# mpitid/babble

Measured on AMD Instinct MI355X. Metric: consensus-ordered events/sec at N participants, higher is better.
Workload: dtype int32; 1 GPU; random-gossip DAG, 256 participants, 10000000 events per GPU, RunConsensus every K=256 events (39063 calls); participants=256, events_per_graph=10000000, k=256, graphs_per_gpu=1, parallelism=replicas1

## Files before the change

### babble_amd/csrc/hge_engine.hip

```cpp
#include <hip/hip_runtime.h>

#include <algorithm>
#include <chrono>
#include <cstdio>
#include <cstdlib>
#include <cstring>
#include <mutex>
#include <optional>
#include <string>
#include <thread>
#include <utility>
#include <vector>

#include "../../include/hge.h"
#include "hge_plan.h"
#include "hge_kernels.hip"
#include "hge_median_rows.hip"
#include "hge_wide32.hip"
#include "hge_coords.hip"
#include "hge_coords_win.hip"
#include "hge_rounds_coop.hip"
#include "hge_rounds_direct.hip"
#include "hge_walk_spec.hip"

// ... 104 lines not shown

  int R = 0;
  int R_set = 0;
  std::vector<std::vector<int32_t>> h_chain;
  int64_t cache_size = 0;
  int32_t chain_limit = INT32_MAX;
  int32_t chain_limit0 = INT32_MAX;
  bool wide32 = false, wide32_pending = false;
  int w32_done = 0;
  std::string failed;
  int test_w32_fail = getenv("HGE_TEST_W32_FAIL") ? atoi(getenv("HGE_TEST_W32_FAIL")) : 0;
  int lcr = -1;
  int lcre = 0;
  int64_t ctx = 0;
  std::vector<int32_t> consensus;
  int32_t* pin_ord = nullptr;
  int32_t* pin_ord_dev = nullptr;
  size_t pin_ord_cap = 0;
  int64_t cons_pin_n = 0;
  bool lazy_order = false;
  int64_t consensus_size() const { return (int64_t)consensus.size() + cons_pin_n; }
  void consensus_sync() {
    if (!cons_pin_n) return;
    consensus.insert(consensus.end(), pin_ord, pin_ord + cons_pin_n);
    cons_pin_n = 0;
  }
  void ensure_pin_ord(size_t n) {
    if (n <= pin_ord_cap && pin_ord) return;
    consensus_sync();
    if (pin_ord) HIPCHK(hipHostFree(pin_ord));
    pin_ord = nullptr;
    pin_ord_dev = nullptr;
    pin_ord_cap = 0;
    HIPCHK(hipHostMalloc((void**)&pin_ord, std::max<size_t>(n, 1) * 4, hipHostMallocDefault));
    pin_ord_cap = std::max<size_t>(n, 1);
    void* dp = nullptr;
    pin_ord_dev = hipHostGetDevicePointer(&dp, pin_ord, 0) == hipSuccess ? (int32_t*)dp : nullptr;
  }
  int64_t n_und = 0;

  std::vector<int64_t> replay_calls;
  std::vector<int64_t> replay_counts;

  int64_t Ecap = 0;
  int ccap = 0, Rcap = 0;
  DBuf<int32_t> d_creator, d_index, d_sp, d_op, d_ntx, d_round, d_rr, d_und;
  DBuf<int64_t> d_ts, d_cts;
  DBuf<uint64_t> d_S;
  DBuf<uint8_t> d_coin, d_wit;
  DBuf<int32_t> d_chain, d_LA, d_FD, d_FSS;
  DBuf<int32_t> s_w32, s_w32a;
  DBuf<uint32_t> d_LA16;
  DBuf<int2> d_opcp;
  DBuf<int64_t> d_tsch;
  DBuf<int32_t> d_C, d_W, d_rcnt, d_minw;
  DBuf<uint64_t> d_ssb, d_seeb;
  DBuf<uint8_t> d_fame;
  DBuf<int32_t> s_small, s_newwit;
  DBuf<int32_t> s_LCR, s_clast;
  DBuf<uint8_t> s_dec, s_decbit;
  DBuf<int32_t> s_segcnt, s_segcall, s_seground, s_theta;
  DBuf<uint8_t> s_segdec;
  DBuf<uint64_t> s_segfws;
  DBuf<int32_t> s_recv, s_rr, s_fund, s_upos, s_und2, s_bpos, s_vis;
  bool vis_all = false;
  DBuf<int64_t> s_cts;
  DBuf<unsigned char> s_keys, s_keys2;
  DBuf<int32_t> s_part, s_fst, s_relay, s_rfail;
  DBuf<uint8_t> s_dec2;
  bool minw_full = true;
  int n_sweeps = 0;
  DBuf<int32_t> d_FDT, s_chg, s_bar, s_dirty;
  DBuf<int32_t> s_src;
  DBuf<int4> s_lwplan;
  DBuf<uint32_t> s_lwsum, s_lwinit;
  DBuf<int32_t> s_lwpos, s_lwrisky;
  int ncu_cache = 0;
  int n_cu() {
    if (!ncu_cache) HIPCHK(hipDeviceGetAttribute(&ncu_cache, hipDeviceAttributeMultiprocessorCount, device));
    return ncu_cache;
  }
  DBuf<int32_t> d_FDTD;
  DBuf<uint8_t> d_FDTW;
  bool rows_bulk = false;
  bool fdtd_stale = false;
  int fdtd_maxlen = 0;
  DBuf<int32_t> s_fdlo;
  bool test_rows_fallback = getenv("HGE_TEST_MEDIAN_ROWS_FALLBACK") != nullptr;
  DBuf<int32_t> d_WLA;
  DBuf<uint16_t> d_WLR;
  DBuf<uint64_t> d_ssc, s_gran;
  DBuf<int32_t> s_bseg;
  DBuf<uint64_t> s_H;
  DBuf<int32_t> s_hn, s_hres;
  uint32_t walk_epoch = 0;
  int walk_chk[2] = {448, 2};
  bool coop_checked = false;
  int coop_nb = 0, coop_ncu = 0, coop_spec_nb = -1, coop_spec_bs = 0;
  const void* coop_spec_fn() const {
    return coop_spec_bs == 1024 ? (const void*)k_rounds_coop_spec<1024> : (const void*)k_rounds_coop_spec<512>;
  }
  DBuf<uint64_t> s_cH, s_cS, s_cT, s_cM;
  DBuf<uint32_t> s_mb;
  DBuf<int32_t> s_cn;
  uint32_t coop_epoch = 0;

  hipEvent_t ev[8] = {};
  bool prof_on = false;
  std::vector<hipEvent_t> prof_pool;
  std::vector<std::pair<std::string, int>> prof_rec;
  std::vector<std::string> prof_names;
  std::vector<double> prof_ms;
  std::vector<int64_t> prof_cnt;
  int R_div = 0;
  std::vector<int32_t> h_minw;
  DBuf<int32_t> s_cctl, s_out;
  std::vector<int32_t> h_cctl;
  int64_t* c_nc = nullptr;
  int32_t *c_Rc = nullptr, *c_Lc = nullptr, *c_flags = nullptr, *c_pr = nullptr, *c_pidx = nullptr;
  int32_t* c_sgo = nullptr;
  const int32_t* segoff_p = nullptr;
  DBuf<int32_t> s_kctl;
  std::vector<int32_t> h_kctl;
  std::vector<hge_plan::Seg> h_segs;
  bool und_fresh = false;
  float stage_ms[7] = {};

  Tables tables() const {
    Tables t;
    t.N = N;
    t.NW = NW;
    t.SM = SM;
    t.ccap = ccap;
    t.Rcap = Rcap;
    t.creator = d_creator.p;
    t.index = d_index.p;
    t.sp = d_sp.p;
    t.op = d_op.p;
    t.ts = d_ts.p;
    t.S = d_S.p;
    t.coin = d_coin.p;
    t.ntx = d_ntx.p;
    t.chain = d_chain.p;
    t.opcp = d_opcp.p;
    t.tsch = d_tsch.p;
    t.LA = d_LA.p;
    t.NW2 = (N + 1) / 2;
    t.LA16 = sweep16() ? d_LA16.p : nullptr;
    t.FD = fdt16() ? nullptr : d_FD.p;
    t.FD16 = fdt16() ? (uint16_t*)d_FD.p : nullptr;
    t.FDTD = d_FDTD.p;
    t.FDTW = d_FDTW.p;
    t.WLA = wla16() ? nullptr : d_WLA.p;
    t.WLA16 = wla16() ? (uint16_t*)d_WLA.p : nullptr;
    t.WLR = (N > 64 && !wide32) ? d_WLR.p : nullptr;
    t.round = d_round.p;
    t.wit = d_wit.p;
    t.C = d_C.p;
    t.W = d_W.p;
    t.ssb = d_ssb.p;
    t.seeb = d_seeb.p;
    t.fame = d_fame.p;
    t.rcnt = d_rcnt.p;
    return t;
  }

  void init(int n, int64_t cap, int dev) {
    N = n;
    NW = (N + 63) / 64;
    SM = 2 * N / 3 + 1;
    device = dev;
    HIPCHK(hipSetDevice(device));
    HIPCHK(hipStreamCreateWithFlags(&st, hipStreamNonBlocking));
    for (auto& e : ev) HIPCHK(hipEventCreate(&e));
    chain_len.assign(N, 0);
    chain_last.assign(N, -1);
    h_chain.assign(N, {});
    chain_limit = N > 32 ? 0xFFFE : INT32_MAX;
    if (const char* cl = getenv("HGE_CHAIN_LIMIT")) chain_limit = std::max(1, std::min(chain_limit, atoi(cl)));
    chain_limit0 = chain_limit;
    coords_len.assign(N, 0);
    const int64_t c0 = std::max<int64_t>(cap, 1024);
    ensure_events(c0);
    ensure_ccap(c0 / N + c0 / (8 * N) + 64);
    ensure_rcap(c0 / (2 * N) + 64);
    s_small.need(16);
  }

  void prof_begin(const char* name) {
    if (!prof_on) return;
    const int slot = (int)prof_rec.size() * 2;
    while ((int)prof_pool.size() < slot + 2) {
      hipEvent_t e;
      HIPCHK(hipEventCreate(&e));
      prof_pool.push_back(e);
    }
    HIPCHK(hipEventRecord(prof_pool[slot], st));
    prof_rec.push_back({name, slot});
  }
  void prof_end() {
    if (!prof_on) return;
    HIPCHK(hipEventRecord(prof_pool[prof_rec.back().second + 1], st));
  }
  void prof_collect() {
    if (prof_rec.empty()) return;
    HIPCHK(hipStreamSynchronize(st));
    for (auto& r : prof_rec) {
      float ms = 0;
      HIPCHK(hipEventElapsedTime(&ms, prof_pool[r.second], prof_pool[r.second + 1]));
      size_t k = 0;
      while (k < prof_names.size() && prof_names[k] != r.first) k++;
      if (k == prof_names.size()) {
        prof_names.push_back(r.first);
        prof_ms.push_back(0);
        prof_cnt.push_back(0);
      }
      prof_ms[k] += ms;
      prof_cnt[k] += 1;
    }
    prof_rec.clear();
  }

  DBuf<uint64_t> s_dbg;
  bool dbg_on = getenv("HGE_STAMPS") != nullptr;
  uint64_t* dbg_p() {
    if (!dbg_on) return nullptr;
    if (!s_dbg.p) {
      s_dbg.need(16);
      HIPCHK(hipMemset(s_dbg.p, 0, 16 * 8));
    }
    return s_dbg.p;
  }
  void dbg_dump() {
    if (!dbg_on || !s_dbg.p) return;
    uint64_t v[16];
    readback(v, s_dbg.p, 16);
    fprintf(stderr, "[hge stamps]");
    for (int i = 0; i < 16; i++) fprintf(stderr, " %llu", (unsigned long long)v[i]);
    fprintf(stderr, "\n");
  }

  void destroy() {
    if (st) (void)hipStreamSynchronize(st);
    if (getenv("HGE_HOST_PHASES") && hp.calls) {
      const double c = (double)hp.calls;
      fprintf(stderr,
              "{\"hge_host_phases\": {\"calls\": %lld, \"launches_per_call\": %.2f, \"copies_per_call\": %.2f, "
              "\"insert_us\": %.2f, \"consensus_us\": %.2f, \"sync_wait_us\": %.2f}}\n",
              (long long)hp.calls, hp.launches / c, hp.copies / c, hp.insert_ns / c / 1e3, hp.call_ns / c / 1e3,
              hp.wait_ns / c / 1e3);
    }
    for (auto& e : ev)
      if (e) (void)hipEventDestroy(e);
    for (auto& e : prof_pool) (void)hipEventDestroy(e);
    prof_pool.clear();
    DBuf<int32_t>* i32s[] = {&d_creator, &d_index,  &d_sp,    &d_op,     &d_ntx,     &d_round,
                             &d_rr,      &d_und,    &d_chain, &d_LA,     &d_FD,      &d_C,
                             &d_W,       &d_rcnt,   &d_minw,  &s_small,  &s_newwit,  &s_LCR,
                             &s_clast,   &s_segcnt, &s_segcall, &s_seground, &s_theta,
                             &s_recv,    &s_rr,     &s_bpos,  &s_fund,   &s_upos,    &s_vis,
                             &s_und2,    &s_part,   &s_fst,    &d_FSS,
                             &d_FDT,     &s_chg,    &s_bar,   &s_bseg,   &s_kctl,    &s_cctl,
                             &s_out,     &s_hn,     &s_hres,  &s_dirty,  &d_WLA,     &s_lwpos,
                             &s_lwrisky, &s_src,    &s_relay, &s_rfail,  &s_fdlo};
    for (auto* b : i32s) b->free_();
    s_dec2.free_();
    s_lwplan.free_();
    d_WLR.free_();
    s_xbuf.free_();
    s_sord.free_();
    s_soff.free_();
    s_lwsum.free_();
    s_lwinit.free_();
    d_ts.free_();
    d_FDTD.free_();
    d_FDTW.free_();
    d_cts.free_();
    s_cts.free_();
    d_S.free_();
    d_ssb.free_();
    d_seeb.free_();
    s_H.free_();
    s_wdbg.free_();
    s_segfws.free_();
    d_coin.free_();
    d_wit.free_();
    d_fame.free_();
    s_dec.free_();
    s_decbit.free_();
    s_segdec.free_();
    s_keys.free_();
    s_keys2.free_();
    d_opcp.free_();
    d_tsch.free_();
    d_LA16.free_();
    d_ssc.free_();
    s_gran.free_();
    s_cH.free_();
    s_cS.free_();
    s_cT.free_();
    s_cM.free_();
    s_cn.free_();
    s_mb.free_();
    s_hist.free_();
    s_hstate.free_();
    s_hssc.free_();
    if (pin) (void)hipHostFree(pin);
    pin = nullptr;
    pin_cap = pin_used = 0;
    if (pin_ord) (void)hipHostFree(pin_ord);
    pin_ord = nullptr;
    pin_ord_dev = nullptr;
    pin_ord_cap = 0;
    cons_pin_n = 0;
    if (st) (void)hipStreamDestroy(st);
    st = nullptr;
  }

  void ensure_events(int64_t m) {
    if (m <= Ecap) return;
    int64_t cap = std::max<int64_t>(m, Ecap + Ecap / 2);
    d_creator.grow_keep(cap, n_dev, st);
    d_index.grow_keep(cap, n_dev, st);
    d_sp.grow_keep(cap, n_dev, st);
    d_op.grow_keep(cap, n_dev, st);
    d_ntx.grow_keep(cap, n_dev, st);
    d_ts.grow_keep(cap, n_dev, st);
    d_S.grow_keep(4 * cap, 4 * n_dev, st);
    d_coin.grow_keep(cap, n_dev, st);
    d_round.grow_keep(cap, n_coords, st);
    d_wit.grow_keep(cap, n_coords, st);
    d_rr.grow_keep(cap, n_coords, st, 0xFF);
    d_cts.grow_keep(cap, n_coords, st, 0);
    d_und.grow_keep(cap, n_und, st);
    Ecap = cap;
  }

  template <typename T>
  void grow_chain_table(DBuf<T>& b, int64_t nc, bool keep, bool rowmajor = true) {
    T* q = nullptr;
    HIPCHK(hipMalloc(&q, sizeof(T) * (size_t)N * nc * N));
    const size_t rows = rowmajor ? N : (size_t)N * N, w = rowmajor ? N : 1;
    if (keep && ccap > 0 && b.p)
      HIPCHK(hipMemcpy2DAsync(q, sizeof(T) * nc * w, b.p, sizeof(T) * ccap * w,
                              sizeof(T) * ccap * w, rows, hipMemcpyDeviceToDevice, st));
    sync();
    b.free_();
    b.p = q;
    b.n = (size_t)N * nc * N;
  }

  void ensure_ccap(int64_t m) {
    if (m <= ccap) return;
    int64_t nc = (std::max<int64_t>(m, (int64_t)ccap + ccap / 2) + 63) & ~(int64_t)63;
    int32_t* chain = nullptr;
    HIPCHK(hipMalloc(&chain, sizeof(int32_t) * N * nc));
    HIPCHK(hipMemsetAsync(chain, 0xFF, sizeof(int32_t) * N * nc, st));
    if (ccap > 0)
      HIPCHK(hipMemcpy2DAsync(chain, sizeof(int32_t) * nc, d_chain.p, sizeof(int32_t) * ccap,
                              sizeof(int32_t) * ccap, N, hipMemcpyDeviceToDevice, st));
    sync();
    d_chain.free_();
    d_chain.p = chain;
    d_chain.n = (size_t)N * nc;
    int2* opcp = nullptr;
    HIPCHK(hipMalloc(&opcp, sizeof(int2) * N * nc));
    if (ccap > 0)
      HIPCHK(hipMemcpy2DAsync(opcp, sizeof(int2) * nc, d_opcp.p, sizeof(int2) * ccap,
                              sizeof(int2) * ccap, N, hipMemcpyDeviceToDevice, st));
    sync();
    d_opcp.free_();
    d_opcp.p = opcp;
    d_opcp.n = (size_t)N * nc;
    int64_t* tsch = nullptr;
    HIPCHK(hipMalloc(&tsch, sizeof(int64_t) * N * nc));
    if (ccap > 0)
      HIPCHK(hipMemcpy2DAsync(tsch, sizeof(int64_t) * nc, d_tsch.p, sizeof(int64_t) * ccap,
                              sizeof(int64_t) * ccap, N, hipMemcpyDeviceToDevice, st));
    sync();
    d_tsch.free_();
    d_tsch.p = tsch;
    d_tsch.n = (size_t)N * nc;
    if (!sweep16()) grow_chain_table(d_LA, nc, true);
    if (N > 32) {
      const size_t w = (size_t)(N + 1) / 2;
      uint32_t* q = nullptr;
      HIPCHK(hipMalloc(&q, sizeof(uint32_t) * (size_t)N * nc * w));
      if (ccap > 0 && d_LA16.p)
        HIPCHK(hipMemcpy2DAsync(q, sizeof(uint32_t) * nc * w, d_LA16.p, sizeof(uint32_t) * ccap * w,
                                sizeof(uint32_t) * ccap * w, N, hipMemcpyDeviceToDevice, st));
      sync();
      d_LA16.free_();
      d_LA16.p = q;
      d_LA16.n = (size_t)N * nc * w;
    }
    if (fdt16()) {
      int32_t* q = nullptr;
      HIPCHK(hipMalloc(&q, sizeof(uint16_t) * (size_t)N * nc * N));
      if (ccap > 0 && d_FD.p)
        HIPCHK(hipMemcpy2DAsync(q, 2 * (size_t)nc * N, d_FD.p, 2 * (size_t)ccap * N, 2 * (size_t)ccap * N, N,
                                hipMemcpyDeviceToDevice, st));
      sync();
      d_FD.free_();
      d_FD.p = q;
      d_FD.n = (size_t)N * nc * N / 2;
    } else {
      grow_chain_table(d_FD, nc, true);
    }
    if (N > 16) {
      grow_chain_table(d_FDTD, nc, true);
      const size_t NT = (size_t)(N + 63) / 64;
      uint8_t* q = nullptr;
      HIPCHK(hipMalloc(&q, (size_t)N * nc * NT));
      if (ccap > 0 && d_FDTW.p)
        HIPCHK(hipMemcpy2DAsync(q, nc * NT, d_FDTW.p, (size_t)ccap * NT, (size_t)ccap * NT, N,
                                hipMemcpyDeviceToDevice, st));
      sync();
      d_FDTW.free_();
      d_FDTW.p = q;
      d_FDTW.n = (size_t)N * nc * NT;
    }
    if (N <= 32) d_FSS.need((size_t)N * nc * std::max(N, 16));
    if (fdt16()) {
      int32_t* q = nullptr;
      HIPCHK(hipMalloc(&q, sizeof(int32_t) * (size_t)N * nc * N));
      if (ccap > 0 && d_FDT.p)
        HIPCHK(hipMemcpy2DAsync(q, 2 * (size_t)nc, d_FDT.p, 2 * (size_t)ccap, 2 * (size_t)ccap, (size_t)N * N,
                                hipMemcpyDeviceToDevice, st));
      sync();
      d_FDT.free_();
      d_FDT.p = q;
      d_FDT.n = (size_t)N * nc * N;
    } else {
      grow_chain_table(d_FDT, nc, true, false);
    }
    ccap = (int)nc;
  }

  void ensure_rcap(int64_t m) {
    if (m <= Rcap) return;
    int64_t nr = std::max<int64_t>(m, (int64_t)Rcap + Rcap / 2);
    const size_t oldn = (size_t)Rcap * N;
    d_C.grow_keep(nr * N, oldn, st, 0x7F);
    d_W.grow_keep(nr * N, oldn, st, 0xFF);
    d_ssb.grow_keep(nr * N * NW, oldn * NW, st, 0);
    d_seeb.grow_keep(nr * N * NW, oldn * NW, st, 0);
    if (N > 32) d_ssc.grow_keep(nr * N * NW, oldn * NW, st, 0);
    d_fame.grow_keep(nr * N, oldn, st, 0);
    d_rcnt.grow_keep(nr, Rcap, st, 0);
    d_minw.need(nr + 20);
    minw_full = true;
    fill_i32(d_C.p + oldn, (int64_t)(nr - Rcap) * N, INF32);
    sync();
    Rcap = (int)nr;
  }

  void reset_state() {
    sync();
    failed.clear();
    minw_full = true;
    cons_pin_n = 0;
    h_creator.clear();
    h_index.clear();
    h_sp.clear();
    h_op.clear();
    h_ntx.clear();
    h_ts.clear();
    h_S.clear();
    h_coin.clear();
    chain_len.assign(N, 0);
    chain_last.assign(N, -1);
    h_chain.assign(N, {});
    coords_len.assign(N, 0);
    n_events = n_dev = n_coords = n_divided = 0;
    up_n0 = up_n1 = -1;
    h_up.clear();
    R = 0;
    R_set = 0;
    h_minw.clear();
    lcr = -1;
    lcre = 0;
    ctx = 0;
    consensus.clear();
    n_und = 0;
    wide32 = wide32_pending = false;
    w32_done = 0;
    chain_limit = chain_limit0;
    reset_rounds();
    HIPCHK(hipMemsetAsync(d_chain.p, 0xFF, (size_t)N * ccap * 4, st));
    sync();
  }

  void reset_rounds() {
    const int64_t nrow = (int64_t)Rcap * N, nbits = nrow * NW;
    const int64_t most = std::max<int64_t>(std::max(nbits, Ecap), Rcap);
    KLAUNCH(k_reset_rounds, dim3(std::min(div_up(most, 256), 4096)), dim3(256), 0, st, tables(), nrow,
            nbits, Ecap, d_rr.p);
  }

  int admit(const hge_event& e, int32_t sp, int32_t op) {
    const int c = e.creator;
    if (c < 0 || c >= N) {
      err = "Could not find fake creator id";
      return HGE_ERR_CREATOR;
    }
    const int known = chain_len[c];
    if (sp == HGE_NONE && op == HGE_NONE && known == 0) {
      if (e.index != 0) {
        err = "Event index does not match the creator's chain position";
        return HGE_ERR_INDEX;
      }
      return HGE_OK;
    }
    if (sp < 0 || sp >= n_events) {
      err = "Self-parent not known";
      return HGE_ERR_SELF_PARENT_UNKNOWN;
    }
    if (h_creator[sp] != c) {
      err = "Self-parent has different creator";
      return HGE_ERR_SELF_PARENT_CREATOR;
    }
    if (op < 0 || op >= n_events) {
      err = "Other-parent not known";
      return HGE_ERR_OTHER_PARENT_UNKNOWN;
    }
    if (sp != chain_last[c]) {
      err = "Self-parent not last known event by creator";
      return HGE_ERR_SELF_PARENT_NOT_LAST;
    }
    if (e.index != known) {
      err = "Event index does not match the creator's chain position";
      return HGE_ERR_INDEX;
    }
    if (known >= chain_limit) {
      if (N > 32 && N <= 256 && !wide32) {
        size_t free_b = 0, total_b = 0;
        const size_t tab = sizeof(int32_t) * (size_t)N * N * (size_t)std::max(ccap, known + 2);
        if (hipMemGetInfo(&free_b, &total_b) == hipSuccess && free_b < (fdt16() ? 2 : 1) * tab + (64u << 20)) {
          err = "Chain capacity exceeded: the int32 position tables past 65,534 events per creator do not fit";
          return HGE_ERR_CAPACITY;
        }
        wide32_pending = true;
        chain_limit = INT32_MAX;
      } else {
        err = "Chain capacity exceeded: at most " + std::to_string(chain_limit) + " events per creator";
        return HGE_ERR_CAPACITY;
      }
    }
    return HGE_OK;
  }

  void append(const hge_event& e, int32_t sp, int32_t op) {
    const int64_t id = n_events++;
    h_creator.push_back(e.creator);
    h_index.push_back(e.index);
    h_sp.push_back(sp);
    h_op.push_back(op);
    h_ntx.push_back(e.n_tx);
    h_ts.push_back(e.timestamp_ns);
    for (int k = 0; k < 4; k++) {
      uint64_t v = 0;
      for (int b = 0; b < 8; b++) v = (v << 8) | e.s[8 * k + b];
      h_S.push_back(v);
    }
    h_coin.push_back(e.hash[16] != 0 ? 1 : 0);
    h_chain[e.creator].push_back((int32_t)id);
    chain_len[e.creator]++;
    chain_last[e.creator] = (int32_t)id;
  }

  std::vector<UpEv> h_up;
  int64_t up_n0 = -1, up_n1 = -1;
  void upload() {
    if (n_dev == n_events) return;
    ensure_events(n_events);
    int maxlen = 0;
    for (int c = 0; c < N; c++) maxlen = std::max(maxlen, chain_len[c]);
    ensure_ccap(maxlen + 1);
    const int64_t a = n_dev, m = n_events - n_dev;
    if (m <= 16384 && a == n_coords) {
      std::vector<UpEv> up((size_t)m);
      if (up_n0 >= 0) throw EngineError(HGE_ERR_INTERNAL, "packed upload pending twice");
      for (int64_t i = 0; i < m; i++) {
        UpEv& r = up[(size_t)i];
        const size_t x = (size_t)(a + i);
        r.creator = h_creator[x];
        r.index = h_index[x];
        r.sp = h_sp[x];
        r.op = h_op[x];
        r.ntx = h_ntx[x];
        r.coin = h_coin[x];
        r.ts = h_ts[x];
        for (int k = 0; k < 4; k++) r.S[k] = h_S[4 * x + k];
      }
      h_up.swap(up);
      up_n0 = a;
      up_n1 = n_events;
      n_dev = n_events;
      return;
    }
    HIPCHK(hipMemcpyAsync(d_creator.p + a, h_creator.data() + a, 4 * m, hipMemcpyHostToDevice, st));
    HIPCHK(hipMemcpyAsync(d_index.p + a, h_index.data() + a, 4 * m, hipMemcpyHostToDevice, st));
    HIPCHK(hipMemcpyAsync(d_sp.p + a, h_sp.data() + a, 4 * m, hipMemcpyHostToDevice, st));
    HIPCHK(hipMemcpyAsync(d_op.p + a, h_op.data() + a, 4 * m, hipMemcpyHostToDevice, st));
    HIPCHK(hipMemcpyAsync(d_ntx.p + a, h_ntx.data() + a, 4 * m, hipMemcpyHostToDevice, st));
    HIPCHK(hipMemcpyAsync(d_ts.p + a, h_ts.data() + a, 8 * m, hipMemcpyHostToDevice, st));
// ... 356 lines not shown
      s_fst.need(N + 1);
      KLAUNCH(k_frontier_start, dim3(1), dim3(256), 0, st, t, s.olen, s.len, s_fst.p, (int32_t*)nullptr,
              (int32_t*)nullptr, (uint64_t*)nullptr, 0);
      readback(fst.data(), s_fst.p, N + 1);
    }
    const int rlo = fst[0];
    if (rlo == INF32) return {};
    int tot = s.fresh ? s.tot0 : 0;
    if (!s.fresh) {
      std::vector<int32_t> lo_off(2 * N + 1);
      for (int c = 0; c < N; c++) {
        lo_off[c] = fst[1 + c];
        lo_off[N + c] = tot;
        tot += std::max(0, chain_len[c] - fst[1 + c]);
      }
      lo_off[2 * N] = tot;
      h2d(s.fss_lo, lo_off.data(), 4 * (2 * N + 1));
    }
    if (tot <= 0) return {};
    const bool long_chain = s.maxlen >= 0xFFFF;
    KLAUNCH_AS(k.fss_name, k.fss, dim3(div_up((int64_t)tot * k.NPC, 256)), dim3(256), 0, st, t, s.fss_lo, s.fss_off, tot,
               long_chain ? d_FSS.p : (int32_t*)nullptr, long_chain ? (uint16_t*)nullptr : (uint16_t*)d_FSS.p,
               (const int32_t*)nullptr);
    if (long_chain) {
      KLAUNCH_AS(k.rounds_fss_name, k.rounds_fss, dim3(1), dim3(64), 0, st, t, d_FSS.p, s.olen, s.len, s.rstate, rlo);
      return {};
    }
    const int nw = s.fresh ? spec_walkers(s.minlen) : 0;
    const int32_t* resume = nw > 1 ? spec_walk(t, s, k, nw) : nullptr;
    KLAUNCH_AS(k.walk_name, k.walk, dim3(1), dim3(1024), 0, st, t, (const uint16_t*)d_FSS.p, s.olen, s.len, s.rstate,
               resume ? 0 : rlo, resume ? 0 : Rprev, dbg_p(), resume, RoundAssign{});
    if (resume && getenv("HGE_WALK_DEBUG")) walk_debug(nw);
    return {};
  }
  const int32_t* spec_walk(const Tables& t, const CoordStep& s, const WalkKernels& k, int nw) {
    const char* hc = getenv("HGE_WALK_HCAP");
    const int Hcap = hc ? std::max(2, atoi(hc)) : std::max(256, std::min(Rcap, 3 * (Rcap / nw) + 256));
    if ((size_t)nw * Hcap * N > s_H.n) {
      s_H.need((size_t)nw * Hcap * N);
      HIPCHK(hipMemsetAsync(s_H.p, 0, s_H.n * sizeof(uint64_t), st));
    }
    s_hres.need(4 * (size_t)nw + 1);
    s_hn.need(2 * (size_t)nw);
    KLAUNCH_AS(k.spec_name, k.spec, dim3(nw), dim3(1024), 0, st, t, (const uint16_t*)d_FSS.p, s.len, nw, Hcap, s_H.p,
               s_hn.p, s_hn.p + nw, (int4*)s_hres.p, ++walk_epoch, walk_chk[0], walk_chk[1], walk_dbg(nw));
    int32_t* resume = s_hres.p + 4 * nw;
    KLAUNCH(k_walk_join, dim3(64), dim3(256), 0, st, t, (const uint64_t*)s_H.p, (const int32_t*)s_hn.p,
            (const int4*)s_hres.p, nw, Hcap, s.rstate, resume);
    return resume;
  }
  void assign_rounds(const CoordStep& s, const Walk& w) {
    const Tables t = tables();
    const int m = (int)(s.n1 - s.n0);
    s_newwit.need(m);
    if (s.fresh) {
      s_newwit.need((size_t)Rcap * N);
      KLAUNCH(k_round_ranges, dim3(div_up((int64_t)Rcap * N, 256)), dim3(256), 0, st, t, s.len,
              (const int32_t*)s.rstate, s_newwit.p, s.rstate + 2);
    } else if (!w.assigned) {
      und_appended = dividing && n_divided == s.n0;
      KLAUNCH(k_round_assign, dim3(div_up(m, 256)), dim3(256), 0, st, t, (int)s.n0, (int)s.n1,
              (const int32_t*)s.rstate, s_newwit.p, s.rstate + 2, und_appended ? d_und.p + n_und : (int32_t*)nullptr);
    }
  }
  int rounds_tail(const CoordStep& s, const Walk& w) {
    if (w.tail_done) return 0;
    const Tables t = tables();
    const int m = (int)(s.n1 - s.n0), G = wit_group();
    const int64_t n_mr = n_und + (s.n1 - n_divided);
    const int mr = !s.fresh && n_mr <= 65536 ? (int)std::max<int64_t>(1, std::min<int64_t>(16, div_up(n_mr, 2048))) : 0;
    const int64_t wmax = std::min<int64_t>(m, (int64_t)Rcap * N);
    const int nb_wb = std::max(1, std::min(div_up(wmax * NW * G, 256), 8192));
    KLAUNCH(k_round_tail, dim3(nb_wb + div_up(Rcap, 4) + mr), dim3(256), 0, st, t, s_newwit.p, s.rstate + 2,
            N > 32 ? (const uint64_t*)d_ssc.p : nullptr, G, nb_wb, (const int32_t*)s.rstate, d_minw.p, w.err_src, mr,
            (const int32_t*)d_und.p, (int)n_und, (int)n_divided, (int)s.n1);
    if (!s.fresh && !mr) {
      int32_t* mnr = d_minw.p + Rcap + hge_plan::kTailMinRound;
      if (n_und > 0)
        KLAUNCH(k_min_round, dim3(div_up(n_und, 256)), dim3(256), 0, st, d_round.p, d_und.p, (int)n_und, mnr);
      if (s.n1 > n_divided)
        KLAUNCH(k_min_round_range, dim3(div_up(s.n1 - n_divided, 256)), dim3(256), 0, st, d_round.p,
                (int)n_divided, (int)s.n1, mnr);
    }
    return mr;
  }
  RoundsOutcome read_rounds(const CoordStep& s, const Walk& w, int mr) {
    h_minw.resize(Rcap + hge_plan::kTailPartial + mr);
    d2h(h_minw.data(), d_minw.p, 4 * h_minw.size());
    sync();
    minw_full = false;
    const hge_plan::RoundsTail r = hge_plan::parse_rounds_tail(h_minw.data() + Rcap, mr);
    if (!s.fresh) mnr_pre = r.min_round;
    mnr_key[0] = s.fresh ? -1 : n_und;
    mnr_key[1] = n_divided;
    mnr_key[2] = s.n1;
    if (w.err_src ? r.handoff_err != 0 : w.host_err) return RoundsOutcome::HandoffTimeout;
    if (r.overflow) return RoundsOutcome::Grow;
    R = r.R;
    h_minw.resize(R);
    return RoundsOutcome::Done;
  }

  int spec_walkers(int minlen) {
    const char* ev = getenv("HGE_WALKERS");
    const int env = ev ? atoi(ev) : -1;
    const int nw = env >= 0 ? env : (minlen >= 4 * 192 ? std::min(32, minlen / 192) : 0);
    return std::max(0, std::min(nw, 64));
  }

  DBuf<uint64_t> s_wdbg;
  uint64_t* walk_dbg(int nw) {
    if (!getenv("HGE_WALK_DEBUG")) return nullptr;
    s_wdbg.need(4 * (size_t)nw);
    return s_wdbg.p;
  }
  void walk_debug(int nw) {
    std::vector<int32_t> res(4 * nw + 1), hn(nw);
    std::vector<uint64_t> wd(4 * nw);
    readback(res.data(), s_hres.p, res.size());
    readback(hn.data(), s_hn.p, hn.size());
    readback(wd.data(), s_wdbg.p, wd.size());
    fprintf(stderr, "walk: nw=%d resume=%d |", nw, res[4 * nw]);
    for (int w = 0; w < nw; w++)
      fprintf(stderr, " %d:%d[%d,%d,%d,%d](%llu/%llu/%llu)", w, hn[w], res[4 * w], res[4 * w + 1],
              res[4 * w + 2], res[4 * w + 3], (unsigned long long)wd[4 * w],
              (unsigned long long)wd[4 * w + 1], (unsigned long long)wd[4 * w + 2]);
    fprintf(stderr, "\n");
  }

  int coop_walkers(int minlen) {
    const int sbs = N > 64 ? 1024 : COOP_SPEC_BS;
    if (sbs != coop_spec_bs) {
      coop_spec_bs = sbs;
      HIPCHK(hipOccupancyMaxActiveBlocksPerMultiprocessor(&coop_spec_nb, coop_spec_fn(), sbs, 0));
    }
    const int cap = (int)std::min<int64_t>(16, (int64_t)coop_spec_nb * coop_ncu / N);
    const char* ev = getenv("HGE_COOP_WALKERS");
    int nw = ev ? atoi(ev) : (minlen >= 1024 && N <= 128 ? 8 : 0);
    nw = std::min(nw, cap);
    return nw >= 2 ? nw : 0;
  }

  std::vector<std::pair<std::pair<const void*, int>, int>> resident_nb;
  hipError_t launch_resident(const void* fn, dim3 grid, dim3 block, void** args) {
    const int bs = (int)(block.x * block.y * block.z);
    int nb = -1;
    for (auto& e : resident_nb)
      if (e.first.first == fn && e.first.second == bs) nb = e.second;
    if (nb < 0) {
      HIPCHK(hipOccupancyMaxActiveBlocksPerMultiprocessor(&nb, fn, bs, 0));
      resident_nb.push_back({{fn, bs}, nb});
    }
    const int64_t blocks = (int64_t)grid.x * grid.y * grid.z;
    if ((int64_t)nb * n_cu() < blocks)
      throw EngineError(HGE_ERR_DEVICE, "frontier grid of " + std::to_string(blocks) + " workgroups x " +
                                            std::to_string(bs) + " threads cannot be co-resident (" +
                                            std::to_string(nb) + " per CU x " + std::to_string(n_cu()) + " CUs)");
    return hipLaunchKernel(fn, grid, block, args, 0, st);
  }
  static std::mutex& frontier_mutex(int dev) {
    static std::mutex m[64];
    return m[dev & 63];
  }
  std::unique_lock<std::mutex> frontier_lock() { return std::unique_lock<std::mutex>(frontier_mutex(device)); }

  bool direct_rounds() const { return (N & 3) == 0; }

  bool frontier_fallback = false;
  int64_t n_frontier_fallbacks = 0;
  Walk rounds_coop(CoordStep& s) {
    const Tables t = tables();
    s_fst.need(N + 1);
    s_bar.need(2);
    s_gran.need(2 * (size_t)N);
    if (!s.take_frontier_start())
      KLAUNCH(k_frontier_start, dim3(1), dim3(256), 0, st, t, s.olen, s.len, s_fst.p, (int32_t*)nullptr,
              s_bar.p, (uint64_t*)s_gran.p, 2 * N);
    int32_t rlo = s.fresh ? INF32 : 0;
    const int32_t* rlo_dev = s.fresh ? nullptr : s_fst.p;
    if (s.fresh) readback(&rlo, s_fst.p, 1);
    if (rlo == INF32) return {};
    const int Rprev = R;
    if (!coop_resident()) {
      frontier_fallback = true;
      return rounds_step32(s);
    }
    if (s.maxlen >= 0xFFFF)
      throw EngineError(HGE_ERR_INTERNAL, "packed rounds walk reached a chain past 65,534 events");
    const bool from_zero = s.fresh && rlo == 0 && Rprev == 0;
    if (ext_on && from_zero && install_ext_rows(s, rlo)) return {};
    Walk w;
    const int nw = from_zero && rlo == 0 ? coop_walkers(s.minlen) : 0;
    if (nw >= 2) {
      const int resume = coop_spec_walk(t, s, nw, Rprev, w);
      if (resume < 0) return w;
      rlo = resume;
    }
    wide_walk(t, s, rlo, rlo_dev, Rprev);
    w.err_src = s_bar.p + 1;
    dbg_dump();
    return w;
  }
  bool coop_resident() {
    if (coop_checked) return true;
    int nb = 0, ncu = 0, coop = 0;
    HIPCHK(hipOccupancyMaxActiveBlocksPerMultiprocessor(&nb, (const void*)k_rounds_coop, COOP_BS, 0));
    HIPCHK(hipDeviceGetAttribute(&ncu, hipDeviceAttributeMultiprocessorCount, device));
    HIPCHK(hipDeviceGetAttribute(&coop, hipDeviceAttributeCooperativeLaunch, device));
    if (!coop || (int64_t)nb * ncu < N) return false;
    coop_nb = nb;
    coop_ncu = ncu;
    coop_checked = true;
    return true;
  }
  bool install_ext_rows(const CoordStep& s, int32_t& rlo) {
    const int K = ext_rows;
    if (K + 1 >= Rcap) {
      const int32_t ov[2] = {0, hge_plan::kRoundsFull};
      h2d(s.rstate, ov, 8);
      return true;
    }
    ext_on = false;
    h2d(d_C.p, ext_C.data(), sizeof(int32_t) * (size_t)K * N);
    if (K > 1) h2d(d_ssc.p + (size_t)N * NW, ext_ssc.data() + (size_t)N * NW, sizeof(uint64_t) * (size_t)(K - 1) * N * NW);
    if (ext_natural) {
      const int32_t rs0 = K;
      h2d(s.rstate, &rs0, 4);
      return true;
    }
    rlo = K - 1;
    return false;
  }
  int coop_spec_walk(Tables t, const CoordStep& s, int nw, int Rprev, Walk& w) {
    const int32_t* FDT = d_FDT.p;
    const int32_t* olen = s.olen;
    const int32_t* len = s.len;
    int32_t* err = s_bar.p + 1;
    const char* hc = getenv("HGE_WALK_HCAP");
    const int Hcap = hc ? std::max(2, std::min(0xFFFF, atoi(hc)))
                        : std::min(0xFFFF, std::min(Rcap, std::max(256, 3 * (Rcap / nw) + 256)));
    int TS = 64;
    while (TS < 2 * Hcap) TS <<= 1;
    const size_t nh = (size_t)nw * Hcap * N, nt = (size_t)nw * TS;
    const size_t hn0 = s_cH.n, tn0 = s_cT.n;
    s_cH.need(nh);
    s_cT.need(nt);
    bool clear = s_cH.n != hn0 || s_cT.n != tn0;
    if (++coop_epoch >= 0x7FFFFFFFu) {
      coop_epoch = 1;
      clear = true;
    }
    if (clear) {
      HIPCHK(hipMemsetAsync(s_cH.p, 0, s_cH.n * sizeof(uint64_t), st));
      HIPCHK(hipMemsetAsync(s_cT.p, 0, s_cT.n * sizeof(uint64_t), st));
    }
    s_cS.need(nh * NW);
    s_cM.need(nw);
    s_cn.need(2 * (size_t)nw + 1);
    HIPCHK(hipMemsetAsync(s_cM.p, 0xFF, (size_t)nw * sizeof(uint64_t), st));
    int64_t nev = 0;
    for (int c = 0; c < N; c++) nev += chain_len[c];
    const int guess = N <= 64 ? 1 : 2;
    CoopSpec cs{s_cH.p, s_cS.p, s_cT.p, (unsigned long long*)s_cM.p, s_cn.p, nw, Hcap, TS,
                coop_epoch, nev, guess};
    void* sargs[] = {&t, &FDT, &olen, &len, &cs, &err};
    prof_begin("k_rounds_coop_spec");
    HIPCHK(launch_resident(coop_spec_fn(), dim3(nw * N), dim3(coop_spec_bs), sargs));
    prof_end();
    int32_t* resume = s_cn.p + 2 * nw;
    KLAUNCH(k_coop_join, dim3(64), dim3(256), 0, st, t, cs, d_ssc.p, s.rstate, resume);
    int32_t hres[2] = {0, 0};
    readback(&hres[0], err, 1);
    if (hres[0]) {
      const int32_t down[2] = {Rprev, hge_plan::kRoundsStoodDown};
      h2d(s.rstate, down, 8);
      w.host_err = true;
      return -1;
    }
    readback(&hres[1], resume, 1);
    if (getenv("HGE_WALK_DEBUG")) {
      std::vector<int32_t> hn(2 * nw);
      std::vector<uint64_t> mg(nw);
      readback(hn.data(), s_cn.p, hn.size());
      readback(mg.data(), s_cM.p, mg.size());
      fprintf(stderr, "coop walk: nw=%d Hcap=%d resume=%d |", nw, Hcap, hres[1]);
      for (int i = 0; i < nw; i++)
        fprintf(stderr, " %d:%d%s->(%d,w%d:%d)", i, hn[i], hn[nw + i] ? "e" : "",
                mg[i] == ~0ull ? -1 : (int)(mg[i] >> 32),
                mg[i] == ~0ull ? -1 : i + (int)((mg[i] >> 16) & 0xFFFF), (int)(mg[i] & 0xFFFF));
      fprintf(stderr, "\n");
    }
    return hres[1];
  }
  void wide_walk(Tables t, const CoordStep& s, int32_t rlo, const int32_t* rlo_dev, int Rprev) {
    const int32_t* FDT = d_FDT.p;
    const int32_t* olen = s.olen;
    const int32_t* len = s.len;
    int32_t* rstate = s.rstate;
    int32_t* err = s_bar.p + 1;
    uint64_t* gran = s_gran.p;
    uint64_t* ssc = d_ssc.p;
    uint64_t* dbg = dbg_p();
    if (direct_rounds()) {
      s_mb.need((size_t)npow() * npow());
      uint32_t* mb = s_mb.p;
      const int32_t* nostart = nullptr;
      int32_t* nohist = nullptr;
      int hmax = 0, extra = 0;
      const char* hs = getenv("HGE_TEST_HANDOFF_STALL");
      int stall_ep = hs ? atoi(hs) : 0;
      void* dargs[] = {&t, &olen, &len, &rstate, &rlo, &rlo_dev, &Rprev, &gran, &err, &ssc, &mb, &dbg,
                       &nostart, &nohist, &hmax, &nostart, &extra, &stall_ep};
      prof_begin("k_rounds_direct");
      HIPCHK(launch_resident(direct_fn(), dim3(N), dim3(1024), dargs));
      prof_end();
    } else {
      void* args[] = {&t, &FDT, &olen, &len, &rstate, &rlo, &rlo_dev, &Rprev, &gran, &err, &ssc, &dbg};
      prof_begin("k_rounds_coop");
      HIPCHK(launch_resident((const void*)k_rounds_coop, dim3(N), dim3(COOP_BS), args));
      prof_end();
    }
    if (getenv("HGE_TEST_HANDOFF_FAIL")) {
      const int32_t one = 1, down = hge_plan::kRoundsStoodDown;
      h2d(err, &one, 4);
      h2d(rstate + 1, &down, 4);
    }
  }
  const void* direct_fn() const {
    return N <= 64 ? (const void*)k_rounds_direct<1024, 64>
         : N <= 128 ? (const void*)k_rounds_direct<1024, 128>
                    : (const void*)k_rounds_direct<1024, 256>;
  }

  bool sweep16() const { return N > 32 && !wide32; }
  bool wla16() const { return N > 192 && (N & 3) == 0 && !wide32; }

  void to_wide32() {
    auto test_stop = [&](int stage) {
      if (test_w32_fail == stage) {
        test_w32_fail = 0;
        throw EngineError(HGE_ERR_DEVICE, "test: to_wide32 stopped after stage " + std::to_string(stage));
      }
    };
    ensure_fdtd();
    if (!(w32_done & 4)) {
      grow_chain_table(d_LA, ccap, false);
      w32_done |= 4;
      test_stop(1);
    }
    if (fdt16()) {
      const size_t n = (size_t)N * N * ccap;
      for (int which = 0; which < 2; which++) {
        if (w32_done & (1 << which)) continue;
        DBuf<int32_t>& b = which ? d_FD : d_FDT;
        int32_t* q = nullptr;
        HIPCHK(hipMalloc(&q, sizeof(int32_t) * n));
        KLAUNCH(k_fdt16_to32, dim3((unsigned)std::min<size_t>(div_up(n, 256), 65536)), dim3(256), 0, st,
                (const uint16_t*)b.p, q, n, which);
        sync();
        b.free_();
        b.p = q;
        b.n = n;
        w32_done |= 1 << which;
        test_stop(2 + which);
      }
    }
    s_w32.need(N);
    h2d(s_w32.p, coords_len.data(), 4 * (size_t)N);
    wide32 = true;
    wide32_pending = false;
    w32_done = 0;
    Tables t = tables();
    int64_t most = 1;
    for (int c = 0; c < N; c++) most = std::max<int64_t>(most, (int64_t)coords_len[c] * N);
    KLAUNCH(k_la16_to_la32, dim3((unsigned)std::min<int64_t>(div_up(most, 256), 4096), N), dim3(256), 0, st, t,
            (const uint32_t*)d_LA16.p, (const int32_t*)s_w32.p);
  }

  Walk rounds_step32(const CoordStep& s) {
    Tables t = tables();
    s_fst.need(N + 1);
    KLAUNCH(k_frontier_start, dim3(1), dim3(256), 0, st, t, s.olen, s.len, s_fst.p, (int32_t*)nullptr,
            (int32_t*)nullptr, (uint64_t*)nullptr, 0);
    int32_t rlo = INF32;
    readback(&rlo, s_fst.p, 1);
    if (rlo == INF32) return {};
    const int Rprev = R, NB = 32;
    s_w32a.need(NB);
    for (int r = rlo;;) {
      HIPCHK(hipMemsetAsync(s_w32a.p, 0, 4 * NB, st));
      int k = 0;
      for (; k < NB && r + k + 1 < Rcap; k++)
        KLAUNCH(k_round_step32, dim3(N), dim3(256), 0, st, t, (const int32_t*)s.olen, (const int32_t*)s.len,
                r + k, Rprev, d_ssc.p, s_w32a.p + k);
      std::vector<int32_t> alive(NB, 0);
      readback(alive.data(), s_w32a.p, NB);
      for (int q = 0; q < k; q++)
        if (!alive[q]) {
          const int32_t rs[2] = {std::max(R, r + q + 1), 0};
          h2d(s.rstate, rs, 8);
          return {};
        }
      r += k;
      if (k < NB) {
        const int32_t rs[2] = {R, hge_plan::kRoundsFull};
        h2d(s.rstate, rs, 8);
        return {};
      }
    }
  }

  bool fdt16() const { return N > 128 && (N & 3) == 0 && !wide32; }

  bool la_windows() const { return N > 32 && N <= 256 && !wide32; }

  void la_windows_run(const Tables& t, const CoordStep& s) {
    const int32_t* olen = s.olen;
    const int32_t* len = s.len;
    const int64_t n0 = s.n0, n1 = s.n1, ne = n1 - n0;
    const int npow = this->npow();
    const int W = t.NW2;
    const int64_t WMIN = 4096;
    const int per_cu = npow == 256 ? 1 : 2;
    int64_t G = std::min<int64_t>((int64_t)n_cu() * per_cu, std::max<int64_t>(1, ne / WMIN));
    if (const char* g = getenv("HGE_LW_G")) G = std::max(1, atoi(g));
    int64_t WN = (div_up(ne, G) + LW_K - 1) / LW_K * LW_K;
    G = div_up(ne, WN);
    s_lwplan.need(ne);
    s_lwsum.need(ne);
    s_lwinit.need((size_t)G * N * W);
    s_lwpos.need((size_t)G * N);
    s_lwrisky.need(G);
    const int MAXP = 64;
    s_chg.need(MAXP);
    const int32_t* wpos = G == 1 ? olen : s_lwpos.p;
    int32_t* risky = G == 1 ? s.risky1 : s_lwrisky.p;
    if (G > 1)
      KLAUNCH(k_lw_pos, dim3(div_up(std::max<int64_t>(G * N, MAXP), 256)), dim3(256), 0, st, t, n0, (int)WN, (int)G,
              len, s_lwpos.p, s_lwrisky.p, s_chg.p, MAXP);
    if (G > 1)
      KLAUNCH(k_lw_plan, dim3(div_up(div_up(ne, LW_K), 4)), dim3(256), 0, st, t, n0, n1, (int)WN, len, s_lwplan.p,
              risky);
    int p = 0;
    for (int group = G == 1 ? 1 : 3;; group = 2) {
      for (int g = 0; g < group; g++, p++) {
        if (p >= MAXP) throw EngineError(HGE_ERR_INTERNAL, "lastAncestors windows did not converge");
        const int32_t* prev = p > 0 ? s_chg.p + p - 1 : nullptr;
        const int pass = p + 1;
#define LWIN(NP)                                                                                         \
  KLAUNCH(k_la_win<NP>, dim3(G), dim3(1024), 0, st, t, s_lwplan.p, n0, n1, (int)WN, wpos, olen,          \
          s_lwinit.p, risky, s_lwsum.p, pass, prev, s_chg.p + p,                                        \
          G == 1 && p == 0 ? len : (const int32_t*)nullptr)
        if (npow == 64) LWIN(64);
        else if (npow == 128) LWIN(128);
        else LWIN(256);
#undef LWIN
      }
      if (G == 1) {
        n_sweeps = 1;
        break;
      }
      std::vector<int32_t> flags(p);
      readback(flags.data(), s_chg.p, p);
      if (!flags[p - 1]) {
        n_sweeps = (int)(std::find(flags.begin(), flags.end(), 0) - flags.begin()) + 1;
        break;
      }
    }
  }

  bool la_seq_ok(int64_t m) const {
    return !sweep16() && N <= 32 && m > 0 && m * (N <= 16 ? 16 : 32) <= LASEQ_MAX && !getenv("HGE_NO_LASEQ");
  }
  static constexpr int MAXSW = 4096;
  void last_ancestors(const Tables& t, CoordStep& s) {
    s_chg.need(MAXSW);
    if (s.la == CoordStep::La::Windows) {
      la_windows_run(t, s);
    } else if (s.la == CoordStep::La::Seq) {
      la_seq_run(t, s);
    } else {
      la_sweeps_run(t, s);
    }
  }
  void la_seq_run(const Tables& t, CoordStep& s) {
    const bool q = !s.fresh, fst = q && s.maxlen < 0xFFFF;
    const bool fd = q && N <= 16 && !getenv("HGE_NO_FD_DIRECT");
    if (fst) s_fst.need(N + 1);
    int32_t* fp = fst ? s_fst.p : (int32_t*)nullptr;
    int32_t* fl = fst ? s.fss_lo : (int32_t*)nullptr;
    const int nq = q && !fd ? N : 0;
    const int nb = 1 + nq + (fst ? 1 : 0);
    if (N <= 16)
      KLAUNCH(k_la_seq<16>, dim3(nb), dim3(256), 0, st, t, (int)s.n0, (int)s.n1, s.up, s.up_dst,
              (const int32_t*)s.olen, (const int32_t*)s.len, nq ? s.qlo : (int32_t*)nullptr, fp, fl,
              fd ? d_FDT.p : (int32_t*)nullptr);
    else
      KLAUNCH(k_la_seq<32>, dim3(nb), dim3(256), 0, st, t, (int)s.n0, (int)s.n1, s.up, s.up_dst,
              (const int32_t*)s.olen, (const int32_t*)s.len, nq ? s.qlo : (int32_t*)nullptr, fp, fl,
              (int32_t*)nullptr);
    s.frontier_started = fst;
    s.qlo_done = q;
    s.fd_done = fd;
    n_sweeps = 1;
  }
  void la_sweeps_run(const Tables& t, const CoordStep& s) {
    const int32_t* olen = s.olen;
    const int32_t* len = s.len;
    const int nseg = s.nseg, SEG = s.SEG, maxnew = s.maxnew;
    const bool p16 = sweep16();
    if (p16) s_dirty.need(nseg);
    int32_t* dirty = p16 ? s_dirty.p : nullptr;
    if (p16)
      KLAUNCH(k_la_clear16, dim3(std::max(1, std::min(64, div_up((int64_t)maxnew * t.NW2, 256))), N),
              dim3(256), 0, st, t, olen, len, s_chg.p, MAXSW, dirty, nseg);
    else
      KLAUNCH(k_la_clear, dim3(std::max(1, std::min(64, div_up((int64_t)maxnew * N, 256))), N),
              dim3(256), 0, st, t, olen, len, s_chg.p, MAXSW);
    const int NPt = p16 ? (t.NW2 <= 32 ? 32 : t.NW2 <= 64 ? 64 : 128)
                        : (N <= 16 ? 16 : N <= 32 ? 32 : N <= 64 ? 64 : N <= 128 ? 128 : 256);
    int sw = 0;
    for (int group = 12;; group = 8) {
      for (int g = 0; g < group; g++, sw++) {
        if (sw >= MAXSW) throw EngineError(HGE_ERR_INTERNAL, "lastAncestors sweeps did not converge");
        const int32_t* prev = sw > 0 ? s_chg.p + sw - 1 : nullptr;
        if (p16) {
          switch (NPt) {
#define SW16(NPV)                                                                                \
  case NPV:                                                                                      \
    KLAUNCH(k_la_sweep16<NPV>, dim3(div_up(nseg, 256 / NPV)), dim3(256), 0, st, t, s.segs, nseg, \
            SEG, len, prev, s_chg.p + sw, olen, s.segbase, dirty, sw);                          \
    break;
            SW16(32)
            SW16(64)
            SW16(128)
#undef SW16
          }
        } else {
          switch (NPt) {
#define SW(NPV)                                                                                  \
  case NPV:                                                                                      \
    KLAUNCH(k_la_sweep<NPV>, dim3(div_up(nseg, 256 / NPV)), dim3(256), 0, st, t, s.segs, nseg,   \
            SEG, len, prev, s_chg.p + sw);                                                       \
    break;
            SW(16)
            SW(32)
            SW(64)
            SW(128)
            SW(256)
#undef SW
          }
        }
      }
      std::vector<int32_t> flags(sw);
      readback(flags.data(), s_chg.p, sw);
      if (!flags[sw - 1]) {
        n_sweeps = (int)(std::find(flags.begin(), flags.end(), 0) - flags.begin()) + 1;
        break;
      }
    }
  }
  void fdtd_pass(const char* name, int zgrid) {
    const Tables t = tables();
    KLAUNCH_AS(name, (k_fd_transpose_ts<uint16_t>), dim3(N, div_up(N, 64), std::max(1, std::min(zgrid, 65535))),
               dim3(256), 0, st, t, (const uint16_t*)d_FDT.p, (const int32_t*)s_fdlo.p,
               (const int32_t*)(s_fdlo.p + N), (const int32_t*)nullptr, (const int32_t*)nullptr);
  }
  void ensure_fdtd() {
    if (!fdtd_stale) return;
    if (!fdt16()) throw EngineError(HGE_ERR_INTERNAL, "stale FD timestamp rows past the uint16 runs");
    HIPCHK(hipMemsetAsync(s_fdlo.p, 0, 4 * (size_t)N, st));
    fdtd_pass("fdtd_ensure (k_fd_transpose_ts<uint16_t>)", div_up(std::max(fdtd_maxlen, 1), 64));
    fdtd_stale = false;
  }
  void first_descendants(const Tables& t, const CoordStep& s) {
    if (s.fd_done) return;
    if (!s.fresh) ensure_fdtd();
    const int32_t* olen = s.olen;
    const int32_t* len = s.len;
    const int maxnew = s.maxnew;
    if (fdt16()) {
      KLAUNCH((k_la16_rows_runs<uint16_t>), dim3(div_up(maxnew + 1, 64), div_up(N, 64), N), dim3(256), 0, st, t,
              (uint16_t*)d_FDT.p, s.plo, olen, len);
    } else if (sweep16()) {
      KLAUNCH((k_la16_rows_runs<int32_t>), dim3(div_up(maxnew + 1, 64), div_up(N, 64), N), dim3(256), 0, st, t,
              d_FDT.p, s.plo, olen, len);
    } else {
      KLAUNCH((k_la16_rows_runs<int32_t, true>), dim3(div_up(maxnew + 1, 64), div_up(N, 64), N), dim3(256), 0,
              st, t, d_FDT.p, s.plo, olen, len);
    }
    int span = 1;
    if (!s.fresh) {
      if (!s.qlo_done) KLAUNCH(k_fd_qlo, dim3(N), dim3(256), 0, st, t, olen, len, s.qlo);
      span = maxnew + 64;
    } else {
      span = std::max(span, s.maxlen);
    }
    if (s.fresh) fdtd_stale = false;
    if (s.fd_rows_only) {
      KLAUNCH(k_fd_rows16, dim3(N, div_up(N, 64), std::min(div_up(span, 64), 65535)), dim3(256), 0, st, t,
              (const uint16_t*)d_FDT.p, (const int32_t*)s.qlo, len);
      s_fdlo.need(2 * (size_t)N);
      h2d(s_fdlo.p + N, chain_len.data(), 4 * (size_t)N);
      fdtd_maxlen = s.maxlen;
      fdtd_stale = true;
    } else if (fdt16())
      KLAUNCH((k_fd_transpose_ts<uint16_t>), dim3(N, div_up(N, 64), std::min(div_up(span, 64), 65535)), dim3(256),
              0, st, t, (const uint16_t*)d_FDT.p, s.qlo, len, (const int32_t*)s.cand_lo,
              (const int32_t*)s.cand_hi);
    else if (N > 16)
      KLAUNCH((k_fd_transpose_ts<int32_t>), dim3(N, div_up(N, 64), std::min(div_up(span, 64), 65535)), dim3(256),
              0, st, t, (const int32_t*)d_FDT.p, s.qlo, len, (const int32_t*)s.cand_lo,
              (const int32_t*)s.cand_hi);
    else
      KLAUNCH(k_transpose, dim3(div_up(span, 64), div_up(N, 64), N), dim3(256), 0, st, t, d_FDT.p,
              (int32_t*)nullptr, s.qlo, len, 1);
  }


  enum class OrderRan {
    Stages,
    CallFront,
    CallTail,
  };
  struct Batch {
    const int64_t* calls = nullptr;
    int ncalls = 0;
    bool do_fame = false, do_order = false, commit = false;
    std::vector<int32_t>* order_out = nullptr;
// ... 1004 lines not shown
  GUARD_END(h)
}

int hge_decide_fame(hge_engine* h) {
  GUARD_BEGIN
  REFUSE_IF_FAILED(h)
    h->consensus_batch({h->n_divided}, true, false, false, nullptr, nullptr);
  return HGE_OK;
  GUARD_END(h)
}

int hge_decide_round_received(hge_engine* h) {
  GUARD_BEGIN
  REFUSE_IF_FAILED(h)
    h->consensus_batch({h->n_divided}, false, true, false, nullptr, nullptr);
  return HGE_OK;
  GUARD_END(h)
}

int hge_find_order(hge_engine* h, int32_t* ids_out, int64_t cap, int64_t* n_out) {
  GUARD_BEGIN
  REFUSE_IF_FAILED(h)
    std::vector<int32_t> order;
  h->consensus_batch({h->n_divided}, false, true, true, &order, nullptr);
  for (int64_t i = 0; i < (int64_t)order.size() && i < cap && ids_out; i++) ids_out[i] = order[i];
  if (n_out) *n_out = (int64_t)order.size();
  return HGE_OK;
  GUARD_END(h)
}

int hge_run_consensus(hge_engine* h, int32_t* ids_out, int64_t cap, int64_t* n_out) {
  GUARD_BEGIN
  REFUSE_IF_FAILED(h)
  const int64_t c0 = hge_engine::now_ns();
  std::vector<int32_t> order;
  if (!h->online_fast(order)) {
    h->divide();
    h->consensus_batch({h->n_divided}, true, true, true, &order, nullptr);
  }
  for (int64_t i = 0; i < (int64_t)order.size() && i < cap && ids_out; i++) ids_out[i] = order[i];
  if (n_out) *n_out = (int64_t)order.size();
  h->hp.calls++;
  h->hp.call_ns += hge_engine::now_ns() - c0;
  return HGE_OK;
  GUARD_END(h)
}

int hge_replay_prepare(hge_engine* h, const hge_event* ev, int64_t n_sub,
                       const int64_t* call_points, int64_t n_calls, int32_t* status_out) {
  GUARD_BEGIN
  if (n_sub < 0 || (n_sub > 0 && !ev) || n_calls < 0 || (n_calls > 0 && !call_points)) {
    h->err = "hge_replay_prepare: bad argument";
    return HGE_ERR_ARG;
  }
  for (int64_t c = 0; c < n_calls; c++) {
    if (call_points[c] < 1 || call_points[c] > n_sub || (c > 0 && call_points[c] <= call_points[c - 1])) {
      h->err = "hge_replay_prepare: call points must be strictly ascending within [1, n_sub]";
      return HGE_ERR_ARG;
    }
  }
  h->reset_state();
  h->sp = hge_engine::SplitPlan();
  h->sp_active = false;
  std::vector<int32_t> idmap(n_sub, -1);
  h->replay_calls.clear();
  int64_t nc = 0;
  for (int64_t i = 0; i < n_sub; i++) {
    const int32_t s = ev[i].self_parent, o = ev[i].other_parent;
    int32_t sp = s < 0 ? HGE_NONE : (s < i && idmap[s] >= 0 ? idmap[s] : HGE_UNKNOWN);
    int32_t op = o < 0 ? HGE_NONE : (o < i && idmap[o] >= 0 ? idmap[o] : HGE_UNKNOWN);
    int r = h->admit(ev[i], sp, op);
    if (r == HGE_OK) {
      idmap[i] = (int32_t)h->n_events;
      h->append(ev[i], sp, op);
    }
    if (status_out) status_out[i] = r == HGE_OK ? idmap[i] : r;
    while (nc < n_calls && call_points[nc] == i + 1) {
      h->replay_calls.push_back(h->n_events);
      nc++;
    }
  }
  h->upload();
  h->cons_pin_n = 0;
  h->ensure_pin_ord((size_t)h->n_events);
  HIPCHK(hipStreamSynchronize(h->st));
  return HGE_OK;
  GUARD_END(h)
}

static void replay_begin(hge_engine* h) {
  h->n_coords = h->n_divided = 0;
  h->coords_len.assign(h->N, 0);
  h->R = 0;
  h->h_minw.clear();
  h->lcr = -1;
  h->lcre = 0;
  h->ctx = 0;
  h->consensus.clear();
  h->cons_pin_n = 0;
  h->n_und = 0;
  h->ext_on = false;
  h->w_start = std::chrono::steady_clock::now();
  h->reset_rounds();
  HIPCHK(hipEventRecord(h->ev[0], h->st));
  h->coords_a();
}

static void replay_end(hge_engine* h, int64_t* n_ordered) {
  const int64_t keep = h->n_events;
  if (h->cstep) h->coords_b();
  HIPCHK(hipEventRecord(h->ev[1], h->st));
  const auto w1 = std::chrono::steady_clock::now();
  h->n_divided = keep;
  h->update_rdiv();
  if (keep > 0) h->fill_iota(h->d_und.p, keep, 0);
  h->n_und = keep;
  h->und_fresh = keep > 0;
  h->replay_counts.clear();
  h->lazy_order = h->pin_ord_cap >= (size_t)keep;
  try {
    h->consensus_batch(h->replay_calls, true, true, true, nullptr, &h->replay_counts);
  } catch (...) {
    h->lazy_order = false;
    throw;
  }
  h->lazy_order = false;
  HIPCHK(hipEventRecord(h->ev[2], h->st));
  HIPCHK(hipEventSynchronize(h->ev[2]));
  const auto w2 = std::chrono::steady_clock::now();
  float a = 0, b = 0;
  HIPCHK(hipEventElapsedTime(&a, h->ev[0], h->ev[1]));
  HIPCHK(hipEventElapsedTime(&b, h->ev[1], h->ev[2]));
  auto ms = [](std::chrono::steady_clock::time_point x, std::chrono::steady_clock::time_point y) {
    return (float)std::chrono::duration<double, std::milli>(y - x).count();
  };
  h->stage_ms[0] = a;
  h->stage_ms[1] = ms(h->w_start, w1);
  h->stage_ms[2] = ms(w1, w2);
  h->stage_ms[3] = b;
  h->stage_ms[4] = ms(h->w_start, w2);
  h->stage_ms[6] = a + b;
  if (n_ordered) *n_ordered = h->consensus_size();
  h->dbg_dump();
}

int hge_replay_run(hge_engine* h, int64_t* n_ordered) {
  GUARD_BEGIN
  REFUSE_IF_FAILED(h)
  h->sp_active = false;
  if (h->rec_on) h->rec_dec.clear();
  struct Bulk {
    hge_engine* h;
    ~Bulk() { h->rows_bulk = false; }
  } bulk{h};
  h->rows_bulk = true;
  replay_begin(h);
  h->rows_bulk = false;
  replay_end(h, n_ordered);
  if (h->rec_on) {
    const int64_t E = h->n_events;
    h->consensus_sync();
    h->rec_order = h->consensus;
    h->rec_counts = h->replay_counts;
    h->rec_rr.resize(E);
    h->rec_cts.resize(E);
    h->readback(h->rec_rr.data(), h->d_rr.p, (size_t)E);
    h->readback(h->rec_cts.data(), h->d_cts.p, (size_t)E);
    h->rec_left.resize(h->n_und);
    if (h->n_und) h->readback(h->rec_left.data(), h->d_und.p, (size_t)h->n_und);
    h->rec_on = false;
    h->rec_have = true;
  }
  return HGE_OK;
  GUARD_END(h)
}

int hge_split_plan(hge_engine* h, int32_t part, int32_t nparts, const int64_t* ev_bounds,
                   const int32_t* call_bounds, const int64_t* cand_lo) {
  if (!h) return HGE_ERR_ARG;
  GUARD_BEGIN
  if (nparts <= 1) {
    h->sp = hge_engine::SplitPlan();
    return HGE_OK;
  }
  auto bad = [&](const char* why) {
    h->err = std::string("hge_split_plan: ") + why;
    return HGE_ERR_ARG;
  };
  if (h->N <= 32 || !h->direct_rounds() || h->wide32 || h->wide32_pending)
    return bad("needs the wide direct rounds path (N > 32, N % 4 == 0, chains below 65,535 events)");
  if (part < 0 || part >= nparts || !ev_bounds || !call_bounds || !cand_lo) return bad("bad argument");
  const int64_t E = h->n_events;
  const int ncalls = (int)h->replay_calls.size();
  if (ev_bounds[0] != 0 || ev_bounds[nparts] != E || call_bounds[0] != 0 || call_bounds[nparts] != ncalls)
    return bad("the bounds must cover the staged stream and its calls");
  for (int g = 0; g < nparts; g++) {
    if (ev_bounds[g + 1] < ev_bounds[g] || call_bounds[g + 1] <= call_bounds[g])
      return bad("bounds must ascend and every part needs a call");
    if (cand_lo[g] < 0 || cand_lo[g] > ev_bounds[g] || cand_lo[g] >= ev_bounds[g + 1])
      return bad("cand_lo[p] must lie in [0, ev_bounds[p]] below ev_bounds[p + 1]");
  }
  if (E > INT32_MAX) return bad("stream too long");
  h->sp.part = part;
  h->sp.nparts = nparts;
  h->sp.a.assign(ev_bounds, ev_bounds + nparts + 1);
  h->sp.cb.assign(call_bounds, call_bounds + nparts + 1);
  h->sp.clo.assign(cand_lo, cand_lo + nparts);
  return HGE_OK;
  GUARD_END(h)
}

int hge_split_exchange(hge_engine* h, hge_exchange_fn fn, void* ctx) {
  if (!h) return HGE_ERR_ARG;
  h->x_fn = fn;
  h->x_ctx = ctx;
  return HGE_OK;
}

int hge_split_emulate(hge_engine* h, int32_t on) {
  if (!h) return HGE_ERR_ARG;
  h->rec_on = on != 0;
  h->rec_have = false;
  h->rec_dec.clear();
  return HGE_OK;
}

int hge_split_run(hge_engine* h, int64_t* n_ordered) {
  if (!h) return HGE_ERR_ARG;
  GUARD_BEGIN
  if (h->sp.nparts <= 1) {
    h->err = "hge_split_run: no split plan (hge_split_plan)";
    return HGE_ERR_ARG;
  }
  if (!h->x_fn && !h->rec_have) {
    h->err = "hge_split_run: no exchange (hge_split_exchange) and no record (hge_split_emulate)";
    return HGE_ERR_ARG;
  }
  struct Off {
    hge_engine* h;
    ~Off() { h->sp_active = false; }
  } off{h};
  h->sp_active = true;
  replay_begin(h);
  replay_end(h, n_ordered);
  return HGE_OK;
  GUARD_END(h)
}

int hge_split_begin(hge_engine* h) {
  GUARD_BEGIN
  if (h->N <= 32 || !h->direct_rounds() || h->wide32 || h->wide32_pending) {
    h->err = "the split walk needs the wide direct rounds path (N > 32, N % 4 == 0)";
    return HGE_ERR_ARG;
  }
  h->sp_active = false;
  replay_begin(h);
  if (!h->cstep) {
    h->err = "nothing staged (hge_replay_prepare first)";
    return HGE_ERR_ARG;
  }
  return HGE_OK;
  GUARD_END(h)
}

int hge_frontier_guess(hge_engine* h, int32_t part, int32_t nparts, int32_t* start_out) {
  if (!h) return HGE_ERR_ARG;
  GUARD_BEGIN
  if (!start_out || nparts < 1 || part < 0 || part >= nparts) {
    h->err = "hge_frontier_guess: bad argument";
    return HGE_ERR_ARG;
  }
  const int64_t T = h->sp.nparts == nparts ? h->sp.a[part] : h->n_events * (int64_t)part / nparts;
  for (int c = 0; c < h->N; c++) {
    const std::vector<int32_t>& ch = h->h_chain[c];
    const size_t k = std::lower_bound(ch.begin(), ch.end(), (int32_t)T) - ch.begin();
    start_out[c] = k < ch.size() ? (int32_t)k : INF32;
  }
  return HGE_OK;
  GUARD_END(h)
}

int hge_frontier_walk(hge_engine* h, const int32_t* start, const int32_t* stopcut, int32_t extra,
                      int32_t hmax, int32_t* rows_out, uint64_t* ssc_out, int32_t* nrows,
                      int32_t* natural) {
  GUARD_BEGIN
  if (!h->cstep || !start || hmax < 2) return HGE_ERR_ARG;
  const int N = h->N, NW = h->NW;
  h->s_hist.need((size_t)hmax * N + N);
  h->s_hssc.need((size_t)hmax * N * NW);
  h->s_hstate.need(N + 4);
  h->h2d(h->s_hstate.p, start, 4 * (size_t)N);
  int32_t* cut = nullptr;
  if (stopcut) {
    h->s_hist.need((size_t)hmax * N + 2 * N);
    cut = h->s_hist.p + (size_t)hmax * N + N;
    h->h2d(cut, stopcut, 4 * (size_t)N);
  }
  int32_t* rstate = h->s_hstate.p + N;
  HIPCHK(hipMemsetAsync(rstate, 0, 16, h->st));
  h->s_bar.need(2);
  h->s_gran.need(2 * (size_t)N);
  HIPCHK(hipMemsetAsync(h->s_bar.p, 0, 8, h->st));
  HIPCHK(hipMemsetAsync(h->s_gran.p, 0, 16 * (size_t)N, h->st));
  h->s_mb.need((size_t)h->npow() * h->npow());
  auto lk = h->frontier_lock();
  Tables t = h->tables();
  const int32_t* olen = h->cstep->olen;
  const int32_t* len = h->cstep->len;
  int rlo = 0, Rprev = 0;
  const int32_t* rlo_dev = nullptr;
  uint64_t* gran = h->s_gran.p;
  int32_t* err = h->s_bar.p + 1;
  uint64_t* ssc = h->s_hssc.p;
  uint32_t* mb = h->s_mb.p;
  uint64_t* dbg = nullptr;
  const int32_t* st0 = h->s_hstate.p;
  int32_t* hist = h->s_hist.p;
  int hm = hmax, ex = std::max(0, (int)extra), nostall = 0;
  void* args[] = {&t, &olen, &len, &rstate, &rlo, &rlo_dev, &Rprev, &gran, &err, &ssc, &mb, &dbg,
                  &st0, &hist, &hm, &cut, &ex, &nostall};
  h->prof_begin("k_rounds_direct_walk");
  HIPCHK(h->launch_resident(h->direct_fn(), dim3(N), dim3(1024), args));
  h->prof_end();
  int32_t rs[2] = {0, 0}, e = 0;
  h->d2h(rs, rstate, 8);
  h->d2h(&e, err, 4);
  h->sync();
  if (e) throw EngineError(HGE_ERR_DEVICE, "rounds frontier hand-off timed out");
  const int n = std::max(1, std::min(rs[0], hmax));
  if (rows_out) h->readback(rows_out, h->s_hist.p, (size_t)n * N);
  if (ssc_out) h->readback(ssc_out, h->s_hssc.p, (size_t)n * N * NW);
  if (nrows) *nrows = n;
  if (natural) *natural = rs[1] == 0 ? 1 : 0;
  return HGE_OK;
  GUARD_END(h)
}

int hge_frontier_rows(hge_engine* h, int32_t from, int32_t n, int32_t* rows_out, uint64_t* ssc_out) {
  GUARD_BEGIN
  const int N = h->N, NW = h->NW;
  if (from < 0 || n < 0 || (size_t)(from + n) * N > h->s_hist.n) return HGE_ERR_ARG;
  if (rows_out && n) h->d2h(rows_out, h->s_hist.p + (size_t)from * N, 4 * (size_t)n * N);
  if (ssc_out && n) h->d2h(ssc_out, h->s_hssc.p + (size_t)from * N * NW, 8 * (size_t)n * N * NW);
  h->sync();
  return HGE_OK;
  GUARD_END(h)
}

int hge_split_finish(hge_engine* h, const int32_t* rows, const uint64_t* ssc, int32_t nrows,
                     int32_t natural, int64_t* n_ordered) {
  GUARD_BEGIN
  if (!h->cstep || !rows || nrows < 1 || (nrows > 1 && !ssc)) return HGE_ERR_ARG;
  const int N = h->N, NW = h->NW;
  h->ext_on = true;
  h->ext_natural = natural != 0;
  h->ext_rows = nrows;
  h->ext_C.assign(rows, rows + (size_t)nrows * N);
  h->ext_ssc.assign((size_t)nrows * N * NW, 0);
  if (nrows > 1) std::copy(ssc + (size_t)N * NW, ssc + (size_t)nrows * N * NW, h->ext_ssc.begin() + (size_t)N * NW);
  replay_end(h, n_ordered);
  return HGE_OK;
  GUARD_END(h)
}

int hge_replay_fetch(hge_engine* h, int32_t* order_out, int64_t cap, int64_t* call_counts_out) {
  GUARD_BEGIN
  if (order_out) {
    const int64_t a = std::min<int64_t>((int64_t)h->consensus.size(), std::max<int64_t>(cap, 0));
    if (a > 0) memcpy(order_out, h->consensus.data(), 4 * (size_t)a);
    const int64_t b = std::min<int64_t>(h->cons_pin_n, std::max<int64_t>(cap - a, 0));
    const int nt = b >= (1 << 20) ? 8 : 1;
    std::vector<std::thread> th;
    for (int k = 1; k < nt; k++)
      th.emplace_back([=] {
        const int64_t lo = b * k / nt, hi = b * (k + 1) / nt;
        memcpy(order_out + a + lo, h->pin_ord + lo, 4 * (size_t)(hi - lo));
      });
    if (b > 0) memcpy(order_out + a, h->pin_ord, 4 * (size_t)(b / nt));
    for (auto& x : th) x.join();
  }
  if (call_counts_out)
    for (size_t c = 0; c < h->replay_counts.size(); c++) call_counts_out[c] = h->replay_counts[c];
  return HGE_OK;
  GUARD_END(h)
}

int hge_replay_order(hge_engine* h, const int32_t** ids, int64_t* n) {
  if (!h || !ids || !n) return HGE_ERR_ARG;
  GUARD_BEGIN
  if (!h->consensus.empty() || !h->cons_pin_n) h->consensus_sync();
  if (h->cons_pin_n) {
    *ids = h->pin_ord;
    *n = h->cons_pin_n;
  } else {
    *ids = h->consensus.data();
    *n = (int64_t)h->consensus.size();
  }
  return HGE_OK;
  GUARD_END(h)
}

int hge_replay(hge_engine* h, const hge_event* ev, int64_t n_sub, const int64_t* call_points,
               int64_t n_calls, int32_t* status_out, int32_t* order_out, int64_t cap,
               int64_t* n_ordered, int64_t* call_counts_out) {
  int rc = hge_replay_prepare(h, ev, n_sub, call_points, n_calls, status_out);
  if (rc) return rc;
  rc = hge_replay_run(h, n_ordered);
  if (rc) return rc;
  return hge_replay_fetch(h, order_out, cap, call_counts_out);
}

int64_t hge_event_count(hge_engine* h) { return h->n_events; }
int32_t hge_participants(hge_engine* h) { return h->N; }
int32_t hge_rounds(hge_engine* h) { return std::max(h->R_div, h->R_set); }
int32_t hge_last_consensus_round(hge_engine* h) { return h->lcr; }
int32_t hge_last_committed_round_events(hge_engine* h) { return h->lcre; }
int64_t hge_consensus_transactions(hge_engine* h) { return h->ctx; }
int64_t hge_consensus_count(hge_engine* h) { return h->consensus_size(); }
static int64_t window_len(int64_t tot, int64_t size) {
  if (size <= 0 || tot <= 2 * size) return tot;
  return size + (tot - 2 * size - 1) % size + 1;
}
int64_t hge_consensus_events(hge_engine* h, int32_t* ids_out, int64_t cap) {
  try {
    h->consensus_sync();
  } catch (const EngineError& e) {
    h->err = e.msg;
    return -1;
  }
  const int64_t tot = (int64_t)h->consensus.size(), w = window_len(tot, h->cache_size);
  for (int64_t i = 0; i < w && i < cap && ids_out; i++) ids_out[i] = h->consensus[tot - w + i];
  return w;
}
int64_t hge_consensus_log(hge_engine* h, int64_t from, int32_t* ids_out, int64_t cap) {
  try {
    h->consensus_sync();
  } catch (const EngineError& e) {
    h->err = e.msg;
    return -1;
  }
  const int64_t tot = (int64_t)h->consensus.size();
  if (from < 0) from = 0;
  for (int64_t i = from; i < tot && i - from < cap && ids_out; i++) ids_out[i - from] = h->consensus[i];
  return std::max<int64_t>(0, tot - from);
}
int64_t hge_undetermined(hge_engine* h, int32_t* ids_out, int64_t cap) {
  try {
    if (ids_out && h->n_und > 0) {
      int64_t m = std::min<int64_t>(cap, h->n_und);
      h->readback(ids_out, h->d_und.p, m);
    }
  } catch (EngineError& e) {
    h->err = e.msg;
    return e.code;
  }
  return h->n_und;
}
int hge_known(hge_engine* h, int32_t* counts_out) {
  for (int c = 0; c < h->N; c++) counts_out[c] = h->chain_len[c];
  return HGE_OK;
}

static int32_t read1(hge_engine* h, const int32_t* p) {
  int32_t v = -1;
  h->readback(&v, p, 1);
  return v;
}

int32_t hge_round_of(hge_engine* h, int32_t id) {
  try {
    if (id < 0 || id >= h->n_events) return -1;
    h->coords();
    return read1(h, h->d_round.p + id);
  } catch (EngineError& e) {
    h->err = e.msg;
    return e.code;
  }
}
int32_t hge_is_witness(hge_engine* h, int32_t id) {
  try {
    if (id < 0 || id >= h->n_events) return 0;
    h->coords();
    uint8_t v = 0;
    h->readback(&v, h->d_wit.p + id, 1);
    return v;
  } catch (EngineError& e) {
    h->err = e.msg;
    return e.code;
  }
}
int32_t hge_round_witness(hge_engine* h, int32_t round, int32_t creator) {
  try {
    if (round < 0 || round >= h->R || creator < 0 || creator >= h->N) return -1;
    int32_t w = read1(h, h->d_W.p + (size_t)round * h->N + creator);
    if (w >= h->n_divided) return -1;
    return w;
  } catch (EngineError& e) {
    h->err = e.msg;
    return e.code;
  }
}
int32_t hge_fame(hge_engine* h, int32_t round, int32_t creator) {
  try {
    if (hge_round_witness(h, round, creator) < 0) return -1;
    uint8_t v = 0;
    h->readback(&v, h->d_fame.p + (size_t)round * h->N + creator, 1);
    return v;
  } catch (EngineError& e) {
    h->err = e.msg;
    return e.code;
  }
}
int32_t hge_round_events(hge_engine* h, int32_t round) {
  try {
    if (round < 0 || round >= h->R) return 0;
    return read1(h, h->d_rcnt.p + round);
  } catch (EngineError& e) {
    h->err = e.msg;
    return e.code;
  }
}
int hge_round_event_ids(hge_engine* h, int32_t round, int32_t* ids_out, uint8_t* witness_out, int64_t cap,
                        int64_t* n_out) {
  if (!h || !n_out) return HGE_ERR_ARG;
  GUARD_BEGIN
  *n_out = 0;
  h->coords();
  if (round < 0 || round >= h->R || h->n_coords == 0) return HGE_OK;
  const int64_t lo = round < (int)h->h_minw.size() ? std::max<int64_t>(0, h->h_minw[round]) : 0;
  const int64_t n = h->n_coords - lo;
  if (n <= 0) return HGE_OK;
  std::vector<int32_t> rd((size_t)n);
  std::vector<uint8_t> wd((size_t)n);
  h->d2h(rd.data(), h->d_round.p + lo, 4 * (size_t)n);
  h->d2h(wd.data(), h->d_wit.p + lo, (size_t)n);
  h->sync();
  int64_t k = 0;
  for (int64_t i = 0; i < n; i++) {
    if (rd[(size_t)i] != round) continue;
    if (k < cap) {
      if (ids_out) ids_out[k] = (int32_t)(lo + i);
      if (witness_out) witness_out[k] = wd[(size_t)i];
    }
    k++;
  }
  *n_out = k;
  return HGE_OK;
  GUARD_END(h)
}

int32_t hge_round_received(hge_engine* h, int32_t id) {
  try {
    if (id < 0 || id >= h->n_events) return -1;
    return read1(h, h->d_rr.p + id);
  } catch (EngineError& e) {
    h->err = e.msg;
    return e.code;
  }
}
int64_t hge_consensus_timestamp(hge_engine* h, int32_t id) {
  try {
    if (id < 0 || id >= h->n_events) return 0;
    int64_t v = 0;
    h->readback(&v, h->d_cts.p + id, 1);
    return v;
  } catch (EngineError& e) {
    h->err = e.msg;
    return e.code;
  }
}

int hge_coordinates(hge_engine* h, int32_t id, int32_t* la_out, int32_t* fd_out) {
  GUARD_BEGIN
  if (id < 0 || id >= h->n_events) return HGE_ERR_ARG;
  h->coords();
  const size_t off = ((size_t)h->h_creator[id] * h->ccap + h->h_index[id]) * h->N;
  if (la_out) {
    if (h->sweep16()) {
      const size_t w = (size_t)(h->N + 1) / 2;
      std::vector<uint32_t> row(w);
      h->readback(row.data(), h->d_LA16.p + ((size_t)h->h_creator[id] * h->ccap + h->h_index[id]) * w, w);
      for (int c = 0; c < h->N; c++) la_out[c] = (int32_t)((row[c >> 1] >> ((c & 1) * 16)) & 0xFFFFu) - 1;
    } else {
      h->readback(la_out, h->d_LA.p + off, h->N);
    }
  }
  if (fd_out && h->fdt16()) {
    std::vector<uint16_t> row(h->N);
    h->readback(row.data(), (const uint16_t*)h->d_FD.p + off, h->N);
    for (int c = 0; c < h->N; c++) fd_out[c] = row[c] == 0xFFFFu ? INF32 : (int32_t)row[c] - 1;
    return HGE_OK;
  }
  if (fd_out) h->readback(fd_out, h->d_FD.p + off, h->N);
  return HGE_OK;
  GUARD_END(h)
}

int32_t hge_ancestor(hge_engine* h, int32_t x, int32_t y) {
  if (x < 0 || x >= h->n_events || y < 0 || y >= h->n_events) return 0;
  if (x == y) return 1;
  std::vector<int32_t> la(h->N);
  if (hge_coordinates(h, x, la.data(), nullptr)) return 0;
  return la[h->h_creator[y]] >= h->h_index[y] ? 1 : 0;
}
int32_t hge_self_ancestor(hge_engine* h, int32_t x, int32_t y) {
  if (x < 0 || x >= h->n_events || y < 0 || y >= h->n_events) return 0;
  if (x == y) return 1;
  return (h->h_creator[x] == h->h_creator[y] && h->h_index[x] >= h->h_index[y]) ? 1 : 0;
}
int32_t hge_see(hge_engine* h, int32_t x, int32_t y) { return hge_ancestor(h, x, y); }
int32_t hge_strongly_see(hge_engine* h, int32_t x, int32_t y) {
  if (x < 0 || x >= h->n_events || y < 0 || y >= h->n_events) return 0;
  std::vector<int32_t> la(h->N), fd(h->N);
  if (hge_coordinates(h, x, la.data(), nullptr)) return 0;
  if (hge_coordinates(h, y, nullptr, fd.data())) return 0;
  int c = 0;
  for (int i = 0; i < h->N; i++) c += la[i] >= fd[i];
  return c >= h->SM ? 1 : 0;
}
int32_t hge_oldest_self_ancestor_to_see(hge_engine* h, int32_t x, int32_t y) {
  if (x < 0 || x >= h->n_events || y < 0 || y >= h->n_events) return -1;
  std::vector<int32_t> fd(h->N);
  if (hge_coordinates(h, y, nullptr, fd.data())) return -1;
  const int cx = h->h_creator[x];
  const int32_t a = fd[cx];
  if (a <= h->h_index[x]) {
    try {
      return read1(h, h->d_chain.p + (size_t)cx * h->ccap + a);
    } catch (EngineError& e) {
      h->err = e.msg;
      return -1;
    }
  }
  return -1;
}

int hge_set_cache_size(hge_engine* h, int64_t size) {
  if (!h || size < 0) return HGE_ERR_ARG;
  h->cache_size = size;
  return HGE_OK;
}
int64_t hge_cache_size(hge_engine* h) { return h->cache_size; }

int hge_participant_events(hge_engine* h, int32_t creator, int64_t skip, int32_t* ids_out,
                           int64_t cap, int64_t* n_out) {
  if (n_out) *n_out = 0;
  if (creator < 0 || creator >= h->N) {
    h->err = "not found";
    return HGE_ERR_NOT_FOUND;
  }
  const std::vector<int32_t>& ch = h->h_chain[creator];
  const int64_t tot = (int64_t)ch.size();
  if (skip >= tot) return HGE_OK;
  const int64_t oldest = tot - window_len(tot, h->cache_size);
  if (skip < oldest) {
    h->err = "too late";
    return HGE_ERR_TOO_LATE;
  }
  if (skip < 0) skip = 0;
  for (int64_t k = skip; k < tot && k - skip < cap && ids_out; k++) ids_out[k - skip] = ch[k];
  if (n_out) *n_out = tot - skip;
  return HGE_OK;
}

int32_t hge_participant_event(hge_engine* h, int32_t creator, int64_t index) {
  if (!h || creator < 0 || creator >= h->N) return HGE_ERR_NOT_FOUND;
  const std::vector<int32_t>& ch = h->h_chain[creator];
  const int64_t tot = (int64_t)ch.size();
  if (index < 0 || index < tot - window_len(tot, h->cache_size)) return HGE_ERR_TOO_LATE;
  if (index >= tot) return HGE_ERR_NOT_FOUND;
  return ch[index];
}

int32_t hge_last_from(hge_engine* h, int32_t creator) {
  if (creator < 0 || creator >= h->N) return HGE_ERR_NOT_FOUND;
  return h->chain_last[creator];
}

int hge_diff(hge_engine* h, const int32_t* known, int32_t* ids_out, int64_t cap, int64_t* n_out) {
  if (n_out) *n_out = 0;
  if (!known) return HGE_ERR_ARG;
  std::vector<int32_t> ids;
  for (int c = 0; c < h->N; c++) {
    const std::vector<int32_t>& ch = h->h_chain[c];
    const int64_t tot = (int64_t)ch.size(), skip = known[c];
    if (skip >= tot) continue;
    if (skip < tot - window_len(tot, h->cache_size)) {
      h->err = "too late";
      return HGE_ERR_TOO_LATE;
    }
    for (int64_t k = std::max<int64_t>(skip, 0); k < tot; k++) ids.push_back(ch[k]);
  }
  std::sort(ids.begin(), ids.end());
  for (int64_t i = 0; i < (int64_t)ids.size() && i < cap && ids_out; i++) ids_out[i] = ids[i];
  if (n_out) *n_out = (int64_t)ids.size();
  return HGE_OK;
}

int hge_wire_info(hge_engine* h, int32_t id, int32_t* out) {
  if (id < 0 || id >= h->n_events || !out) return HGE_ERR_ARG;
  const int32_t sp = h->h_sp[id], op = h->h_op[id];
  out[0] = sp >= 0 ? h->h_index[sp] : -1;
  out[1] = op >= 0 ? h->h_creator[op] : -1;
  out[2] = op >= 0 ? h->h_index[op] : -1;
  out[3] = h->h_creator[id];
  return HGE_OK;
}

int hge_read_wire_parents(hge_engine* h, int32_t creator_id, int32_t self_parent_index,
                          int32_t other_parent_creator_id, int32_t other_parent_index,
                          int32_t* sp_out, int32_t* op_out) {
  if (creator_id < 0 || creator_id >= h->N) return HGE_ERR_NOT_FOUND;
  int32_t sp = HGE_NONE, op = HGE_NONE;
  if (self_parent_index >= 0) {
    sp = hge_participant_event(h, creator_id, self_parent_index);
    if (sp < 0) return sp;
  }
  if (other_parent_index >= 0) {
    op = hge_participant_event(h, other_parent_creator_id, other_parent_index);
    if (op < 0) return op;
  }
  if (sp_out) *sp_out = sp;
  if (op_out) *op_out = op;
  return HGE_OK;
}

int hge_event_rounds(hge_engine* h, int32_t* round_out, uint8_t* witness_out, int64_t cap) {
  GUARD_BEGIN
  h->coords();
  const int64_t m = std::min<int64_t>(cap, h->n_events);
  if (m > 0 && round_out) h->d2h(round_out, h->d_round.p, 4 * (size_t)m);
  if (m > 0 && witness_out) h->d2h(witness_out, h->d_wit.p, (size_t)m);
  h->sync();
  return HGE_OK;
  GUARD_END(h)
}

int hge_event_received(hge_engine* h, int32_t* rr_out, int64_t* cts_out, int64_t cap) {
  GUARD_BEGIN
  const int64_t m = std::min<int64_t>(cap, h->n_events);
  if (m > 0 && rr_out) h->d2h(rr_out, h->d_rr.p, 4 * (size_t)m);
  if (m > 0 && cts_out) h->d2h(cts_out, h->d_cts.p, 8 * (size_t)m);
  h->sync();
  return HGE_OK;
  GUARD_END(h)
}

int hge_consensus_timestamp_sources(hge_engine* h, const int32_t* ids, int64_t n, int32_t* src_out) {
  if (!h || n < 0 || (n > 0 && (!ids || !src_out))) return HGE_ERR_ARG;
  GUARD_BEGIN
  if (n == 0) return HGE_OK;
  for (int64_t i = 0; i < n; i++)
    if (ids[i] < 0 || ids[i] >= h->n_events) throw EngineError(HGE_ERR_ARG, "hge_consensus_timestamp_sources: unknown id");
  h->s_src.need((size_t)n * 2);
  h->h2d(h->s_src.p, ids, 4 * (size_t)n);
  hipLaunchKernelGGL(k_cts_source, dim3((unsigned)div_up(n, 4)), dim3(256), 0, h->st, h->tables(),
                     (const int32_t*)h->s_src.p, (int)n, (const int32_t*)h->d_rr.p, (const int64_t*)h->d_cts.p,
                     h->s_src.p + n);
  const hipError_t le = hipGetLastError();
  if (le != hipSuccess) throw EngineError(HGE_ERR_DEVICE, std::string("launch k_cts_source: ") + hipGetErrorString(le));
  h->readback(src_out, h->s_src.p + n, (size_t)n);
  return HGE_OK;
  GUARD_END(h)
}

int32_t hge_fame_table(hge_engine* h, int32_t rounds, int8_t* fame_out) {
  if (!h) return HGE_ERR_ARG;
  GUARD_BEGIN
  const int R = std::min<int>(std::max(rounds, 0), std::min(h->R, h->Rcap));
  if (R == 0 || !fame_out) return 0;
  const size_t n = (size_t)R * h->N;
  std::vector<int32_t> w(n);
  std::vector<uint8_t> f(n);
  h->d2h(w.data(), h->d_W.p, 4 * n);
  h->d2h(f.data(), h->d_fame.p, n);
  h->sync();
  for (size_t i = 0; i < n; i++)
    fame_out[i] = (w[i] >= 0 && w[i] < h->n_divided) ? (int8_t)f[i] : (int8_t)-1;
  return R;
  GUARD_END(h)
}

int32_t hge_parent_round(hge_engine* h, int32_t x) {
  if (x < 0 || x >= h->n_events) return -1;
  const int32_t sp = h->h_sp[x], op = h->h_op[x];
  if (sp < 0 && op < 0) return 0;
  if (sp < 0 || op < 0) return 0;
  const int32_t a = hge_round_of(h, sp), b = hge_round_of(h, op);
  return std::max(a, b);
}

int32_t hge_round_inc(hge_engine* h, int32_t x) {
  if (x < 0 || x >= h->n_events) return 0;
  const int32_t pr = hge_parent_round(h, x);
  if (pr < 0 || hge_rounds(h) < pr + 1) return 0;
  try {
    h->coords();
    if (pr >= h->Rcap) return 0;
    std::vector<int32_t> w(h->N);
    h->readback(w.data(), h->d_W.p + (size_t)pr * h->N, h->N);
    int c = 0;
    for (int i = 0; i < h->N; i++)
      if (w[i] >= 0 && w[i] < h->n_events) c += hge_strongly_see(h, x, w[i]);
    return c >= h->SM ? 1 : 0;
  } catch (EngineError& e) {
    h->err = e.msg;
    return 0;
  }
}

int hge_round_diff(hge_engine* h, int32_t x, int32_t y, int32_t* out) {
  if (x < 0 || x >= h->n_events || y < 0 || y >= h->n_events || !out) return HGE_ERR_ARG;
  const int32_t a = hge_round_of(h, x), b = hge_round_of(h, y);
  if (a < 0 || b < 0) return HGE_ERR_INTERNAL;
  *out = a - b;
  return HGE_OK;
}

int hge_set_round(hge_engine* h, int32_t round, const int32_t* ids, const uint8_t* witness,
                  const uint8_t* fame, int32_t n) {
  GUARD_BEGIN
  if (round < 0 || n < 0 || (n > 0 && !ids)) return HGE_ERR_ARG;
  h->coords();
  h->ensure_rcap((int64_t)round + 1);
  for (int32_t i = 0; i < n; i++) {
    const int32_t x = ids[i];
    if (x < 0 || x >= h->n_events) return HGE_ERR_ARG;
    if (witness && !witness[i]) continue;
    const size_t slot = (size_t)round * h->N + h->h_creator[x];
    h->h2d(h->d_W.p + slot, &ids[i], 4);
    const uint8_t f = fame ? fame[i] : 0;
    h->h2d(h->d_fame.p + slot, &f, 1);
    h->sync();
  }
  h->R_set = std::max(h->R_set, round + 1);
  return HGE_OK;
  GUARD_END(h)
}

int hge_set_profiling(hge_engine* h, int on) {
  h->prof_on = on != 0;
  return HGE_OK;
}

int hge_reset_kernel_stats(hge_engine* h) {
  h->prof_names.clear();
  h->prof_ms.clear();
  h->prof_cnt.clear();
  return HGE_OK;
}

int hge_kernel_stats(hge_engine* h, int k, char* name, int namecap, double* total_ms,
                     int64_t* launches) {
  const int n = (int)h->prof_names.size();
  if (k < 0 || k >= n) return n;
  if (name && namecap > 0) {
    snprintf(name, namecap, "%s", h->prof_names[k].c_str());
  }
  if (total_ms) *total_ms = h->prof_ms[k];
  if (launches) *launches = h->prof_cnt[k];
  return n;
}

int32_t hge_coordinate_sweeps(hge_engine* h) { return h ? h->n_sweeps : -1; }

int64_t hge_host_syncs(hge_engine* h) { return h ? h->n_syncs : -1; }

int hge_stage_times(hge_engine* h, float* ms_out, int cap) {
  int n = std::min(cap, 7);
  for (int i = 0; i < n; i++) ms_out[i] = h->stage_ms[i];
  return n;
}

int64_t hge_frontier_fallbacks(hge_engine* h) {
  if (!h) return HGE_ERR_ARG;
  return h->n_frontier_fallbacks;
}

}
```

### babble_amd/csrc/hge_rounds_direct.hip

```cpp
#include <hip/hip_runtime.h>
#include <stdint.h>

namespace hge {

#ifdef HGE_DIR_STAMPS
constexpr bool kDirStamps = true;
#else
constexpr bool kDirStamps = false;
#endif
constexpr int DIR_MAXP = 16;
constexpr int DIR_CH = 32;

template <int BS, int NPOW>
struct DirGeo {
  static constexpr int W = BS >= 1024 ? 64 : 32;
  static constexpr int TPM = BS / NPOW;
  static constexpr int CPT = NPOW / TPM;
  static constexpr int CW = CPT / 2;
  static constexpr int VW = (CW % 4 == 0) ? 4 : 2;
  static constexpr int PS = CW + VW;
  static constexpr int RS = TPM * PS;
  static constexpr int WIN_INTS = W * NPOW;
  static constexpr int PREF = (DIR_CH * NPOW / 4 + BS - 1) / BS;
  static constexpr int MBW = NPOW / 2;
  static constexpr int MVW = (CW % 4 == 0) ? 4 : 2;
};

template <int BS, int NPOW>
struct DirLDS {
  int sP[256];
  uint32_t sLA[DirGeo<BS, NPOW>::W * DirGeo<BS, NPOW>::RS] __attribute__((aligned(16)));
  int sCnt[DIR_MAXP];
  int sCntW[DIR_MAXP][BS / 64] __attribute__((aligned(16)));
  int sHist[DirGeo<BS, NPOW>::W / 2];
  uint32_t sBits[8];
  int sFlag[2];
  int s_stamp;
  uint64_t sdbg[2];
};

__device__ __forceinline__ uint32_t dir_pack_la(int a, int b) {
  return (uint32_t)(a + 2) | ((uint32_t)(b + 2) << 16);
}
__device__ __forceinline__ uint32_t dir_pack_fd(int a, int b) {
  const uint32_t lo = a == INF32 ? 0xFFFFu : (uint32_t)(a + 1);
  const uint32_t hi = b == INF32 ? 0xFFFFu : (uint32_t)(b + 1);
  return lo | (hi << 16);
}

template <int BS, int NPOW>
__device__ __forceinline__ void dir_fetch(const Tables& t, int c, int p0, int nr, int lenc,
                                          uint2 (&v)[DirGeo<BS, NPOW>::PREF]) {
  using G = DirGeo<BS, NPOW>;
  const int N = t.N;
  nr = min(nr, DIR_CH);
  const int have = (p0 == INF32 || nr <= 0) ? 0 : max(0, min(nr, lenc - p0));
  if (have == 0) return;
  const uint32_t* base = t.LA16 + ((size_t)c * t.ccap + p0) * (size_t)t.NW2;
  const int qmax = have * N / 4 - 1;
#pragma unroll
  for (int m = 0; m < G::PREF; m++) {
    const int q = min((int)threadIdx.x + m * BS, qmax);
    v[m] = *(const uint2*)(base + 2 * (size_t)q);
  }
}

template <int BS, int NPOW>
__device__ __forceinline__ void dir_store(const Tables& t, DirLDS<BS, NPOW>& L, int p0, int nr, int lenc,
                                          uint2 (&v)[DirGeo<BS, NPOW>::PREF]) {
  using G = DirGeo<BS, NPOW>;
  const int N = t.N;
  if (p0 == INF32 || nr <= 0) return;
  nr = min(nr, DIR_CH);
  const int have = max(0, min(nr, lenc - p0));
#pragma unroll
  for (int m = 0; m < G::PREF; m++) {
    const int q = threadIdx.x + m * BS;
    const int row = (4 * q) / N;
    if (row >= nr) continue;
    const bool hv = row < have;
    const int col = 4 * q - row * N;
    const int part = col / G::CPT, w = (col - part * G::CPT) / 2;
    const int slot = (p0 + row) & (DirGeo<BS, NPOW>::W - 1);
    uint2* dst = (uint2*)(L.sLA + slot * G::RS + part * G::PS + w);
    *dst = hv ? make_uint2(v[m].x + 0x00010001u, v[m].y + 0x00010001u) : make_uint2(0u, 0u);
  }
}

template <int BS, int NPOW>
__device__ __forceinline__ void dir_load(const Tables& t, DirLDS<BS, NPOW>& L, int c, int p0, int nr, int lenc,
                                         uint2 (&v)[DirGeo<BS, NPOW>::PREF]) {
  if (p0 == INF32) return;
  for (int q = 0; q < nr; q += DIR_CH) {
    dir_fetch<BS, NPOW>(t, c, p0 + q, nr - q, lenc, v);
    dir_store<BS, NPOW>(t, L, p0 + q, nr - q, lenc, v);
  }
}

template <int BS, int NPOW>
__device__ __forceinline__ void dir_members_fd(const Tables& t, int d, int part, int Pd,
                                               uint32_t (&mw)[DirGeo<BS, NPOW>::CW]) {
  using G = DirGeo<BS, NPOW>;
  const int N = t.N;
  const int c0 = part * G::CPT;
  const bool act = d < N && Pd != INF32;
  if (t.FD16) {
    const uint16_t* row = t.FD16 + rowoff(t, act ? d : 0, act ? Pd : 0);
#pragma unroll
    for (int k = 0; k < G::CW / 2; k++) {
      uint2 a = *(const uint2*)(row + min(c0 + 4 * k, N - 4));
      if (!act || c0 + 4 * k >= N) a = make_uint2(~0u, ~0u);
      mw[2 * k] = a.x;
      mw[2 * k + 1] = a.y;
    }
    return;
  }
  const int32_t* row = t.FD + rowoff(t, act ? d : 0, act ? Pd : 0);
#pragma unroll
  for (int k = 0; k < G::CW / 2; k++) {
    int4 a = *(const int4*)(row + min(c0 + 4 * k, N - 4));
    if (!act || c0 + 4 * k >= N) a = make_int4(INF32, INF32, INF32, INF32);
    mw[2 * k] = dir_pack_fd(a.x, a.y);
    mw[2 * k + 1] = dir_pack_fd(a.z, a.w);
  }
}

template <int BS, int NPOW>
__device__ __forceinline__ void dir_members_mb(const uint32_t* mb, uint32_t (&mw)[DirGeo<BS, NPOW>::CW]) {
  using G = DirGeo<BS, NPOW>;
  constexpr int MVW = G::MVW;
  const __amdgpu_buffer_rsrc_t rs =
      __builtin_amdgcn_make_buffer_rsrc((void*)mb, 0, BS * G::CW * 4, 0x00020000);
#pragma unroll
  for (int k = 0; k < G::CW / MVW; k++) {
    const int off = (k * BS + (int)threadIdx.x) * MVW * 4;
    if constexpr (MVW == 4) {
      typedef uint32_t u32x4 __attribute__((ext_vector_type(4)));
      const u32x4 x = __builtin_amdgcn_raw_buffer_load_b128(rs, off, 0, 16);
      mw[4 * k] = x.x;
      mw[4 * k + 1] = x.y;
      mw[4 * k + 2] = x.z;
      mw[4 * k + 3] = x.w;
    } else {
      typedef uint32_t u32x2 __attribute__((ext_vector_type(2)));
      const u32x2 x = __builtin_amdgcn_raw_buffer_load_b64(rs, off, 0, 16);
      mw[2 * k] = x.x;
      mw[2 * k + 1] = x.y;
    }
  }
}

template <int BS, int NPOW>
__device__ __forceinline__ void dir_stage_member(const Tables& t, uint32_t* mb, int c, int p) {
  using G = DirGeo<BS, NPOW>;
  constexpr int MVW = G::MVW;
  const int lane = threadIdx.x;
  const int N = t.N;
  if (4 * lane < NPOW) {
    unsigned long long x;
    if (t.FD16) {
      uint2 a = make_uint2(~0u, ~0u);
      if (p != INF32 && 4 * lane < N) a = *(const uint2*)(t.FD16 + rowoff(t, c, p) + 4 * lane);
      x = (unsigned long long)a.x | ((unsigned long long)a.y << 32);
    } else {
      int4 a = make_int4(INF32, INF32, INF32, INF32);
      if (p != INF32 && 4 * lane < N) a = *(const int4*)(t.FD + rowoff(t, c, p) + 4 * lane);
      x = (unsigned long long)dir_pack_fd(a.x, a.y) | ((unsigned long long)dir_pack_fd(a.z, a.w) << 32);
    }
    const int w = 2 * lane, part = w / G::CW, wp = w - part * G::CW;
    const int k = wp / MVW, sub = wp - k * MVW;
    const size_t word = ((size_t)k * BS + (size_t)c * G::TPM + part) * MVW + sub;
    __hip_atomic_store((gu64_t*)(mb + word), x, __ATOMIC_RELAXED, __HIP_MEMORY_SCOPE_AGENT);
  }
}

template <int BS, int NPOW>
__device__ __forceinline__ int dir_count(const DirLDS<BS, NPOW>& L, int p, int part,
                                         const uint32_t (&mw)[DirGeo<BS, NPOW>::CW]) {
  using G = DirGeo<BS, NPOW>;
  const uint32_t* src = L.sLA + (p & (DirGeo<BS, NPOW>::W - 1)) * G::RS + part * G::PS;
  uint32_t acc0 = 0, acc1 = 0;
  const uint32_t ones = 0x00010001u;
  static_assert(G::CW % 2 == 0, "member slices are whole word pairs");
  static_assert(G::CW % G::VW == 0, "LDS reads cover whole slices");
#pragma unroll
  for (int k0 = 0; k0 < G::CW; k0 += G::VW) {
    uint32_t la[G::VW];
    if constexpr (G::VW == 4) {
      const uint4 q = *(const uint4*)(src + k0);
      la[0] = q.x;
      la[1] = q.y;
      la[2] = q.z;
      la[3] = q.w;
    } else {
      const uint2 q = *(const uint2*)(src + k0);
      la[0] = q.x;
      la[1] = q.y;
    }
#pragma unroll
    for (int k = 0; k < G::VW; k += 2) {
      uint32_t d0, d1;
      asm("v_pk_sub_u16 %0, %4, %6 clamp\n\t"
          "v_pk_sub_u16 %1, %5, %7 clamp\n\t"
          "v_pk_min_u16 %0, %0, %8\n\t"
          "v_pk_min_u16 %1, %1, %8\n\t"
          "v_pk_add_u16 %2, %2, %0\n\t"
          "v_pk_add_u16 %3, %3, %1"
          : "=&v"(d0), "=&v"(d1), "+v"(acc0), "+v"(acc1)
          : "v"(la[k]), "v"(la[k + 1]), "v"(mw[k0 + k]), "v"(mw[k0 + k + 1]), "v"(ones));
    }
  }
  int cnt = (int)(acc0 & 0xFFFFu) + (int)(acc0 >> 16) + (int)(acc1 & 0xFFFFu) + (int)(acc1 >> 16);
  if constexpr (G::TPM > 1) cnt += __builtin_amdgcn_mov_dpp(cnt, 0xB1, 0xF, 0xF, false);
  if constexpr (G::TPM > 2) cnt += __builtin_amdgcn_mov_dpp(cnt, 0x4E, 0xF, 0xF, false);
  if constexpr (G::TPM > 4) cnt += __builtin_amdgcn_mov_dpp(cnt, 0x141, 0xF, 0xF, false);
  if constexpr (G::TPM > 8) cnt += __builtin_amdgcn_mov_dpp(cnt, 0x140, 0xF, 0xF, false);
  static_assert(G::TPM <= 16, "a member's lanes lie in one DPP row");
  return cnt;
}

template <int BS, int NPOW>
__device__ __forceinline__ int dir_probe(const Tables& t, DirLDS<BS, NPOW>& L, int p, int part, int slot,
                                         const uint32_t (&mw)[DirGeo<BS, NPOW>::CW], bool& pass) {
  const bool st = kDirStamps && L.s_stamp && threadIdx.x == 0;
  const uint64_t t0 = st ? stamp() : 0;
  const int cnt = dir_count<BS, NPOW>(L, p, part, mw);
  pass = cnt >= t.SM;
  const uint64_t t1 = st ? stamp() : 0;
  const uint64_t b = __ballot(part == 0 && pass);
  if ((threadIdx.x & 63) == 0) L.sCntW[slot][threadIdx.x >> 6] = (int)__builtin_popcountll(b);
  __syncthreads();
  int r = 0;
#pragma unroll
  for (int w = 0; w < BS / 64; w += 4) {
    const int4 q = *(const int4*)&L.sCntW[slot][w];
    r += q.x + q.y + q.z + q.w;
  }
  if (st) {
    L.sdbg[0] += t1 - t0;
    L.sdbg[1] += stamp() - t1;
  }
  return r;
}

template <int BS, int NPOW>
__device__ int dir_probe_search(const Tables& t, int c, int lenc, DirLDS<BS, NPOW>& L, int part,
                                const uint32_t (&mw)[DirGeo<BS, NPOW>::CW], int& slot,
                                uint2 (&pv)[DirGeo<BS, NPOW>::PREF], int& lo, bool& pb, int a) {
  constexpr int W = DirGeo<BS, NPOW>::W;
  const int SM = t.SM;
  for (;;) {
    const int last = min(W, lenc - lo) - 1;
    if (a <= last) {
      bool ps;
      int b = last;
      if (dir_probe<BS, NPOW>(t, L, lo + b, part, slot++, mw, ps) >= SM) {
        pb = ps;
        while (a < b) {
          const int mid = (a + b) >> 1;
          if (dir_probe<BS, NPOW>(t, L, lo + mid, part, slot++, mw, ps) >= SM) {
            b = mid;
            pb = ps;
          } else {
            a = mid + 1;
          }
        }
        return lo + a;
      }
    }
    if (lo + W >= lenc) return INF32;
    lo += W;
    __syncthreads();
    dir_load<BS, NPOW>(t, L, c, lo, W, lenc, pv);
    if (threadIdx.x < DIR_MAXP) L.sCnt[threadIdx.x] = 0;
    slot = 0;
    __syncthreads();
    a = 0;
  }
}

template <int BS, int NPOW>
__device__ int dir_select(const Tables& t, int c, int lenc, DirLDS<BS, NPOW>& L, int d, int part,
                          const uint32_t (&mw)[DirGeo<BS, NPOW>::CW], int& slot,
                          uint2 (&pv)[DirGeo<BS, NPOW>::PREF], int& lo, bool& pb) {
  constexpr int H = DirGeo<BS, NPOW>::W / 2;
  constexpr int STEPS = H == 32 ? 5 : H == 16 ? 4 : 3;
  static_assert((1 << STEPS) == H, "window half is a power of two");
  const int SM = t.SM;
  if (lo == INF32 || lo >= lenc) return INF32;
  const int e = min(H - 1, lenc - lo - 1);
  const bool st = kDirStamps && L.s_stamp && threadIdx.x == 0;
  const uint64_t t0 = st ? stamp() : 0;
  int a = 0, b = e;
#pragma unroll
  for (int s = 0; s < STEPS; s++) {
    const int mid = (a + b) >> 1;
    if (dir_count<BS, NPOW>(L, lo + mid, part, mw) >= SM) b = mid;
    else a = mid + 1;
  }
  if (part == 0 && d < t.N) atomicAdd(&L.sHist[a], 1);
  uint64_t t1 = 0;
  if (st) {
    asm volatile("s_waitcnt lgkmcnt(0)" ::: "memory");
    t1 = stamp();
  }
  __syncthreads();
  if (st) {
    L.sdbg[0] += t1 - t0;
    L.sdbg[1] += stamp() - t1;
  }
  const int lane = threadIdx.x & 63;
  int v = lane < H ? L.sHist[lane] : 0;
  HGE_DPP_SCAN(v, dpp_add, 0);
  const uint64_t ge = __ballot(lane < H && v >= SM);
  const int ks = ge ? (int)__builtin_ctzll(ge) : H;
  if (ks < e) {
    pb = a <= ks;
    return lo + ks;
  }
  return dir_probe_search<BS, NPOW>(t, c, lenc, L, part, mw, slot, pv, lo, pb, e);
}

template <int BS, int NPOW>
__global__ void __launch_bounds__(BS, 4) k_rounds_direct(Tables t, const int32_t* olen, const int32_t* len,
                                                      int32_t* rstate, int rlo, const int32_t* rlo_dev,
                                                      int Rprev, uint64_t* gran,
                                                      int32_t* err, uint64_t* ssc, uint32_t* mbuf,
                                                      uint64_t* dbg, const int32_t* start, int32_t* hist,
                                                      int hmax, const int32_t* stopcut, int extra, int stall_ep) {
  using G = DirGeo<BS, NPOW>;
  if (rlo_dev) {
    rlo = *rlo_dev;
    if (rlo == INF32) return;
  }
  uint64_t st_t = 0, st_acc[9] = {0, 0, 0, 0, 0, 0, 0, 0, 0};
  const bool stamping = kDirStamps && dbg && blockIdx.x == 0 && threadIdx.x == 0;
#define DSTAMP(k)                  \
  if (stamping) {                  \
    const uint64_t now_ = stamp(); \
    st_acc[(k)] += now_ - st_t;    \
    st_t = now_;                   \
  }
#define DSTAMP_START                \
  if (stamping) st_t = stamp();
  __shared__ DirLDS<BS, NPOW> L;
  const int N = t.N, NW = t.NW;
  const int c = blockIdx.x, tid = threadIdx.x;
  const int d = tid / G::TPM, part = tid - d * G::TPM;
  const int lenc = len[c];
  gu64_t* gr[2] = {(gu64_t*)gran, (gu64_t*)(gran + N)};
  uint32_t* mbp[2] = {mbuf, mbuf + (size_t)NPOW * G::MBW};
  if (tid < N) {
    int P;
    if (hist) {
      P = start[tid];
      if (c == 0) hist[tid] = P;
    } else {
      P = t.C[(size_t)rlo * N + tid];
      if (rlo == 0 && olen[tid] == 0 && len[tid] > 0) P = 0;
      if (c == 0 && rlo == 0 && olen[tid] == 0 && len[tid] > 0) t.C[tid] = 0;
    }
    L.sP[tid] = P;
  }
  if (tid == 0) {
    L.s_stamp = stamping ? 1 : 0;
    L.sdbg[0] = L.sdbg[1] = 0;
  }
  __syncthreads();
  const int rcap = hist ? hmax : t.Rcap;
  int extra_left = -1;
  uint2 pv[G::PREF];
  int lo = L.sP[c];
  dir_load<BS, NPOW>(t, L, c, lo, DirGeo<BS, NPOW>::W, lenc, pv);
  int f0 = INF32, fn = 0;
  uint32_t mw[G::CW];
  dir_members_fd<BS, NPOW>(t, d, part, d < N ? L.sP[d] : INF32, mw);
  for (int r = rlo;; r++) {
    if (r + 1 >= rcap) {
      if (c == 0 && tid == 0) {
        rstate[1] = 1;
        if (hist) rstate[0] = r + 1;
      }
      break;
    }
    DSTAMP_START
    if (d >= N) {
#pragma unroll
      for (int k = 0; k < G::CW; k++) mw[k] = 0xFFFFFFFFu;
    }
    if (tid < DIR_MAXP) L.sCnt[tid] = 0;
    if (tid < 8) L.sBits[tid] = 0;
    if (tid < DirGeo<BS, NPOW>::W / 2) L.sHist[tid] = 0;
    if (tid == 0) L.sFlag[(r + 1) & 1] = 0;
    __syncthreads();
    DSTAMP(0);
    const int Pc = L.sP[c];
    const int cur = (r + 1 < Rprev) ? t.C[(size_t)(r + 1) * N + c] : INF32;
    int slot = 0;
    int nxt = INF32;
    bool pb = false, have_bits = false;
    if (Pc != INF32) {
      if (cur != INF32) {
        nxt = cur;
      } else {
        const int s = dir_select<BS, NPOW>(t, c, lenc, L, d, part, mw, slot, pv, lo, pb);
        nxt = s < lenc ? s : INF32;
        have_bits = nxt != INF32;
      }
    }
    DSTAMP(1);
    if (stamping) st_acc[6] += slot;
    const bool stall = stall_ep > 0 && r - rlo + 1 == stall_ep;
    if (tid < 64 && !(stall && c == 0)) {
      dir_stage_member<BS, NPOW>(t, mbp[(r + 1) & 1], c, nxt);
      asm volatile("s_waitcnt vmcnt(0)" ::: "memory");
      if (tid == 0) {
        if (hist) hist[(size_t)(r + 1) * N + c] = nxt;
        else if (nxt != INF32 && cur == INF32) t.C[(size_t)(r + 1) * N + c] = nxt;
        const uint64_t g = ((uint64_t)(uint32_t)(r - rlo + 1) << 32) | (uint32_t)nxt;
        __hip_atomic_store(gr[(r + 1) & 1] + c, (unsigned long long)g, __ATOMIC_RELAXED,
                           __HIP_MEMORY_SCOPE_AGENT);
      }
    }
    if (nxt != INF32) {
      if (!have_bits) {
        if (nxt < lo || nxt >= lo + DirGeo<BS, NPOW>::W) {
          __syncthreads();
          lo = nxt;
          dir_load<BS, NPOW>(t, L, c, lo, DirGeo<BS, NPOW>::W, lenc, pv);
          __syncthreads();
        }
        pb = dir_count<BS, NPOW>(L, nxt, part, mw) >= t.SM;
      }
      if (part == 0 && d < N && pb) atomicOr(&L.sBits[d >> 5], 1u << (d & 31));
      __syncthreads();
      if (tid < NW)
        ssc[((size_t)(r + 1) * N + c) * NW + tid] =
            (uint64_t)L.sBits[2 * tid] | ((uint64_t)L.sBits[2 * tid + 1] << 32);
    }
    DSTAMP(2);
    if (nxt == INF32) {
      f0 = INF32;
      fn = 0;
    } else {
      f0 = (lo != INF32 && nxt < lo + DirGeo<BS, NPOW>::W) ? lo + DirGeo<BS, NPOW>::W : nxt;
      fn = nxt + DirGeo<BS, NPOW>::W - f0;
    }
    lo = nxt;
    dir_fetch<BS, NPOW>(t, c, f0, fn, lenc, pv);
    dir_store<BS, NPOW>(t, L, f0, fn, lenc, pv);
    if (fn > DIR_CH) {
      for (int q = DIR_CH; q < fn; q += DIR_CH) {
        dir_fetch<BS, NPOW>(t, c, f0 + q, fn - q, lenc, pv);
        dir_store<BS, NPOW>(t, L, f0 + q, fn - q, lenc, pv);
      }
    }
    asm volatile("s_waitcnt vmcnt(0)" ::: "memory");
    DSTAMP(3);
    {
      const unsigned ep = (unsigned)(r - rlo + 1);
      const gu64_t* g = gr[(r + 1) & 1];
      unsigned spins = 0;
      bool fail = false;
      int P = INF32;
      for (;;) {
        bool ok = true;
        if (d < N) {
          const unsigned long long x = __hip_atomic_load(g + d, __ATOMIC_RELAXED, __HIP_MEMORY_SCOPE_AGENT);
          ok = (unsigned)(x >> 32) == ep;
          P = (int)(uint32_t)x;
        }
        if (__all(ok)) break;
        if (stall || ++spins > (1u << 21)) {
          fail = true;
          break;
        }
        __builtin_amdgcn_s_sleep(1);
      }
      __builtin_amdgcn_fence(__ATOMIC_ACQUIRE, "wavefront");
      if (part == 0 && d < N) L.sP[d] = P;
      const bool any = __ballot(d < N && P != INF32) != 0;
      const bool notpast = stopcut && __ballot(part == 0 && d < N && P < stopcut[d]) != 0;
      if ((threadIdx.x & 63) == 0 && (any || notpast || fail))
        atomicOr(&L.sFlag[(r + 1) & 1], (any ? 1 : 0) | (notpast ? 2 : 0) | (fail ? 4 : 0));
      if (fail && (threadIdx.x & 63) == 0) {
        atomicOr(err, 1);
        atomicOr(rstate + 1, 4);
      }
      if (!fail) dir_members_mb<BS, NPOW>(mbp[(r + 1) & 1], mw);
    }
    __syncthreads();
    DSTAMP(4);
    const int fl = L.sFlag[(r + 1) & 1];
    const int stop = (fl & 4) ? 2 : ((fl & 1) ? 0 : 1);
    if (stop) {
      if (stop == 1 && c == 0 && tid == 0) rstate[0] = hist ? r + 2 : max(rstate[0], r + 1);
      break;
    }
    if (stopcut) {
      if (extra_left < 0 && !(fl & 2)) extra_left = extra;
      if (extra_left >= 0 && extra_left-- == 0) {
        if (c == 0 && tid == 0) {
          rstate[0] = r + 2;
          rstate[1] = 2;
        }
        break;
      }
    }
  }
  if (stamping) {
    for (int q = 0; q < 9; q++) dbg[q] += st_acc[q];
    dbg[9] += L.sdbg[0];
    dbg[10] += L.sdbg[1];
  }
#undef DSTAMP
#undef DSTAMP_START
}

template __global__ void k_rounds_direct<1024, 64>(Tables, const int32_t*, const int32_t*, int32_t*, int, const int32_t*, int,
    uint64_t*, int32_t*, uint64_t*, uint32_t*, uint64_t*, const int32_t*, int32_t*, int, const int32_t*, int, int);
template __global__ void k_rounds_direct<1024, 128>(Tables, const int32_t*, const int32_t*, int32_t*, int, const int32_t*, int,
    uint64_t*, int32_t*, uint64_t*, uint32_t*, uint64_t*, const int32_t*, int32_t*, int, const int32_t*, int, int);
template __global__ void k_rounds_direct<1024, 256>(Tables, const int32_t*, const int32_t*, int32_t*, int, const int32_t*, int,
    uint64_t*, int32_t*, uint64_t*, uint32_t*, uint64_t*, const int32_t*, int32_t*, int, const int32_t*, int, int);

}
```

### babble_amd/engine.py

```python
import ctypes
import os

import numpy as np

_ROOT = os.path.dirname(os.path.dirname(os.path.abspath(__file__)))
LIB_PATH = os.environ.get("HGE_LIB", os.path.join(_ROOT, "build", "libhge.so"))

HGE_NONE = -1
HGE_UNKNOWN = -2

ERRORS = {
    -1: "Could not find fake creator id",
    -2: "Self-parent not known",
    -3: "Self-parent has different creator",
    -4: "Other-parent not known",
    -5: "Self-parent not last known event by creator",
    -6: "Event index does not match the creator's chain position",
    -7: "Chain capacity exceeded",
    -11: "too late",
    -12: "not found",
}
HGE_ERR_CAPACITY = -7
HGE_ERR_TOO_LATE = -11
HGE_ERR_NOT_FOUND = -12
HGE_ERR_SIGNATURE = -13
HGE_ERR_SPLIT = -14

EXCHANGE_FN = ctypes.CFUNCTYPE(ctypes.c_int, ctypes.c_void_p, ctypes.c_int32, ctypes.c_int64,
                               ctypes.POINTER(ctypes.c_void_p))


class HgeEvent(ctypes.Structure):
    _fields_ = [
        ("creator", ctypes.c_int32),
        ("index", ctypes.c_int32),
        ("self_parent", ctypes.c_int32),
        ("other_parent", ctypes.c_int32),
        ("timestamp_ns", ctypes.c_int64),
        ("s", ctypes.c_uint8 * 32),
        ("hash", ctypes.c_uint8 * 32),
        ("n_tx", ctypes.c_int32),
        ("reserved", ctypes.c_int32),
    ]


EVENT_DTYPE = np.dtype([
    ("creator", "<i4"), ("index", "<i4"), ("self_parent", "<i4"), ("other_parent", "<i4"),
    ("timestamp_ns", "<i8"), ("s", "u1", (32,)), ("hash", "u1", (32,)), ("n_tx", "<i4"),
    ("reserved", "<i4"),
])
assert EVENT_DTYPE.itemsize == ctypes.sizeof(HgeEvent)

EXPORTS = [
    "hge_create", "hge_destroy", "hge_last_error", "hge_reset", "hge_insert_events",
    "hge_divide_rounds", "hge_decide_fame", "hge_decide_round_received", "hge_find_order",
    "hge_run_consensus", "hge_replay", "hge_replay_prepare", "hge_replay_run",
    "hge_replay_fetch", "hge_replay_order", "hge_event_count", "hge_participants", "hge_rounds",
    "hge_last_consensus_round", "hge_last_committed_round_events",
    "hge_consensus_transactions", "hge_consensus_count", "hge_consensus_events",
    "hge_undetermined", "hge_known", "hge_round_of", "hge_is_witness", "hge_round_witness",
    "hge_fame", "hge_round_events", "hge_round_received", "hge_consensus_timestamp",
    "hge_consensus_timestamp_sources",
    "hge_ancestor", "hge_self_ancestor", "hge_see", "hge_strongly_see",
    "hge_oldest_self_ancestor_to_see", "hge_coordinates", "hge_coordinate_sweeps", "hge_host_syncs", "hge_frontier_fallbacks",
    "hge_stage_times",
    "hge_set_profiling", "hge_reset_kernel_stats", "hge_kernel_stats",
    "hge_consensus_log", "hge_event_rounds", "hge_event_received", "hge_set_cache_size",
    "hge_cache_size", "hge_participant_events", "hge_participant_event", "hge_last_from",
    "hge_diff", "hge_wire_info", "hge_read_wire_parents", "hge_parent_round", "hge_round_inc",
    "hge_round_diff", "hge_set_round", "hge_round_event_ids", "hge_split_begin", "hge_frontier_guess",
    "hge_frontier_walk", "hge_split_finish", "hge_frontier_rows", "hge_split_plan", "hge_split_exchange", "hge_split_run", "hge_split_emulate",
    "hge_verify_events", "hge_sha256_batch", "hge_ingest", "hge_fame_table",
    "hge_store_create", "hge_store_destroy", "hge_store_set_event", "hge_store_has_event",
    "hge_store_participant_events", "hge_store_participant_event", "hge_store_last_from",
    "hge_store_known", "hge_store_add_consensus_event", "hge_store_consensus_events",
    "hge_store_consensus_count", "hge_store_set_round", "hge_store_get_round", "hge_store_rounds",
    "hge_store_round_witnesses", "hge_store_round_events",
    "hge_batch_create", "hge_batch_destroy", "hge_batch_last_error", "hge_batch_add", "hge_batch_stage",
    "hge_batch_run", "hge_batch_graphs", "hge_batch_info", "hge_batch_results", "hge_batch_kernel_ms",
    "hge_batch_fallbacks",
    "hge_gob_encode_wire_events", "hge_gob_decode_wire_events", "hge_gob_encode_event_body",
]

_lib = None


class HgeError(RuntimeError):

    def __init__(self, code, msg, accepted=None):
        super().__init__(f"{msg} (hge status {code})")
        self.code = code
        self.accepted = accepted


def lib():
    global _lib
    if _lib is not None:
        return _lib
    if not os.path.exists(LIB_PATH):
        raise ImportError(f"HIP engine library not built: {LIB_PATH} (run __graft_entry__.build())")
    try:
        import torch
    except ImportError:
        pass
    L = ctypes.CDLL(LIB_PATH)
    vp, i32, i64 = ctypes.c_void_p, ctypes.c_int32, ctypes.c_int64
    P = ctypes.POINTER
    L.hge_create.argtypes = [i32, i64, i32, ctypes.c_uint32, P(vp)]
    L.hge_destroy.argtypes = [vp]
    L.hge_destroy.restype = None
    L.hge_last_error.argtypes = [vp]
    L.hge_last_error.restype = ctypes.c_char_p
    L.hge_reset.argtypes = [vp]
    L.hge_insert_events.argtypes = [vp, ctypes.c_void_p, i64, P(i32), P(i64)]
    for f in ("hge_divide_rounds", "hge_decide_fame", "hge_decide_round_received"):
        getattr(L, f).argtypes = [vp]
    for f in ("hge_find_order", "hge_run_consensus"):
        getattr(L, f).argtypes = [vp, P(i32), i64, P(i64)]
    L.hge_replay.argtypes = [vp, ctypes.c_void_p, i64, P(i64), i64, P(i32), P(i32), i64, P(i64),
                             P(i64)]
    L.hge_replay_prepare.argtypes = [vp, ctypes.c_void_p, i64, P(i64), i64, P(i32)]
    L.hge_replay_run.argtypes = [vp, P(i64)]
    L.hge_replay_fetch.argtypes = [vp, P(i32), i64, P(i64)]
    L.hge_replay_order.argtypes = [vp, P(P(i32)), P(i64)]
    for f in ("hge_event_count", "hge_consensus_transactions", "hge_consensus_count"):
        getattr(L, f).argtypes = [vp]
        getattr(L, f).restype = i64
    for f in ("hge_participants", "hge_rounds", "hge_last_consensus_round",
              "hge_last_committed_round_events"):
        getattr(L, f).argtypes = [vp]
        getattr(L, f).restype = i32
    for f in ("hge_consensus_events", "hge_undetermined"):
        getattr(L, f).argtypes = [vp, P(i32), i64]
        getattr(L, f).restype = i64
    L.hge_known.argtypes = [vp, P(i32)]
    for f in ("hge_round_of", "hge_is_witness", "hge_round_events", "hge_round_received"):
        getattr(L, f).argtypes = [vp, i32]
        getattr(L, f).restype = i32
    L.hge_consensus_timestamp.argtypes = [vp, i32]
    L.hge_consensus_timestamp.restype = i64
    for f in ("hge_round_witness", "hge_fame", "hge_ancestor", "hge_self_ancestor", "hge_see",
              "hge_strongly_see", "hge_oldest_self_ancestor_to_see"):
        getattr(L, f).argtypes = [vp, i32, i32]
        getattr(L, f).restype = i32
    L.hge_coordinates.argtypes = [vp, i32, P(i32), P(i32)]
    L.hge_stage_times.argtypes = [vp, P(ctypes.c_float), ctypes.c_int]
    L.hge_coordinate_sweeps.restype = ctypes.c_int32
    L.hge_coordinate_sweeps.argtypes = [vp]
    if hasattr(L, "hge_gob_encode_wire_events"):
        L.hge_gob_encode_wire_events.argtypes = [vp, i64, P(ctypes.c_uint8), P(i64), i32, P(ctypes.c_uint8), i64,
                                                 P(i64)]
        L.hge_gob_decode_wire_events.argtypes = [P(ctypes.c_uint8), i64, vp, i64, P(ctypes.c_uint8), i64, P(i64),
                                                 i64, P(i64), P(i64), P(i64)]
        L.hge_gob_encode_event_body.argtypes = [vp, P(ctypes.c_uint8), P(i64), P(ctypes.c_uint8), P(i64), i32,
                                                P(ctypes.c_uint8), i64, P(i64)]
    if hasattr(L, "hge_host_syncs"):
        L.hge_host_syncs.restype = i64
        L.hge_host_syncs.argtypes = [vp]
    L.hge_frontier_fallbacks.restype = i64
    L.hge_frontier_fallbacks.argtypes = [vp]
    L.hge_consensus_log.argtypes = [vp, i64, P(i32), i64]
    L.hge_consensus_log.restype = i64
    L.hge_event_rounds.argtypes = [vp, P(i32), P(ctypes.c_uint8), i64]
    L.hge_event_received.argtypes = [vp, P(i32), P(i64), i64]
    L.hge_consensus_timestamp_sources.argtypes = [vp, P(i32), i64, P(i32)]
    L.hge_fame_table.argtypes = [vp, i32, P(ctypes.c_int8)]
    L.hge_fame_table.restype = i32
    L.hge_set_cache_size.argtypes = [vp, i64]
    L.hge_cache_size.argtypes = [vp]
    L.hge_cache_size.restype = i64
    L.hge_participant_events.argtypes = [vp, i32, i64, P(i32), i64, P(i64)]
    L.hge_participant_event.argtypes = [vp, i32, i64]
    L.hge_participant_event.restype = i32
    L.hge_last_from.argtypes = [vp, i32]
    L.hge_last_from.restype = i32
    L.hge_diff.argtypes = [vp, P(i32), P(i32), i64, P(i64)]
    L.hge_wire_info.argtypes = [vp, i32, P(i32)]
    L.hge_read_wire_parents.argtypes = [vp, i32, i32, i32, i32, P(i32), P(i32)]
    L.hge_parent_round.argtypes = [vp, i32]
    L.hge_parent_round.restype = i32
    L.hge_round_inc.argtypes = [vp, i32]
    L.hge_round_inc.restype = i32
    L.hge_round_diff.argtypes = [vp, i32, i32, P(i32)]
    L.hge_set_round.argtypes = [vp, i32, P(i32), P(ctypes.c_uint8), P(ctypes.c_uint8), i32]
    if hasattr(L, "hge_round_event_ids"):
        L.hge_round_event_ids.argtypes = [vp, i32, P(i32), P(ctypes.c_uint8), i64, P(i64)]
    L.hge_split_begin.argtypes = [vp]
    L.hge_frontier_guess.argtypes = [vp, i32, i32, P(i32)]
    L.hge_frontier_walk.argtypes = [vp, P(i32), P(i32), i32, i32, P(i32), P(ctypes.c_uint64), P(i32), P(i32)]
    L.hge_split_finish.argtypes = [vp, P(i32), P(ctypes.c_uint64), i32, i32, P(i64)]
    L.hge_frontier_rows.argtypes = [vp, i32, i32, P(i32), P(ctypes.c_uint64)]
    if hasattr(L, "hge_split_run"):
        L.hge_split_plan.argtypes = [vp, i32, i32, P(i64), P(i32), P(i64)]
        L.hge_split_run.argtypes = [vp, P(i64)]
        L.hge_split_exchange.argtypes = [vp, EXCHANGE_FN, vp]
    if hasattr(L, "hge_split_emulate"):
        L.hge_split_emulate.argtypes = [vp, i32]
    u8p = P(ctypes.c_uint8)
    L.hge_verify_events.argtypes = [i64, u8p, P(i64), u8p, u8p, i32, u8p, P(i32)]
    L.hge_sha256_batch.argtypes = [i64, u8p, P(i64), i32, u8p]
    L.hge_ingest.argtypes = [vp, ctypes.c_void_p, i64, u8p, P(i64), u8p, u8p, i64, i32, P(i32), P(i64),
                             P(ctypes.c_double)]
    L.hge_set_profiling.argtypes = [vp, ctypes.c_int]
    L.hge_reset_kernel_stats.argtypes = [vp]
    L.hge_kernel_stats.argtypes = [vp, ctypes.c_int, ctypes.c_char_p, ctypes.c_int,
                                   P(ctypes.c_double), P(i64)]
    L.hge_batch_create.argtypes = [i32, i32, P(vp)]
    L.hge_batch_destroy.argtypes = [vp]
    L.hge_batch_destroy.restype = None
    L.hge_batch_last_error.argtypes = [vp]
    L.hge_batch_last_error.restype = ctypes.c_char_p
    L.hge_batch_add.argtypes = [vp, ctypes.c_void_p, i64, P(i64), i64, P(i32), P(i32)]
    L.hge_batch_stage.argtypes = [vp]
    L.hge_batch_run.argtypes = [vp, P(i64)]
    L.hge_batch_graphs.argtypes = [vp]
    L.hge_batch_graphs.restype = i32
    L.hge_batch_info.argtypes = [vp, i32, P(i64)]
    L.hge_batch_results.argtypes = [vp, i32, P(i32), P(i64), P(i32), P(ctypes.c_uint8), P(i32), P(i64),
                                    P(ctypes.c_int8), P(i32)]
    L.hge_batch_kernel_ms.argtypes = [vp, P(ctypes.c_float), i32]
    L.hge_batch_fallbacks.argtypes = [vp]
    L.hge_batch_fallbacks.restype = ctypes.c_int64
    _lib = L
    return L


def _p32(a):
    return a.ctypes.data_as(ctypes.POINTER(ctypes.c_int32))


def _p64(a):
    return a.ctypes.data_as(ctypes.POINTER(ctypes.c_int64))


def _pu8(a):
    return a.ctypes.data_as(ctypes.POINTER(ctypes.c_uint8))


def _flat(bodies):
    if isinstance(bodies, tuple):
        flat, off = bodies
        return np.ascontiguousarray(flat, np.uint8), np.ascontiguousarray(off, np.int64)
    off = np.zeros(len(bodies) + 1, np.int64)
    off[1:] = np.cumsum([len(b) for b in bodies])
    flat = np.frombuffer(b"".join(bodies), np.uint8) if off[-1] else np.zeros(1, np.uint8)
    return np.ascontiguousarray(flat), off


def verify_events(bodies, pubs, sigs, threads=0):
    flat, off = _flat(bodies)
    n = len(off) - 1
    pubs = np.ascontiguousarray(pubs, np.uint8).reshape(n, 65)
    sigs = np.ascontiguousarray(sigs, np.uint8).reshape(n, 64)
    ok = np.zeros(max(n, 1), np.int32)
    hashes = np.zeros((max(n, 1), 32), np.uint8)
    rc = lib().hge_verify_events(n, _pu8(flat), _p64(off), _pu8(pubs), _pu8(sigs), threads, _pu8(hashes), _p32(ok))
    if rc != 0:
        raise HgeError(rc, "hge_verify_events failed")
    return ok[:n].astype(bool), hashes[:n]


class GobTime(ctypes.Structure):
    _fields_ = [("unix_sec", ctypes.c_int64), ("nsec", ctypes.c_int32), ("offset_min", ctypes.c_int16),
                ("set", ctypes.c_int16)]


class WireEvent(ctypes.Structure):
    _fields_ = [("self_parent_index", ctypes.c_int64), ("other_parent_creator_id", ctypes.c_int64),
                ("other_parent_index", ctypes.c_int64), ("creator_id", ctypes.c_int64), ("index", ctypes.c_int64),
                ("timestamp", GobTime), ("r", ctypes.c_uint8 * 32), ("s", ctypes.c_uint8 * 32),
                ("r_set", ctypes.c_int32), ("s_set", ctypes.c_int32), ("tx_first", ctypes.c_int64),
                ("tx_count", ctypes.c_int32), ("pad", ctypes.c_int32)]


class GobBody(ctypes.Structure):
    _fields_ = [("tx_count", ctypes.c_int32), ("n_parents", ctypes.c_int32),
                ("creator", ctypes.POINTER(ctypes.c_uint8)), ("creator_len", ctypes.c_int64),
                ("timestamp", GobTime), ("index", ctypes.c_int64)]


WIRE_INT_FIELDS = ("self_parent_index", "other_parent_creator_id", "other_parent_index", "creator_id", "index")


def _gob_time(ts):
    if ts is None:
        return GobTime(0, 0, 0, 0)
    return GobTime(int(ts[0]), int(ts[1]), int(ts[2]), 1)


def gob_encode_wire_events(events, first_type_id=65):
    n = len(events)
    arr = (WireEvent * max(n, 1))()
    txs = []
    for k, e in enumerate(events):
        w = arr[k]
        for f in WIRE_INT_FIELDS:
            setattr(w, f, int(e.get(f, 0)))
        w.timestamp = _gob_time(e.get("timestamp"))
        for name in ("r", "s"):
            v = e.get(name)
            if v is not None:
                getattr(w, name)[:] = list(int(v).to_bytes(32, "big"))
                setattr(w, name + "_set", 1)
        w.tx_first = len(txs)
        w.tx_count = len(e.get("transactions", []))
        txs.extend(e.get("transactions", []))
    flat, off = _flat(txs)
    L = lib()
    nout = ctypes.c_int64()
    rc = L.hge_gob_encode_wire_events(arr, n, _pu8(flat), _p64(off), first_type_id, None, 0, ctypes.byref(nout))
    if rc != 0:
        raise HgeError(rc, "hge_gob_encode_wire_events failed")
    out = np.zeros(max(1, nout.value), np.uint8)
    rc = L.hge_gob_encode_wire_events(arr, n, _pu8(flat), _p64(off), first_type_id, _pu8(out), nout.value,
                                      ctypes.byref(nout))
    if rc != 0:
        raise HgeError(rc, "hge_gob_encode_wire_events failed")
    return out[:nout.value].tobytes()


def gob_decode_wire_events(buf):
    b = np.frombuffer(bytes(buf), np.uint8) if len(buf) else np.zeros(1, np.uint8)
    L = lib()
    ne, nt, nb = ctypes.c_int64(), ctypes.c_int64(), ctypes.c_int64()
    rc = L.hge_gob_decode_wire_events(_pu8(b), len(buf), None, 0, None, 0, None, 0, ctypes.byref(ne),
                                      ctypes.byref(nt), ctypes.byref(nb))
    if rc not in (0, -12):
        raise HgeError(rc, "not a gob stream of WireEvents")
    arr = (WireEvent * max(1, ne.value))()
    tx = np.zeros(max(1, nb.value), np.uint8)
    off = np.zeros(nt.value + 1, np.int64)
    rc = L.hge_gob_decode_wire_events(_pu8(b), len(buf), arr, ne.value, _pu8(tx), nb.value, _p64(off), len(off),
                                      ctypes.byref(ne), ctypes.byref(nt), ctypes.byref(nb))
    if rc != 0:
        raise HgeError(rc, "not a gob stream of WireEvents")
    out = []
    for k in range(ne.value):
        w = arr[k]
        e = {f: int(getattr(w, f)) for f in WIRE_INT_FIELDS}
        t = w.timestamp
        e["timestamp"] = (int(t.unix_sec), int(t.nsec), int(t.offset_min)) if t.set else None
        e["r"] = int.from_bytes(bytes(w.r), "big") if w.r_set else None
        e["s"] = int.from_bytes(bytes(w.s), "big") if w.s_set else None
        e["transactions"] = [tx[off[w.tx_first + j]:off[w.tx_first + j + 1]].tobytes() for j in range(w.tx_count)]
        out.append(e)
    return out


def gob_encode_event_body(transactions, parents, creator, timestamp, index, first_type_id=65):
    tflat, toff = _flat(list(transactions))
    pflat, poff = _flat([p.encode() for p in parents])
    cr = np.frombuffer(bytes(creator), np.uint8) if len(creator) else np.zeros(1, np.uint8)
    body = GobBody(len(transactions), len(parents), _pu8(cr), len(creator), _gob_time(timestamp), int(index))
    L = lib()
    nout = ctypes.c_int64()
    rc = L.hge_gob_encode_event_body(ctypes.byref(body), _pu8(tflat), _p64(toff), _pu8(pflat), _p64(poff),
                                     first_type_id, None, 0, ctypes.byref(nout))
    if rc != 0:
        raise HgeError(rc, "hge_gob_encode_event_body failed")
    out = np.zeros(max(1, nout.value), np.uint8)
    rc = L.hge_gob_encode_event_body(ctypes.byref(body), _pu8(tflat), _p64(toff), _pu8(pflat), _p64(poff),
                                     first_type_id, _pu8(out), nout.value, ctypes.byref(nout))
    if rc != 0:
        raise HgeError(rc, "hge_gob_encode_event_body failed")
    return out[:nout.value].tobytes()


def sha256_batch(data, threads=0):
    flat, off = _flat(data)
    n = len(off) - 1
    out = np.zeros((max(n, 1), 32), np.uint8)
    rc = lib().hge_sha256_batch(n, _pu8(flat), _p64(off), threads, _pu8(out))
    if rc != 0:
        raise HgeError(rc, "hge_sha256_batch failed")
    return out[:n]


def events_array(dag):
    E = len(dag["creator"])
    ev = np.zeros(E, EVENT_DTYPE)
    ev["creator"] = dag["creator"]
    ev["index"] = dag["index"]
    ev["self_parent"] = dag["sp"]
    ev["other_parent"] = dag["op"]
    ev["timestamp_ns"] = dag["ts"]
    ev["s"] = dag["S"]
    ev["hash"] = dag["hash"]
    ev["n_tx"] = dag.get("ntx", np.zeros(E, np.int32))
    return ev


class Engine:

    def __init__(self, n_participants, capacity_events=1 << 16, device=0):
        self.L = lib()
        h = ctypes.c_void_p()
        rc = self.L.hge_create(n_participants, capacity_events, device, 0, ctypes.byref(h))
        if rc != 0:
            raise HgeError(rc, "hge_create failed")
        self.h = h
        self.n = n_participants
        self._obuf = None

    def close(self):
        if getattr(self, "h", None):
            self.L.hge_destroy(self.h)
            self.h = None

    def __del__(self):
        try:
            self.close()
        except Exception:
            pass

    def _check(self, rc):
        if rc != 0:
            xe, self._xerr = getattr(self, "_xerr", None), None
            if xe is not None:
                raise HgeError(rc, self.L.hge_last_error(self.h).decode()) from xe
            raise HgeError(rc, self.L.hge_last_error(self.h).decode())
        return rc

    def insert_events(self, ev):
        ev = np.ascontiguousarray(ev, EVENT_DTYPE)
        status = np.zeros(len(ev), np.int32)
        acc = ctypes.c_int64()
        rc = self.L.hge_insert_events(self.h, ev.ctypes.data, len(ev), _p32(status), ctypes.byref(acc))
        if rc != 0:
            raise HgeError(rc, self.L.hge_last_error(self.h).decode(), accepted=status[:acc.value].copy())
        return status[:acc.value]

    def ingest(self, ev, bodies, keys, sigs, k, threads=0):
        ev = np.ascontiguousarray(ev, EVENT_DTYPE)
        flat, off = _flat(bodies)
        n = len(ev)
        assert len(off) == n + 1
        keys = np.ascontiguousarray(keys, np.uint8).reshape(self.n, 65)
        sigs = np.ascontiguousarray(sigs, np.uint8).reshape(n, 64)
        status = np.zeros(max(n, 1), np.int32)
        acc = ctypes.c_int64()
        tm = (ctypes.c_double * 3)()
        rc = self.L.hge_ingest(self.h, ev.ctypes.data, n, _pu8(flat), _p64(off), _pu8(keys), _pu8(sigs), int(k),
                               threads, _p32(status), ctypes.byref(acc), tm)
        if rc in (-8, -9, -10):
            raise HgeError(rc, self.L.hge_last_error(self.h).decode())
        return rc, status[:n], acc.value, {"verify_ms": tm[0], "device_ms": tm[1], "wall_ms": tm[2]}

    def insert(self, creator, index, sp, op, ts, S=b"\0" * 32, hash32=b"\1" * 32, ntx=0):
        ev = np.zeros(1, EVENT_DTYPE)
        ev["creator"], ev["index"], ev["self_parent"], ev["other_parent"] = creator, index, sp, op
        ev["timestamp_ns"] = ts
        ev["s"][0] = np.frombuffer(S, np.uint8)
        ev["hash"][0] = np.frombuffer(hash32, np.uint8)
        ev["n_tx"] = ntx
        return int(self.insert_events(ev)[0])

    def divide_rounds(self):
        self._check(self.L.hge_divide_rounds(self.h))

    def decide_fame(self):
        self._check(self.L.hge_decide_fame(self.h))

    def decide_round_received(self):
        self._check(self.L.hge_decide_round_received(self.h))

    def _order_call(self, fn):
        cap = max(1, int(self.L.hge_event_count(self.h)))
        if self._obuf is None or len(self._obuf) < cap:
            self._obuf = np.empty(max(cap, 2 * (0 if self._obuf is None else len(self._obuf))), np.int32)
        out = self._obuf
        n = ctypes.c_int64()
        self._check(fn(self.h, _p32(out), len(out), ctypes.byref(n)))
        return out[:n.value].copy()

    def find_order(self):
        return self._order_call(self.L.hge_find_order)

    def run_consensus(self):
        return self._order_call(self.L.hge_run_consensus)

    def replay(self, dag_or_events, call_points):
        ev = dag_or_events if isinstance(dag_or_events, np.ndarray) else events_array(dag_or_events)
        self.prepare(ev, call_points)
        self.run()
        return self.fetch()

    def prepare(self, ev, call_points):
        ev = np.ascontiguousarray(ev, EVENT_DTYPE)
        cp = np.ascontiguousarray(call_points, np.int64)
        self._status = np.zeros(len(ev), np.int32)
        self._ncalls = len(cp)
        self._calls = cp.copy()
        self._check(self.L.hge_replay_prepare(self.h, ev.ctypes.data, len(ev), _p64(cp), len(cp),
                                              _p32(self._status)))
        return self._status

    def run(self):
        n = ctypes.c_int64()
        self._check(self.L.hge_replay_run(self.h, ctypes.byref(n)))
        self._nordered = n.value
        return n.value

    def order_view(self):
        p = ctypes.POINTER(ctypes.c_int32)()
        n = ctypes.c_int64()
        self._check(self.L.hge_replay_order(self.h, ctypes.byref(p), ctypes.byref(n)))
        if n.value == 0:
            return np.zeros(0, np.int32)
        return np.ctypeslib.as_array(p, shape=(n.value,))

    def fetch(self):
        order = np.zeros(max(1, self._nordered), np.int32)
        counts = np.zeros(max(1, self._ncalls), np.int64)
        self._check(self.L.hge_replay_fetch(self.h, _p32(order), len(order), _p64(counts)))
        return self._status, order[:self._nordered], counts[:self._ncalls]

    def call_events(self):
        acc = np.cumsum(self._status >= 0)
        return acc[self._calls - 1].astype(np.int64)

    def split_plan(self, part, nparts, plan=None):
        if nparts <= 1 or plan is None:
            self._check(self.L.hge_split_plan(self.h, 0, 0, None, None, None))
            return
        evb = np.ascontiguousarray(plan["ev_bounds"], np.int64)
        cb = np.ascontiguousarray(plan["call_bounds"], np.int32)
        clo = np.ascontiguousarray(plan["cand_lo"], np.int64)
        self._check(self.L.hge_split_plan(self.h, part, nparts, _p64(evb), _p32(cb), _p64(clo)))

    def clear_exchange(self):
        self._xcb = None
        self._check(self.L.hge_split_exchange(self.h, ctypes.cast(None, EXCHANGE_FN), None))

    def split_emulate(self, on=True):
        self._check(self.L.hge_split_emulate(self.h, 1 if on else 0))

    def split_run(self):
        n = ctypes.c_int64()
        self._check(self.L.hge_split_run(self.h, ctypes.byref(n)))
        self._nordered = n.value
        return n.value

    def set_exchange(self, fn):
        def cb(_ctx, op, nbytes, bufp):
            try:
                r = fn(int(op), int(nbytes))
                if op == 0:
                    bufp[0] = r
                return 0
            except Exception as e:
                self._xerr = e
                return 1
        self._xcb = EXCHANGE_FN(cb)
        self._check(self.L.hge_split_exchange(self.h, self._xcb, None))

    def split_begin(self):
        self._check(self.L.hge_split_begin(self.h))

    def frontier_guess(self, part, nparts):
        out = np.zeros(self.n, np.int32)
        self._check(self.L.hge_frontier_guess(self.h, part, nparts, _p32(out)))
        return out

    def frontier_walk(self, start, stopcut=None, extra=0, hmax=None):
        nw = (self.n + 63) // 64
        if hmax is None:
            hmax = int(self.known().max()) + 2
        nr = ctypes.c_int32()
        nat = ctypes.c_int32()
        start = np.ascontiguousarray(start, np.int32)
        cut = None if stopcut is None else np.ascontiguousarray(stopcut, np.int32)
        self._check(self.L.hge_frontier_walk(self.h, _p32(start), None if cut is None else _p32(cut),
                                             extra, hmax, None, None, ctypes.byref(nr), ctypes.byref(nat)))
        n = nr.value
        rows = np.zeros((n, self.n), np.int32)
        ssc = np.zeros((n, self.n, nw), np.uint64)
        self._check(self.L.hge_frontier_rows(self.h, 0, n, _p32(rows),
                                             ssc.ctypes.data_as(ctypes.POINTER(ctypes.c_uint64))))
        return rows, ssc, bool(nat.value)

    def split_finish(self, rows, ssc, natural):
        rows = np.ascontiguousarray(rows, np.int32)
        ssc = np.ascontiguousarray(ssc, np.uint64)
        n = ctypes.c_int64()
        self._check(self.L.hge_split_finish(self.h, _p32(rows),
                                            ssc.ctypes.data_as(ctypes.POINTER(ctypes.c_uint64)),
                                            len(rows), 1 if natural else 0, ctypes.byref(n)))
        self._nordered = n.value
        return n.value

    def set_profiling(self, on=True):
        self.L.hge_set_profiling(self.h, 1 if on else 0)
        self.L.hge_reset_kernel_stats(self.h)

    def kernel_stats(self):
        out = {}
        n = self.L.hge_kernel_stats(self.h, -1, None, 0, None, None)
        buf = ctypes.create_string_buffer(128)
        for k in range(n):
            ms = ctypes.c_double()
            cnt = ctypes.c_int64()
            self.L.hge_kernel_stats(self.h, k, buf, 128, ctypes.byref(ms), ctypes.byref(cnt))
            out[buf.value.decode()] = (ms.value, cnt.value)
        return out

    def coordinate_sweeps(self):
        return self.L.hge_coordinate_sweeps(self.h)

    def host_syncs(self):
        return int(self.L.hge_host_syncs(self.h))

    def frontier_fallbacks(self):
        return int(self.L.hge_frontier_fallbacks(self.h))

    def stage_times(self):
        out = (ctypes.c_float * 7)()
        n = self.L.hge_stage_times(self.h, out, 7)
        return list(out)[:n]

    def event_count(self):
        return self.L.hge_event_count(self.h)

    def rounds(self):
        return self.L.hge_rounds(self.h)

    def last_consensus_round(self):
        r = self.L.hge_last_consensus_round(self.h)
        return None if r < 0 else r

    def last_committed_round_events(self):
        return self.L.hge_last_committed_round_events(self.h)

    def consensus_transactions(self):
        return self.L.hge_consensus_transactions(self.h)

    def consensus_events(self):
        m = self.L.hge_consensus_events(self.h, None, 0)
        out = np.zeros(max(1, m), np.int32)
        self.L.hge_consensus_events(self.h, _p32(out), m)
        return out[:m]

    def undetermined(self):
        m = self.L.hge_undetermined(self.h, None, 0)
        out = np.zeros(max(1, m), np.int32)
        self.L.hge_undetermined(self.h, _p32(out), m)
        return out[:m]

    def known(self):
        out = np.zeros(self.n, np.int32)
        self.L.hge_known(self.h, _p32(out))
        return out

    def round(self, x):
        return self.L.hge_round_of(self.h, x)

    def witness(self, x):
        return bool(self.L.hge_is_witness(self.h, x))

    def round_witness(self, r, creator):
        w = self.L.hge_round_witness(self.h, r, creator)
        return None if w < 0 else w

    def round_witnesses(self, r):
        return sorted(w for w in (self.round_witness(r, c) for c in range(self.n)) if w is not None)

    def fame(self, r, creator):
        return self.L.hge_fame(self.h, r, creator)

    def round_events(self, r):
        return self.L.hge_round_events(self.h, r)

    def round_received(self, x):
        r = self.L.hge_round_received(self.h, x)
        return None if r < 0 else r

    def consensus_timestamp(self, x):
        return self.L.hge_consensus_timestamp(self.h, x)

    def ancestor(self, x, y):
        return bool(self.L.hge_ancestor(self.h, x, y))

    def self_ancestor(self, x, y):
        return bool(self.L.hge_self_ancestor(self.h, x, y))

    def see(self, x, y):
        return bool(self.L.hge_see(self.h, x, y))

    def strongly_see(self, x, y):
        return bool(self.L.hge_strongly_see(self.h, x, y))

    def oldest_self_ancestor_to_see(self, x, y):
        r = self.L.hge_oldest_self_ancestor_to_see(self.h, x, y)
        return None if r < 0 else r

    def event_rounds(self):
        m = self.event_count()
        r = np.zeros(max(m, 1), np.int32)
        w = np.zeros(max(m, 1), np.uint8)
        self._check(self.L.hge_event_rounds(self.h, _p32(r), w.ctypes.data_as(ctypes.POINTER(ctypes.c_uint8)), m))
        return r[:m], w[:m].astype(bool)

    def event_received(self):
        m = self.event_count()
        rr = np.zeros(max(m, 1), np.int32)
        cts = np.zeros(max(m, 1), np.int64)
        self._check(self.L.hge_event_received(self.h, _p32(rr), _p64(cts), m))
        return rr[:m], cts[:m]

    def consensus_timestamp_sources(self, ids):
        ids = np.ascontiguousarray(ids, np.int32)
        out = np.zeros(max(len(ids), 1), np.int32)
        if len(ids):
            self._check(self.L.hge_consensus_timestamp_sources(self.h, _p32(ids), len(ids), _p32(out)))
        return out[:len(ids)]

    def round_event_ids(self, r):
        n = ctypes.c_int64()
        self._check(self.L.hge_round_event_ids(self.h, r, None, None, 0, ctypes.byref(n)))
        ids = np.zeros(max(1, n.value), np.int32)
        wit = np.zeros(max(1, n.value), np.uint8)
        self._check(self.L.hge_round_event_ids(self.h, r, _p32(ids), _pu8(wit), n.value, ctypes.byref(n)))
        return ids[:n.value], wit[:n.value].astype(bool)

    def fame_table(self):
        R = self.rounds()
        out = np.full((max(R, 1), self.n), -1, np.int8)
        got = self.L.hge_fame_table(self.h, R, out.ctypes.data_as(ctypes.POINTER(ctypes.c_int8)))
        if got < 0:
            raise HgeError(got, self.L.hge_last_error(self.h).decode())
        return out[:R]

    def consensus_log(self, start=0):
        m = self.L.hge_consensus_log(self.h, start, None, 0)
        out = np.zeros(max(m, 1), np.int32)
        self.L.hge_consensus_log(self.h, start, _p32(out), m)
        return out[:m]

    def set_cache_size(self, size):
        self._check(self.L.hge_set_cache_size(self.h, size))

    def participant_events(self, creator, skip):
        n = ctypes.c_int64()
        rc = self.L.hge_participant_events(self.h, creator, skip, None, 0, ctypes.byref(n))
        if rc != 0:
            raise HgeError(rc, self.L.hge_last_error(self.h).decode())
        out = np.zeros(max(n.value, 1), np.int32)
        self._check(self.L.hge_participant_events(self.h, creator, skip, _p32(out), n.value, ctypes.byref(n)))
        return out[:n.value]

    def participant_event(self, creator, index):
        r = self.L.hge_participant_event(self.h, creator, index)
        if r < 0:
            raise HgeError(r, ERRORS.get(r, "error"))
        return r

    def last_from(self, creator):
        r = self.L.hge_last_from(self.h, creator)
        if r < -1:
            raise HgeError(r, ERRORS.get(r, "error"))
        return None if r == -1 else r

    def diff(self, known):
        known = np.ascontiguousarray(known, np.int32)
        n = ctypes.c_int64()
        rc = self.L.hge_diff(self.h, _p32(known), None, 0, ctypes.byref(n))
        if rc != 0:
            raise HgeError(rc, self.L.hge_last_error(self.h).decode())
        out = np.zeros(max(n.value, 1), np.int32)
        self._check(self.L.hge_diff(self.h, _p32(known), _p32(out), n.value, ctypes.byref(n)))
        return out[:n.value]

    def wire_info(self, x):
        out = np.zeros(4, np.int32)
        self._check(self.L.hge_wire_info(self.h, x, _p32(out)))
        return tuple(int(v) for v in out)

    def read_wire_parents(self, creator_id, sp_index, op_creator_id, op_index):
        sp = ctypes.c_int32()
        op = ctypes.c_int32()
        rc = self.L.hge_read_wire_parents(self.h, creator_id, sp_index, op_creator_id, op_index,
                                          ctypes.byref(sp), ctypes.byref(op))
        if rc != 0:
            raise HgeError(rc, ERRORS.get(rc, "error"))
        return sp.value, op.value

    def parent_round(self, x):
        return self.L.hge_parent_round(self.h, x)

    def round_inc(self, x):
        return bool(self.L.hge_round_inc(self.h, x))

    def round_diff(self, x, y):
        out = ctypes.c_int32()
        self._check(self.L.hge_round_diff(self.h, x, y, ctypes.byref(out)))
        return out.value

    def set_round(self, r, entries):
        ids = np.array([e[0] for e in entries], np.int32)
        w = np.array([int(e[1]) for e in entries], np.uint8)
        f = np.array([e[2] for e in entries], np.uint8)
        u8 = ctypes.POINTER(ctypes.c_uint8)
        self._check(self.L.hge_set_round(self.h, r, _p32(ids), w.ctypes.data_as(u8),
                                         f.ctypes.data_as(u8), len(ids)))

    def coordinates(self, x):
        la = np.zeros(self.n, np.int32)
        fd = np.zeros(self.n, np.int32)
        self._check(self.L.hge_coordinates(self.h, x, _p32(la), _p32(fd)))
        return la, fd


class Batch:

    def __init__(self, n_participants, device=0):
        self.L = lib()
        h = ctypes.c_void_p()
        rc = self.L.hge_batch_create(n_participants, device, ctypes.byref(h))
        if rc != 0:
            raise HgeError(rc, "hge_batch_create failed")
        self.h = h
        self.n = n_participants
        self.status = []

    def close(self):
        if getattr(self, "h", None):
            self.L.hge_batch_destroy(self.h)
            self.h = None

    def __del__(self):
        try:
            self.close()
        except Exception:
            pass

    def _check(self, rc):
        if rc != 0:
            raise HgeError(rc, self.L.hge_batch_last_error(self.h).decode())

    def add(self, dag_or_events, call_points):
        ev = dag_or_events if isinstance(dag_or_events, np.ndarray) else events_array(dag_or_events)
        ev = np.ascontiguousarray(ev, EVENT_DTYPE)
        cp = np.ascontiguousarray(call_points, np.int64)
        st = np.zeros(max(len(ev), 1), np.int32)
        g = ctypes.c_int32()
        self._check(self.L.hge_batch_add(self.h, ev.ctypes.data, len(ev), _p64(cp), len(cp), _p32(st),
                                         ctypes.byref(g)))
        self.status.append(st[:len(ev)])
        return g.value

    def stage(self):
        self._check(self.L.hge_batch_stage(self.h))

    def run(self):
        m = ctypes.c_int64()
        self._check(self.L.hge_batch_run(self.h, ctypes.byref(m)))
        return m.value

    def graphs(self):
        return self.L.hge_batch_graphs(self.h)

    def info(self, g):
        a = np.zeros(8, np.int64)
        self._check(self.L.hge_batch_info(self.h, g, _p64(a)))
        keys = ("events", "calls", "rounds", "lcr", "lcre", "transactions", "ordered", "undetermined")
        return dict(zip(keys, a.tolist()))

    KERNELS = ("kb_coords", "kb_fd", "kb_fdrows", "kb_front", "kb_fame", "kb_fold", "kb_receive", "kb_order")

    def fallbacks(self):
        return int(self.L.hge_batch_fallbacks(self.h))

    def kernel_ms(self):
        a = (ctypes.c_float * 8)()
        n = self.L.hge_batch_kernel_ms(self.h, a, 8)
        if n < 0:
            self._check(n)
        return dict(zip(self.KERNELS, [float(a[k]) for k in range(n)]))

    def state(self, g):
        inf = self.info(g)
        E, K, R = inf["events"], inf["calls"], inf["rounds"]
        order = np.zeros(max(inf["ordered"], 1), np.int32)
        counts = np.zeros(max(K, 1), np.int64)
        rounds = np.zeros(max(E, 1), np.int32)
        wit = np.zeros(max(E, 1), np.uint8)
        rr = np.zeros(max(E, 1), np.int32)
        cts = np.zeros(max(E, 1), np.int64)
        fame = np.zeros((max(R, 1), self.n), np.int8)
        und = np.zeros(max(inf["undetermined"], 1), np.int32)
        self._check(self.L.hge_batch_results(self.h, g, _p32(order), _p64(counts), _p32(rounds),
                                             wit.ctypes.data_as(ctypes.POINTER(ctypes.c_uint8)), _p32(rr),
                                             _p64(cts), fame.ctypes.data_as(ctypes.POINTER(ctypes.c_int8)),
                                             _p32(und)))
        return dict(status=self.status[g], order=order[:inf["ordered"]], counts=counts[:K], rounds=rounds[:E],
                    witness=wit[:E].astype(bool), fame=fame[:R], rr=rr[:E], cts=cts[:E],
                    undetermined=und[:inf["undetermined"]],
                    scalars=np.array([R, inf["lcr"], inf["lcre"], inf["transactions"]], np.int64))
```

### include/hge.h

```cpp
#ifndef HGE_H
#define HGE_H

#include <stdint.h>

#ifdef __cplusplus
extern "C" {
#endif

typedef struct hge_engine hge_engine;

enum hge_status {
  HGE_OK = 0,
  HGE_ERR_CREATOR = -1,
  HGE_ERR_SELF_PARENT_UNKNOWN = -2,
  HGE_ERR_SELF_PARENT_CREATOR = -3,
  HGE_ERR_OTHER_PARENT_UNKNOWN = -4,
  HGE_ERR_SELF_PARENT_NOT_LAST = -5,
  HGE_ERR_INDEX = -6,
  HGE_ERR_CAPACITY = -7,
  HGE_ERR_ARG = -8,
  HGE_ERR_DEVICE = -9,
  HGE_ERR_INTERNAL = -10,
  HGE_ERR_TOO_LATE = -11,
  HGE_ERR_NOT_FOUND = -12,
  HGE_ERR_SIGNATURE = -13,
  HGE_ERR_SPLIT = -14
};

#define HGE_NONE (-1)
#define HGE_UNKNOWN (-2)

typedef struct hge_event {
  int32_t creator;
  int32_t index;
  int32_t self_parent;
  int32_t other_parent;
  int64_t timestamp_ns;
  uint8_t s[32];
  uint8_t hash[32];
  int32_t n_tx;
  int32_t reserved;
} hge_event;

int hge_create(int32_t n_participants, int64_t capacity_events, int32_t device,
               uint32_t flags, hge_engine** out);
void hge_destroy(hge_engine* h);
const char* hge_last_error(hge_engine* h);
int hge_reset(hge_engine* h);

int hge_insert_events(hge_engine* h, const hge_event* ev, int64_t n, int32_t* status_out,
                      int64_t* n_accepted);

int hge_verify_events(int64_t n, const uint8_t* bodies, const int64_t* body_off, const uint8_t* pubs,
                      const uint8_t* sigs, int32_t threads, uint8_t* body_hash_out, int32_t* ok_out);
int hge_sha256_batch(int64_t n, const uint8_t* data, const int64_t* off, int32_t threads, uint8_t* out);
int hge_ingest(hge_engine* h, const hge_event* ev, int64_t n, const uint8_t* bodies, const int64_t* body_off,
               const uint8_t* keys, const uint8_t* sigs, int64_t k, int32_t threads, int32_t* status_out,
               int64_t* n_accepted, double* times_out);

int hge_divide_rounds(hge_engine* h);
int hge_decide_fame(hge_engine* h);
int hge_decide_round_received(hge_engine* h);
int hge_find_order(hge_engine* h, int32_t* ids_out, int64_t cap, int64_t* n_out);
int hge_run_consensus(hge_engine* h, int32_t* ids_out, int64_t cap, int64_t* n_out);

int hge_replay(hge_engine* h, const hge_event* ev, int64_t n_sub, const int64_t* call_points,
               int64_t n_calls, int32_t* status_out, int32_t* order_out, int64_t cap,
               int64_t* n_ordered, int64_t* call_counts_out);
int hge_replay_prepare(hge_engine* h, const hge_event* ev, int64_t n_sub,
                       const int64_t* call_points, int64_t n_calls, int32_t* status_out);
int hge_replay_run(hge_engine* h, int64_t* n_ordered);
int hge_replay_fetch(hge_engine* h, int32_t* order_out, int64_t cap, int64_t* call_counts_out);
int hge_replay_order(hge_engine* h, const int32_t** ids, int64_t* n);

typedef struct hge_batch hge_batch;
int hge_batch_create(int32_t n_participants, int32_t device, hge_batch** out);
void hge_batch_destroy(hge_batch* b);
const char* hge_batch_last_error(hge_batch* b);
int hge_batch_add(hge_batch* b, const hge_event* ev, int64_t n_sub, const int64_t* call_points, int64_t n_calls,
                  int32_t* status_out, int32_t* graph_out);
int hge_batch_stage(hge_batch* b);
int hge_batch_run(hge_batch* b, int64_t* n_ordered);
int32_t hge_batch_graphs(hge_batch* b);
int hge_batch_info(hge_batch* b, int32_t g, int64_t* info);
int hge_batch_results(hge_batch* b, int32_t g, int32_t* order, int64_t* counts, int32_t* round, uint8_t* witness,
                      int32_t* rr, int64_t* cts, int8_t* fame, int32_t* undetermined);
int hge_batch_kernel_ms(hge_batch* b, float* ms, int32_t cap);
int64_t hge_batch_fallbacks(hge_batch* b);

typedef int (*hge_exchange_fn)(void* ctx, int32_t op, int64_t bytes_per_part, void** buf);
int hge_split_plan(hge_engine* h, int32_t part, int32_t nparts, const int64_t* ev_bounds,
                   const int32_t* call_bounds, const int64_t* cand_lo);
int hge_split_exchange(hge_engine* h, hge_exchange_fn fn, void* ctx);
int hge_split_run(hge_engine* h, int64_t* n_ordered);
int hge_split_emulate(hge_engine* h, int32_t on);

int hge_split_begin(hge_engine* h);
int hge_frontier_guess(hge_engine* h, int32_t part, int32_t nparts, int32_t* start_out);
int hge_frontier_walk(hge_engine* h, const int32_t* start, const int32_t* stopcut, int32_t extra,
                      int32_t hmax, int32_t* rows_out, uint64_t* ssc_out, int32_t* nrows,
                      int32_t* natural);
int hge_frontier_rows(hge_engine* h, int32_t from, int32_t n, int32_t* rows_out, uint64_t* ssc_out);
int hge_split_finish(hge_engine* h, const int32_t* rows, const uint64_t* ssc, int32_t nrows,
                     int32_t natural, int64_t* n_ordered);

int64_t hge_event_count(hge_engine* h);
int32_t hge_participants(hge_engine* h);
int32_t hge_rounds(hge_engine* h);
int32_t hge_last_consensus_round(hge_engine* h);
int32_t hge_last_committed_round_events(hge_engine* h);
int64_t hge_consensus_transactions(hge_engine* h);
int64_t hge_consensus_count(hge_engine* h);
int64_t hge_consensus_events(hge_engine* h, int32_t* ids_out, int64_t cap);
int64_t hge_consensus_log(hge_engine* h, int64_t from, int32_t* ids_out, int64_t cap);
int64_t hge_undetermined(hge_engine* h, int32_t* ids_out, int64_t cap);
int hge_known(hge_engine* h, int32_t* counts_out);
int32_t hge_round_of(hge_engine* h, int32_t id);
int32_t hge_is_witness(hge_engine* h, int32_t id);
int32_t hge_round_witness(hge_engine* h, int32_t round, int32_t creator);
int32_t hge_fame(hge_engine* h, int32_t round, int32_t creator);
int32_t hge_round_events(hge_engine* h, int32_t round);
int hge_round_event_ids(hge_engine* h, int32_t round, int32_t* ids_out, uint8_t* witness_out, int64_t cap,
                        int64_t* n_out);
int32_t hge_round_received(hge_engine* h, int32_t id);
int64_t hge_consensus_timestamp(hge_engine* h, int32_t id);
int hge_consensus_timestamp_sources(hge_engine* h, const int32_t* ids, int64_t n, int32_t* src_out);

int hge_event_rounds(hge_engine* h, int32_t* round_out, uint8_t* witness_out, int64_t cap);
int hge_event_received(hge_engine* h, int32_t* rr_out, int64_t* cts_out, int64_t cap);
int32_t hge_fame_table(hge_engine* h, int32_t rounds, int8_t* fame_out);

int hge_set_cache_size(hge_engine* h, int64_t size);
int64_t hge_cache_size(hge_engine* h);
int hge_participant_events(hge_engine* h, int32_t creator, int64_t skip, int32_t* ids_out,
                           int64_t cap, int64_t* n_out);
int32_t hge_participant_event(hge_engine* h, int32_t creator, int64_t index);
int32_t hge_last_from(hge_engine* h, int32_t creator);
int hge_diff(hge_engine* h, const int32_t* known, int32_t* ids_out, int64_t cap, int64_t* n_out);
int hge_wire_info(hge_engine* h, int32_t id, int32_t* out4);
int hge_read_wire_parents(hge_engine* h, int32_t creator_id, int32_t self_parent_index,
                          int32_t other_parent_creator_id, int32_t other_parent_index,
                          int32_t* sp_out, int32_t* op_out);

typedef struct hge_store hge_store;
int hge_store_create(int32_t n_participants, int64_t cache_size, hge_store** out);
void hge_store_destroy(hge_store* s);
int hge_store_set_event(hge_store* s, int64_t key, int32_t creator);
int32_t hge_store_has_event(hge_store* s, int64_t key);
int hge_store_participant_events(hge_store* s, int32_t creator, int64_t skip, int64_t* keys_out, int64_t cap,
                                 int64_t* n_out);
int hge_store_participant_event(hge_store* s, int32_t creator, int64_t index, int64_t* key_out);
int hge_store_last_from(hge_store* s, int32_t creator, int64_t* key_out, int32_t* found);
int hge_store_known(hge_store* s, int32_t* counts_out);
int hge_store_add_consensus_event(hge_store* s, int64_t key);
int64_t hge_store_consensus_events(hge_store* s, int64_t* keys_out, int64_t cap);
int64_t hge_store_consensus_count(hge_store* s);
int hge_store_set_round(hge_store* s, int32_t round, const int64_t* keys, const uint8_t* witness,
                        const uint8_t* famous, int32_t n);
int hge_store_get_round(hge_store* s, int32_t round, int64_t* keys_out, uint8_t* witness_out,
                        uint8_t* famous_out, int32_t cap, int32_t* n_out);
int32_t hge_store_rounds(hge_store* s);
int hge_store_round_witnesses(hge_store* s, int32_t round, int64_t* keys_out, int32_t cap, int32_t* n_out);
int32_t hge_store_round_events(hge_store* s, int32_t round);

int32_t hge_parent_round(hge_engine* h, int32_t x);
int32_t hge_round_inc(hge_engine* h, int32_t x);
int hge_round_diff(hge_engine* h, int32_t x, int32_t y, int32_t* out);
int hge_set_round(hge_engine* h, int32_t round, const int32_t* ids, const uint8_t* witness,
                  const uint8_t* fame, int32_t n);

int32_t hge_ancestor(hge_engine* h, int32_t x, int32_t y);
int32_t hge_self_ancestor(hge_engine* h, int32_t x, int32_t y);
int32_t hge_see(hge_engine* h, int32_t x, int32_t y);
int32_t hge_strongly_see(hge_engine* h, int32_t x, int32_t y);
int32_t hge_oldest_self_ancestor_to_see(hge_engine* h, int32_t x, int32_t y);
int hge_coordinates(hge_engine* h, int32_t id, int32_t* la_out, int32_t* fd_out);

typedef struct {
  int64_t unix_sec;
  int32_t nsec;
  int16_t offset_min;
  int16_t set;
} hge_gob_time;
typedef struct {
  int64_t self_parent_index, other_parent_creator_id, other_parent_index, creator_id, index;
  hge_gob_time timestamp;
  uint8_t r[32], s[32];
  int32_t r_set, s_set;
  int64_t tx_first;
  int32_t tx_count, pad;
} hge_wire_event;
typedef struct {
  int32_t tx_count, n_parents;
  const uint8_t* creator;
  int64_t creator_len;
  hge_gob_time timestamp;
  int64_t index;
} hge_gob_body;
int hge_gob_encode_wire_events(const hge_wire_event* ev, int64_t n, const uint8_t* tx, const int64_t* tx_off,
                               int32_t first_type_id, uint8_t* out, int64_t cap, int64_t* n_out);
int hge_gob_decode_wire_events(const uint8_t* buf, int64_t len, hge_wire_event* ev, int64_t cap_ev, uint8_t* tx,
                               int64_t cap_bytes, int64_t* tx_off, int64_t cap_tx, int64_t* n_ev, int64_t* n_tx,
                               int64_t* n_bytes);
int hge_gob_encode_event_body(const hge_gob_body* body, const uint8_t* tx, const int64_t* tx_off,
                              const uint8_t* parents, const int64_t* parent_off, int32_t first_type_id,
                              uint8_t* out, int64_t cap, int64_t* n_out);

int hge_stage_times(hge_engine* h, float* ms_out, int cap);
int32_t hge_coordinate_sweeps(hge_engine* h);
int64_t hge_host_syncs(hge_engine* h);
int64_t hge_frontier_fallbacks(hge_engine* h);
int hge_set_profiling(hge_engine* h, int on);
int hge_reset_kernel_stats(hge_engine* h);
int hge_kernel_stats(hge_engine* h, int k, char* name, int namecap, double* total_ms,
                     int64_t* launches);

#ifdef __cplusplus
}
#endif
#endif
```

Baseline: 198.2 million events/s.

## Add narrow 8-bit packed strongly-see counting path in direct rounds walk

Adds a narrowed representation for the direct-rounds binary-search selection. Window rows and member rows are encoded relative to a per-creator 16-bit base into saturated 8-bit lanes with guard bits, so the strongly-see comparison becomes a packed subtract-and-popcount over half as many words. An exact fallback path runs when bases exceed the 16-bit range or values saturate. This is meant to cut LDS traffic and ALU work in the count loop, at the cost of extra encode passes, more LDS, and per-block path counters written back with atomics.

Result: faster. 203.8 million events/s, median of 6 (+2.8%).

```diff
diff --git a/babble_amd/csrc/hge_engine.hip b/babble_amd/csrc/hge_engine.hip
--- a/babble_amd/csrc/hge_engine.hip
+++ b/babble_amd/csrc/hge_engine.hip
@@ -430,6 +430,7 @@
     s_cM.free_();
     s_cn.free_();
     s_mb.free_();
+    s_wpaths.free_();
     s_hist.free_();
     s_hstate.free_();
     s_hssc.free_();
@@ -1392,15 +1393,17 @@
     uint64_t* ssc = d_ssc.p;
     uint64_t* dbg = dbg_p();
     if (direct_rounds()) {
-      s_mb.need((size_t)npow() * npow());
-      uint32_t* mb = s_mb.p;
+      uint32_t* mb = walk_mb();
+      unsigned long long* paths = walk_paths();
+      unsigned long long* paths_next = s_wpaths.p + 2 * ((walk_seq + 1) & 1);
       const int32_t* nostart = nullptr;
       int32_t* nohist = nullptr;
       int hmax = 0, extra = 0;
       const char* hs = getenv("HGE_TEST_HANDOFF_STALL");
       int stall_ep = hs ? atoi(hs) : 0;
+      int force_exact = walk_force_exact();
       void* dargs[] = {&t, &olen, &len, &rstate, &rlo, &rlo_dev, &Rprev, &gran, &err, &ssc, &mb, &dbg,
-                       &nostart, &nohist, &hmax, &nostart, &extra, &stall_ep};
+                       &nostart, &nohist, &hmax, &nostart, &extra, &stall_ep, &force_exact, &paths, &paths_next};
       prof_begin("k_rounds_direct");
       HIPCHK(launch_resident(direct_fn(), dim3(N), dim3(1024), dargs));
       prof_end();
@@ -1415,6 +1418,24 @@
       h2d(err, &one, 4);
       h2d(rstate + 1, &down, 4);
     }
+  }
+  uint32_t* walk_mb() {
+    s_mb.need((size_t)npow() * npow());
+    return s_mb.p;
+  }
+  DBuf<unsigned long long> s_wpaths;
+  int walk_seq = 0;
+  unsigned long long* walk_paths() {
+    if (!s_wpaths.p) {
+      s_wpaths.need(4);
+      HIPCHK(hipMemset(s_wpaths.p, 0, 4 * sizeof(unsigned long long)));
+    }
+    walk_seq++;
+    return s_wpaths.p + 2 * (walk_seq & 1);
+  }
+  static int walk_force_exact() {
+    const char* e = getenv("HGE_TEST_DIR_EXACT");
+    return e && atoi(e) != 0 ? 1 : 0;
   }
   const void* direct_fn() const {
     return N <= 64 ? (const void*)k_rounds_direct<1024, 64>
@@ -3025,7 +3046,6 @@
   h->s_gran.need(2 * (size_t)N);
   HIPCHK(hipMemsetAsync(h->s_bar.p, 0, 8, h->st));
   HIPCHK(hipMemsetAsync(h->s_gran.p, 0, 16 * (size_t)N, h->st));
-  h->s_mb.need((size_t)h->npow() * h->npow());
   auto lk = h->frontier_lock();
   Tables t = h->tables();
   const int32_t* olen = h->cstep->olen;
@@ -3035,13 +3055,15 @@
   uint64_t* gran = h->s_gran.p;
   int32_t* err = h->s_bar.p + 1;
   uint64_t* ssc = h->s_hssc.p;
-  uint32_t* mb = h->s_mb.p;
+  uint32_t* mb = h->walk_mb();
+  unsigned long long* paths = h->walk_paths();
+  unsigned long long* paths_next = h->s_wpaths.p + 2 * ((h->walk_seq + 1) & 1);
   uint64_t* dbg = nullptr;
   const int32_t* st0 = h->s_hstate.p;
   int32_t* hist = h->s_hist.p;
-  int hm = hmax, ex = std::max(0, (int)extra), nostall = 0;
+  int hm = hmax, ex = std::max(0, (int)extra), nostall = 0, force_exact = hge_engine::walk_force_exact();
   void* args[] = {&t, &olen, &len, &rstate, &rlo, &rlo_dev, &Rprev, &gran, &err, &ssc, &mb, &dbg,
-                  &st0, &hist, &hm, &cut, &ex, &nostall};
+                  &st0, &hist, &hm, &cut, &ex, &nostall, &force_exact, &paths, &paths_next};
   h->prof_begin("k_rounds_direct_walk");
   HIPCHK(h->launch_resident(h->direct_fn(), dim3(N), dim3(1024), args));
   h->prof_end();
@@ -3587,6 +3609,19 @@
 
 int32_t hge_coordinate_sweeps(hge_engine* h) { return h ? h->n_sweeps : -1; }
 
+int hge_walk_select_paths(hge_engine* h, int64_t* narrow, int64_t* exact) {
+  GUARD_BEGIN
+  unsigned long long v[2] = {0, 0};
+  if (h->s_wpaths.p && h->walk_seq > 0) {
+    h->d2h(v, h->s_wpaths.p + 2 * (h->walk_seq & 1), 16);
+    h->sync();
+  }
+  if (narrow) *narrow = (int64_t)v[0];
+  if (exact) *exact = (int64_t)v[1];
+  return HGE_OK;
+  GUARD_END(h)
+}
+
 int64_t hge_host_syncs(hge_engine* h) { return h ? h->n_syncs : -1; }
 
 int hge_stage_times(hge_engine* h, float* ms_out, int cap) {
diff --git a/babble_amd/csrc/hge_narrow.h b/babble_amd/csrc/hge_narrow.h
--- /dev/null
+++ b/babble_amd/csrc/hge_narrow.h
@@ -0,0 +1,78 @@
+#pragma once
+
+#include <stdint.h>
+
+#if defined(__HIPCC__) || defined(__CUDACC__)
+#define HGE_NAR_HD __host__ __device__ __forceinline__
+#else
+#define HGE_NAR_HD inline
+#endif
+
+namespace hge_narrow {
+
+constexpr uint32_t kNarGuard = 0x80808080u;
+constexpr uint32_t kNarAMax = 126;
+constexpr uint32_t kNarBaseNone = 0xFFFEu;
+constexpr int32_t kNarBaseMax = 65400;
+constexpr int32_t kNarInf32 = 0x7FFFFFFF;
+
+HGE_NAR_HD uint32_t nar_base16(int32_t P) { return P == kNarInf32 ? kNarBaseNone : (uint32_t)P; }
+HGE_NAR_HD bool nar_base_too_large(int32_t P) { return P != kNarInf32 && P > kNarBaseMax; }
+
+HGE_NAR_HD uint32_t nar_sub_sat2(uint32_t x, uint32_t c) {
+#if defined(__HIP_DEVICE_COMPILE__)
+  typedef unsigned short u16x2 __attribute__((ext_vector_type(2)));
+  const u16x2 r = __builtin_elementwise_sub_sat(__builtin_bit_cast(u16x2, x), __builtin_bit_cast(u16x2, c));
+  return __builtin_bit_cast(uint32_t, r);
+#else
+  const uint32_t xl = x & 0xFFFFu, cl = c & 0xFFFFu, xh = x >> 16, ch = c >> 16;
+  return (xl > cl ? xl - cl : 0u) | ((xh > ch ? xh - ch : 0u) << 16);
+#endif
+}
+HGE_NAR_HD uint32_t nar_min2(uint32_t x, uint32_t y) {
+#if defined(__HIP_DEVICE_COMPILE__)
+  typedef unsigned short u16x2 __attribute__((ext_vector_type(2)));
+  const u16x2 r = __builtin_elementwise_min(__builtin_bit_cast(u16x2, x), __builtin_bit_cast(u16x2, y));
+  return __builtin_bit_cast(uint32_t, r);
+#else
+  const uint32_t xl = x & 0xFFFFu, yl = y & 0xFFFFu, xh = x >> 16, yh = y >> 16;
+  return (xl < yl ? xl : yl) | ((xh < yh ? xh : yh) << 16);
+#endif
+}
+HGE_NAR_HD uint32_t nar_max2(uint32_t x, uint32_t y) {
+#if defined(__HIP_DEVICE_COMPILE__)
+  typedef unsigned short u16x2 __attribute__((ext_vector_type(2)));
+  const u16x2 r = __builtin_elementwise_max(__builtin_bit_cast(u16x2, x), __builtin_bit_cast(u16x2, y));
+  return __builtin_bit_cast(uint32_t, r);
+#else
+  const uint32_t xl = x & 0xFFFFu, yl = y & 0xFFFFu, xh = x >> 16, yh = y >> 16;
+  return (xl > yl ? xl : yl) | ((xh > yh ? xh : yh) << 16);
+#endif
+}
+HGE_NAR_HD uint32_t nar_pack4(uint32_t x0, uint32_t x1) {
+#if defined(__HIP_DEVICE_COMPILE__)
+  return __builtin_amdgcn_perm(x1, x0, 0x06040200u);
+#else
+  return (x0 & 0xFFu) | ((x0 >> 8) & 0xFF00u) | ((x1 & 0xFFu) << 16) | ((x1 << 8) & 0xFF000000u);
+#endif
+}
+
+HGE_NAR_HD uint32_t nar_enc_window4(uint32_t la0, uint32_t la1, uint32_t c0, uint32_t c1, uint32_t& mx) {
+  const uint32_t cap = kNarAMax | (kNarAMax << 16);
+  const uint32_t x0 = nar_sub_sat2(la0, c0), x1 = nar_sub_sat2(la1, c1);
+  mx = nar_max2(mx, nar_max2(x0, x1));
+  return nar_pack4(nar_min2(x0, cap), nar_min2(x1, cap)) | kNarGuard;
+}
+HGE_NAR_HD bool nar_window_flag(uint32_t mx) { return (mx & 0xFFFFu) >= kNarAMax || (mx >> 16) >= kNarAMax; }
+
+HGE_NAR_HD uint32_t nar_enc_member4(uint32_t fd0, uint32_t fd1, uint32_t c0, uint32_t c1, uint32_t& mn) {
+  const uint32_t cap = kNarAMax | (kNarAMax << 16);
+  const uint32_t t0 = nar_sub_sat2(fd0, c0), t1 = nar_sub_sat2(fd1, c1);
+  mn = nar_min2(mn, nar_min2(t0, t1));
+  return nar_pack4(nar_min2(t0, cap), nar_min2(t1, cap)) + 0x01010101u;
+}
+HGE_NAR_HD bool nar_member_flag(uint32_t mn) { return (mn & 0xFFFFu) == 0 || (mn >> 16) == 0; }
+
+HGE_NAR_HD uint32_t nar_ge4(uint32_t aw, uint32_t bw) { return (aw - bw) & kNarGuard; }
+
+}
diff --git a/babble_amd/csrc/hge_rounds_direct.hip b/babble_amd/csrc/hge_rounds_direct.hip
--- a/babble_amd/csrc/hge_rounds_direct.hip
+++ b/babble_amd/csrc/hge_rounds_direct.hip
@@ -1,5 +1,17 @@
 #include <hip/hip_runtime.h>
 #include <stdint.h>
+
+#include "hge_narrow.h"
+
+#ifndef HGE_DIR_NARROW_64
+#define HGE_DIR_NARROW_64 1
+#endif
+#ifndef HGE_DIR_NARROW_128
+#define HGE_DIR_NARROW_128 1
+#endif
+#ifndef HGE_DIR_NARROW_256
+#define HGE_DIR_NARROW_256 1
+#endif
 
 namespace hge {
 
@@ -24,7 +36,21 @@
   static constexpr int PREF = (DIR_CH * NPOW / 4 + BS - 1) / BS;
   static constexpr int MBW = NPOW / 2;
   static constexpr int MVW = (CW % 4 == 0) ? 4 : 2;
+  static constexpr bool NARROW = NPOW <= 64 ? HGE_DIR_NARROW_64 != 0
+                               : NPOW <= 128 ? HGE_DIR_NARROW_128 != 0 : HGE_DIR_NARROW_256 != 0;
+  static constexpr int H = W / 2;
+  static constexpr int NCW = CW / 2;
+  static constexpr int NVW = (NCW % 4 == 0) ? 4 : (NCW % 2 == 0) ? 2 : 1;
+  static constexpr int NPS = NCW + NVW;
+  static constexpr int NRS = TPM * NPS;
+  static constexpr int NENC = (H * NPOW / 4 + BS - 1) / BS;
 };
+
+__device__ __forceinline__ int dir_tid() {
+  int x = threadIdx.x;
+  asm volatile("" : "+v"(x));
+  return x;
+}
 
 template <int BS, int NPOW>
 struct DirLDS {
@@ -34,6 +60,9 @@
   int sCntW[DIR_MAXP][BS / 64] __attribute__((aligned(16)));
   int sHist[DirGeo<BS, NPOW>::W / 2];
   uint32_t sBits[8];
+  uint32_t sB16[DirGeo<BS, NPOW>::NARROW ? DirGeo<BS, NPOW>::RS : 4] __attribute__((aligned(16)));
+  uint32_t sN[DirGeo<BS, NPOW>::NARROW ? DirGeo<BS, NPOW>::H * DirGeo<BS, NPOW>::NRS : 4] __attribute__((aligned(16)));
+  int sEx[2];
   int sFlag[2];
   int s_stamp;
   uint64_t sdbg[2];
@@ -58,9 +87,10 @@
   if (have == 0) return;
   const uint32_t* base = t.LA16 + ((size_t)c * t.ccap + p0) * (size_t)t.NW2;
   const int qmax = have * N / 4 - 1;
+  const int tx = dir_tid();
 #pragma unroll
   for (int m = 0; m < G::PREF; m++) {
-    const int q = min((int)threadIdx.x + m * BS, qmax);
+    const int q = min(tx + m * BS, qmax);
     v[m] = *(const uint2*)(base + 2 * (size_t)q);
   }
 }
@@ -73,9 +103,10 @@
   if (p0 == INF32 || nr <= 0) return;
   nr = min(nr, DIR_CH);
   const int have = max(0, min(nr, lenc - p0));
+  const int tx = dir_tid();
 #pragma unroll
   for (int m = 0; m < G::PREF; m++) {
-    const int q = threadIdx.x + m * BS;
+    const int q = tx + m * BS;
     const int row = (4 * q) / N;
     if (row >= nr) continue;
     const bool hv = row < have;
@@ -131,9 +162,10 @@
   constexpr int MVW = G::MVW;
   const __amdgpu_buffer_rsrc_t rs =
       __builtin_amdgcn_make_buffer_rsrc((void*)mb, 0, BS * G::CW * 4, 0x00020000);
+  const int tx = dir_tid();
 #pragma unroll
   for (int k = 0; k < G::CW / MVW; k++) {
-    const int off = (k * BS + (int)threadIdx.x) * MVW * 4;
+    const int off = (k * BS + tx) * MVW * 4;
     if constexpr (MVW == 4) {
       typedef uint32_t u32x4 __attribute__((ext_vector_type(4)));
       const u32x4 x = __builtin_amdgcn_raw_buffer_load_b128(rs, off, 0, 16);
@@ -154,7 +186,8 @@
 __device__ __forceinline__ void dir_stage_member(const Tables& t, uint32_t* mb, int c, int p) {
   using G = DirGeo<BS, NPOW>;
   constexpr int MVW = G::MVW;
-  const int lane = threadIdx.x;
+  int lane = threadIdx.x;
+  asm volatile("" : "+v"(lane));
   const int N = t.N;
   if (4 * lane < NPOW) {
     unsigned long long x;
@@ -219,6 +252,120 @@
   return cnt;
 }
 
+
+template <int BS, int NPOW>
+__device__ __forceinline__ int dir_base_slot(int d) {
+  using G = DirGeo<BS, NPOW>;
+  const int w = d >> 1, part = w / G::CW;
+  return 2 * (part * G::PS + (w - part * G::CW)) + (d & 1);
+}
+
+template <int BS, int NPOW>
+__device__ __forceinline__ uint32_t dir_encode_window(const Tables& t, DirLDS<BS, NPOW>& L, int lo) {
+  using G = DirGeo<BS, NPOW>;
+  constexpr int GPR = NPOW / 4;
+  uint32_t mx = 0;
+  const int tx = dir_tid();
+#pragma unroll
+  for (int m = 0; m < G::NENC; m++) {
+    const int q = tx + m * BS;
+    if (q >= G::H * GPR) continue;
+    const int k = q / GPR, col = 4 * (q - k * GPR);
+    const int part = col / G::CPT, cp = col - part * G::CPT;
+    const int off = part * G::PS + cp / 2;
+    uint32_t word = hge_narrow::kNarGuard;
+    if (col < t.N) {
+      const uint2 la = *(const uint2*)(L.sLA + ((lo + k) & (G::W - 1)) * G::RS + off);
+      const uint2 cb = *(const uint2*)(L.sB16 + off);
+      word = hge_narrow::nar_enc_window4(la.x, la.y, cb.x, cb.y, mx);
+    }
+    L.sN[k * G::NRS + part * G::NPS + cp / 4] = word;
+  }
+  return mx;
+}
+
+template <int BS, int NPOW>
+__device__ __forceinline__ uint32_t dir_encode_members(const DirLDS<BS, NPOW>& L, int part,
+                                                       const uint32_t (&mw)[DirGeo<BS, NPOW>::CW],
+                                                       uint32_t (&nw)[DirGeo<BS, NPOW>::NCW]) {
+  using G = DirGeo<BS, NPOW>;
+  const uint32_t* src = L.sB16 + part * G::PS;
+  uint32_t mn = 0xFFFFFFFFu;
+#pragma unroll
+  for (int k0 = 0; k0 < G::CW; k0 += G::VW) {
+    uint32_t cb[G::VW];
+    if constexpr (G::VW == 4) {
+      const uint4 q = *(const uint4*)(src + k0);
+      cb[0] = q.x;
+      cb[1] = q.y;
+      cb[2] = q.z;
+      cb[3] = q.w;
+    } else {
+      const uint2 q = *(const uint2*)(src + k0);
+      cb[0] = q.x;
+      cb[1] = q.y;
+    }
+#pragma unroll
+    for (int k = 0; k < G::VW; k += 2)
+      nw[(k0 + k) / 2] = hge_narrow::nar_enc_member4(mw[k0 + k], mw[k0 + k + 1], cb[k], cb[k + 1], mn);
+  }
+  return mn;
+}
+
+template <int BS, int NPOW>
+__device__ __forceinline__ int dir_count_n(const DirLDS<BS, NPOW>& L, int k, int part,
+                                           const uint32_t (&nw)[DirGeo<BS, NPOW>::NCW]) {
+  using G = DirGeo<BS, NPOW>;
+  const uint32_t* src = L.sN + k * G::NRS + part * G::NPS;
+  uint32_t acc0 = 0, acc1 = 0;
+#pragma unroll
+  for (int k0 = 0; k0 < G::NCW; k0 += G::NVW) {
+    uint32_t a[G::NVW];
+    if constexpr (G::NVW == 4) {
+      const uint4 q = *(const uint4*)(src + k0);
+      a[0] = q.x;
+      a[1] = q.y;
+      a[2] = q.z;
+      a[3] = q.w;
+    } else if constexpr (G::NVW == 2) {
+      const uint2 q = *(const uint2*)(src + k0);
+      a[0] = q.x;
+      a[1] = q.y;
+    } else {
+      a[0] = src[k0];
+    }
+#pragma unroll
+    for (int j = 0; j < G::NVW; j++) {
+      const uint32_t ge = hge_narrow::nar_ge4(a[j], nw[k0 + j]);
+      if (j & 1) asm("v_bcnt_u32_b32 %0, %1, %0" : "+v"(acc1) : "v"(ge));
+      else asm("v_bcnt_u32_b32 %0, %1, %0" : "+v"(acc0) : "v"(ge));
+    }
+  }
+  int cnt = (int)(acc0 + acc1);
+  if constexpr (G::TPM > 1) cnt += __builtin_amdgcn_mov_dpp(cnt, 0xB1, 0xF, 0xF, false);
+  if constexpr (G::TPM > 2) cnt += __builtin_amdgcn_mov_dpp(cnt, 0x4E, 0xF, 0xF, false);
+  if constexpr (G::TPM > 4) cnt += __builtin_amdgcn_mov_dpp(cnt, 0x141, 0xF, 0xF, false);
+  if constexpr (G::TPM > 8) cnt += __builtin_amdgcn_mov_dpp(cnt, 0x140, 0xF, 0xF, false);
+  return cnt;
+}
+
+template <int BS, int NPOW>
+__device__ __forceinline__ void dir_members_reload(const Tables& t, const DirLDS<BS, NPOW>& L, const uint32_t* mb,
+                                                   bool first, int d, int part,
+                                                   uint32_t (&mw)[DirGeo<BS, NPOW>::CW]) {
+  using G = DirGeo<BS, NPOW>;
+  if (first) {
+    asm volatile("" : "+v"(d), "+v"(part));
+    dir_members_fd<BS, NPOW>(t, d, part, d < t.N ? L.sP[d] : INF32, mw);
+  } else {
+    dir_members_mb<BS, NPOW>(mb, mw);
+  }
+  if (d >= t.N) {
+#pragma unroll
+    for (int k = 0; k < G::CW; k++) mw[k] = 0xFFFFFFFFu;
+  }
+}
+
 template <int BS, int NPOW>
 __device__ __forceinline__ int dir_probe(const Tables& t, DirLDS<BS, NPOW>& L, int p, int part, int slot,
                                          const uint32_t (&mw)[DirGeo<BS, NPOW>::CW], bool& pass) {
@@ -239,6 +386,22 @@
   if (st) {
     L.sdbg[0] += t1 - t0;
     L.sdbg[1] += stamp() - t1;
+  }
+  return r;
+}
+
+template <int BS, int NPOW>
+__device__ __forceinline__ int dir_probe_n(const Tables& t, DirLDS<BS, NPOW>& L, int k, int part, int slot,
+                                           const uint32_t (&nw)[DirGeo<BS, NPOW>::NCW], bool& pass) {
+  pass = dir_count_n<BS, NPOW>(L, k, part, nw) >= t.SM;
+  const uint64_t b = __ballot(part == 0 && pass);
+  if ((threadIdx.x & 63) == 0) L.sCntW[slot][threadIdx.x >> 6] = (int)__builtin_popcountll(b);
+  __syncthreads();
+  int r = 0;
+#pragma unroll
+  for (int w = 0; w < BS / 64; w += 4) {
+    const int4 q = *(const int4*)&L.sCntW[slot][w];
+    r += q.x + q.y + q.z + q.w;
   }
   return r;
 }
@@ -279,10 +442,10 @@
   }
 }
 
-template <int BS, int NPOW>
+template <int BS, int NPOW, bool NAR>
 __device__ int dir_select(const Tables& t, int c, int lenc, DirLDS<BS, NPOW>& L, int d, int part,
-                          const uint32_t (&mw)[DirGeo<BS, NPOW>::CW], int& slot,
-                          uint2 (&pv)[DirGeo<BS, NPOW>::PREF], int& lo, bool& pb) {
+                          const uint32_t (&mw)[NAR ? DirGeo<BS, NPOW>::NCW : DirGeo<BS, NPOW>::CW], int& slot,
+                          uint2 (&pv)[DirGeo<BS, NPOW>::PREF], int& lo, bool& pb, const uint32_t* mb, bool first) {
   constexpr int H = DirGeo<BS, NPOW>::W / 2;
   constexpr int STEPS = H == 32 ? 5 : H == 16 ? 4 : 3;
   static_assert((1 << STEPS) == H, "window half is a power of two");
@@ -295,7 +458,10 @@
 #pragma unroll
   for (int s = 0; s < STEPS; s++) {
     const int mid = (a + b) >> 1;
-    if (dir_count<BS, NPOW>(L, lo + mid, part, mw) >= SM) b = mid;
+    int cnt;
+    if constexpr (NAR) cnt = dir_count_n<BS, NPOW>(L, mid, part, mw);
+    else cnt = dir_count<BS, NPOW>(L, lo + mid, part, mw);
+    if (cnt >= SM) b = mid;
     else a = mid + 1;
   }
   if (part == 0 && d < t.N) atomicAdd(&L.sHist[a], 1);
@@ -309,7 +475,8 @@
     L.sdbg[0] += t1 - t0;
     L.sdbg[1] += stamp() - t1;
   }
-  const int lane = threadIdx.x & 63;
+  int lane = threadIdx.x & 63;
+  asm volatile("" : "+v"(lane));
   int v = lane < H ? L.sHist[lane] : 0;
   HGE_DPP_SCAN(v, dpp_add, 0);
   const uint64_t ge = __ballot(lane < H && v >= SM);
@@ -318,7 +485,21 @@
     pb = a <= ks;
     return lo + ks;
   }
-  return dir_probe_search<BS, NPOW>(t, c, lenc, L, part, mw, slot, pv, lo, pb, e);
+  if constexpr (NAR) {
+    if (lenc - lo <= H) {
+      bool ps;
+      if (dir_probe_n<BS, NPOW>(t, L, e, part, slot++, mw, ps) >= SM) {
+        pb = ps;
+        return lo + e;
+      }
+      return INF32;
+    }
+    uint32_t mx[DirGeo<BS, NPOW>::CW];
+    dir_members_reload<BS, NPOW>(t, L, mb, first, d, part, mx);
+    return dir_probe_search<BS, NPOW>(t, c, lenc, L, part, mx, slot, pv, lo, pb, e);
+  } else {
+    return dir_probe_search<BS, NPOW>(t, c, lenc, L, part, mw, slot, pv, lo, pb, e);
+  }
 }
 
 template <int BS, int NPOW>
@@ -327,11 +508,16 @@
                                                       int Rprev, uint64_t* gran,
                                                       int32_t* err, uint64_t* ssc, uint32_t* mbuf,
                                                       uint64_t* dbg, const int32_t* start, int32_t* hist,
-                                                      int hmax, const int32_t* stopcut, int extra, int stall_ep) {
+                                                      int hmax, const int32_t* stopcut, int extra, int stall_ep,
+                                                      int force_exact, unsigned long long* paths,
+                                                      unsigned long long* paths_next) {
   using G = DirGeo<BS, NPOW>;
   if (rlo_dev) {
     rlo = *rlo_dev;
-    if (rlo == INF32) return;
+    if (rlo == INF32) {
+      if (blockIdx.x == 0 && threadIdx.x == 0 && paths) paths_next[0] = paths_next[1] = 0;
+      return;
+    }
   }
   uint64_t st_t = 0, st_acc[9] = {0, 0, 0, 0, 0, 0, 0, 0, 0};
   const bool stamping = kDirStamps && dbg && blockIdx.x == 0 && threadIdx.x == 0;
@@ -362,11 +548,19 @@
     }
     L.sP[tid] = P;
   }
+  if constexpr (G::NARROW) {
+    if (tid < NPOW) ((uint16_t*)L.sB16)[dir_base_slot<BS, NPOW>(tid)] = tid < N ? (uint16_t)hge_narrow::nar_base16(L.sP[tid]) : 0;
+  }
   if (tid == 0) {
     L.s_stamp = stamping ? 1 : 0;
     L.sdbg[0] = L.sdbg[1] = 0;
+    L.sEx[0] = L.sEx[1] = 0;
   }
   __syncthreads();
+  if constexpr (G::NARROW) {
+    if (tid < N && hge_narrow::nar_base_too_large(L.sP[tid])) atomicOr(&L.sEx[rlo & 1], 1);
+  }
+  int n_nar = 0, n_ex = 0;
   const int rcap = hist ? hmax : t.Rcap;
   int extra_left = -1;
   uint2 pv[G::PREF];
@@ -375,6 +569,7 @@
   int f0 = INF32, fn = 0;
   uint32_t mw[G::CW];
   dir_members_fd<BS, NPOW>(t, d, part, d < N ? L.sP[d] : INF32, mw);
+  if constexpr (G::NARROW) __syncthreads();
   for (int r = rlo;; r++) {
     if (r + 1 >= rcap) {
       if (c == 0 && tid == 0) {
@@ -391,47 +586,75 @@
     if (tid < DIR_MAXP) L.sCnt[tid] = 0;
     if (tid < 8) L.sBits[tid] = 0;
     if (tid < DirGeo<BS, NPOW>::W / 2) L.sHist[tid] = 0;
-    if (tid == 0) L.sFlag[(r + 1) & 1] = 0;
+    if (tid == 0) {
+      L.sFlag[(r + 1) & 1] = 0;
+      L.sEx[(r + 1) & 1] = 0;
+    }
+    const int Pc = L.sP[c];
+    const int cur = (r + 1 < Rprev) ? t.C[(size_t)(r + 1) * N + c] : INF32;
+    uint32_t nw[G::NCW];
+    bool enc = false;
+    if constexpr (G::NARROW) {
+      enc = Pc != INF32 && cur == INF32 && lo != INF32 && lo < lenc && !force_exact;
+      if (enc) {
+        const uint32_t mx = dir_encode_window<BS, NPOW>(t, L, lo);
+        const uint32_t mn = dir_encode_members<BS, NPOW>(L, part, mw, nw);
+        if (hge_narrow::nar_window_flag(mx) || hge_narrow::nar_member_flag(mn)) L.sEx[r & 1] = 1;
+      }
+    }
     __syncthreads();
     DSTAMP(0);
-    const int Pc = L.sP[c];
-    const int cur = (r + 1 < Rprev) ? t.C[(size_t)(r + 1) * N + c] : INF32;
     int slot = 0;
     int nxt = INF32;
-    bool pb = false, have_bits = false;
-    if (Pc != INF32) {
-      if (cur != INF32) {
-        nxt = cur;
+    bool pb = false;
+    const bool stall = stall_ep > 0 && r - rlo + 1 == stall_ep;
+    auto publish = [&]() {
+      DSTAMP(1);
+      if (stamping) st_acc[6] += slot;
+      if (tid < 64 && !(stall && c == 0)) {
+        dir_stage_member<BS, NPOW>(t, mbp[(r + 1) & 1], c, nxt);
+        asm volatile("s_waitcnt vmcnt(0)" ::: "memory");
+        if (tid == 0) {
+          if (hist) hist[(size_t)(r + 1) * N + c] = nxt;
+          else if (nxt != INF32 && cur == INF32) t.C[(size_t)(r + 1) * N + c] = nxt;
+          const uint64_t g = ((uint64_t)(uint32_t)(r - rlo + 1) << 32) | (uint32_t)nxt;
+          __hip_atomic_store(gr[(r + 1) & 1] + c, (unsigned long long)g, __ATOMIC_RELAXED,
+                             __HIP_MEMORY_SCOPE_AGENT);
+        }
+      }
+    };
+    if (Pc == INF32) {
+      publish();
+    } else if (cur != INF32) {
+      nxt = cur;
+      publish();
+      if (nxt < lo || nxt >= lo + DirGeo<BS, NPOW>::W) {
+        __syncthreads();
+        lo = nxt;
+        dir_load<BS, NPOW>(t, L, c, lo, DirGeo<BS, NPOW>::W, lenc, pv);
+        __syncthreads();
+      }
+      pb = dir_count<BS, NPOW>(L, nxt, part, mw) >= t.SM;
+    } else {
+      int s;
+      if constexpr (G::NARROW) {
+        const uint32_t* mbr = mbp[r & 1];
+        if (enc && L.sEx[r & 1] == 0) {
+          n_nar++;
+          s = dir_select<BS, NPOW, true>(t, c, lenc, L, d, part, nw, slot, pv, lo, pb, mbr, r == rlo);
+        } else {
+          n_ex++;
+          dir_members_reload<BS, NPOW>(t, L, mbr, r == rlo, d, part, mw);
+          s = dir_select<BS, NPOW, false>(t, c, lenc, L, d, part, mw, slot, pv, lo, pb, mbr, r == rlo);
+        }
       } else {
-        const int s = dir_select<BS, NPOW>(t, c, lenc, L, d, part, mw, slot, pv, lo, pb);
-        nxt = s < lenc ? s : INF32;
-        have_bits = nxt != INF32;
-      }
-    }
-    DSTAMP(1);
-    if (stamping) st_acc[6] += slot;
-    const bool stall = stall_ep > 0 && r - rlo + 1 == stall_ep;
-    if (tid < 64 && !(stall && c == 0)) {
-      dir_stage_member<BS, NPOW>(t, mbp[(r + 1) & 1], c, nxt);
-      asm volatile("s_waitcnt vmcnt(0)" ::: "memory");
-      if (tid == 0) {
-        if (hist) hist[(size_t)(r + 1) * N + c] = nxt;
-        else if (nxt != INF32 && cur == INF32) t.C[(size_t)(r + 1) * N + c] = nxt;
-        const uint64_t g = ((uint64_t)(uint32_t)(r - rlo + 1) << 32) | (uint32_t)nxt;
-        __hip_atomic_store(gr[(r + 1) & 1] + c, (unsigned long long)g, __ATOMIC_RELAXED,
-                           __HIP_MEMORY_SCOPE_AGENT);
-      }
+        n_ex++;
+        s = dir_select<BS, NPOW, false>(t, c, lenc, L, d, part, mw, slot, pv, lo, pb, nullptr, false);
+      }
+      nxt = s < lenc ? s : INF32;
+      publish();
     }
     if (nxt != INF32) {
-      if (!have_bits) {
-        if (nxt < lo || nxt >= lo + DirGeo<BS, NPOW>::W) {
-          __syncthreads();
-          lo = nxt;
-          dir_load<BS, NPOW>(t, L, c, lo, DirGeo<BS, NPOW>::W, lenc, pv);
-          __syncthreads();
-        }
-        pb = dir_count<BS, NPOW>(L, nxt, part, mw) >= t.SM;
-      }
       if (part == 0 && d < N && pb) atomicOr(&L.sBits[d >> 5], 1u << (d & 31));
       __syncthreads();
       if (tid < NW)
@@ -458,6 +681,8 @@
     asm volatile("s_waitcnt vmcnt(0)" ::: "memory");
     DSTAMP(3);
     {
+      const int tp = dir_tid();
+      const int d = tp / G::TPM, part = tp - d * G::TPM;
       const unsigned ep = (unsigned)(r - rlo + 1);
       const gu64_t* g = gr[(r + 1) & 1];
       unsigned spins = 0;
@@ -478,7 +703,14 @@
         __builtin_amdgcn_s_sleep(1);
       }
       __builtin_amdgcn_fence(__ATOMIC_ACQUIRE, "wavefront");
-      if (part == 0 && d < N) L.sP[d] = P;
+      if (part == 0 && d < N) {
+        L.sP[d] = P;
+        if constexpr (G::NARROW) ((uint16_t*)L.sB16)[dir_base_slot<BS, NPOW>(d)] = (uint16_t)hge_narrow::nar_base16(P);
+      }
+      if constexpr (G::NARROW) {
+        if (__ballot(part == 0 && d < N && hge_narrow::nar_base_too_large(P)) != 0 && (threadIdx.x & 63) == 0)
+          L.sEx[(r + 1) & 1] = 1;
+      }
       const bool any = __ballot(d < N && P != INF32) != 0;
       const bool notpast = stopcut && __ballot(part == 0 && d < N && P < stopcut[d]) != 0;
       if ((threadIdx.x & 63) == 0 && (any || notpast || fail))
@@ -487,7 +719,12 @@
         atomicOr(err, 1);
         atomicOr(rstate + 1, 4);
       }
-      if (!fail) dir_members_mb<BS, NPOW>(mbp[(r + 1) & 1], mw);
+      if (!fail) {
+        dir_members_mb<BS, NPOW>(mbp[(r + 1) & 1], mw);
+      } else {
+#pragma unroll
+        for (int k = 0; k < G::CW; k++) mw[k] = 0;
+      }
     }
     __syncthreads();
     DSTAMP(4);
@@ -508,6 +745,11 @@
       }
     }
   }
+  if (tid == 0 && paths) {
+    atomicAdd(paths, (unsigned long long)n_nar);
+    atomicAdd(paths + 1, (unsigned long long)n_ex);
+    if (c == 0) paths_next[0] = paths_next[1] = 0;
+  }
   if (stamping) {
     for (int q = 0; q < 9; q++) dbg[q] += st_acc[q];
     dbg[9] += L.sdbg[0];
@@ -518,10 +760,10 @@
 }
 
 template __global__ void k_rounds_direct<1024, 64>(Tables, const int32_t*, const int32_t*, int32_t*, int, const int32_t*, int,
-    uint64_t*, int32_t*, uint64_t*, uint32_t*, uint64_t*, const int32_t*, int32_t*, int, const int32_t*, int, int);
+    uint64_t*, int32_t*, uint64_t*, uint32_t*, uint64_t*, const int32_t*, int32_t*, int, const int32_t*, int, int, int, unsigned long long*, unsigned long long*);
 template __global__ void k_rounds_direct<1024, 128>(Tables, const int32_t*, const int32_t*, int32_t*, int, const int32_t*, int,
-    uint64_t*, int32_t*, uint64_t*, uint32_t*, uint64_t*, const int32_t*, int32_t*, int, const int32_t*, int, int);
+    uint64_t*, int32_t*, uint64_t*, uint32_t*, uint64_t*, const int32_t*, int32_t*, int, const int32_t*, int, int, int, unsigned long long*, unsigned long long*);
 template __global__ void k_rounds_direct<1024, 256>(Tables, const int32_t*, const int32_t*, int32_t*, int, const int32_t*, int,
-    uint64_t*, int32_t*, uint64_t*, uint32_t*, uint64_t*, const int32_t*, int32_t*, int, const int32_t*, int, int);
-
-}
+    uint64_t*, int32_t*, uint64_t*, uint32_t*, uint64_t*, const int32_t*, int32_t*, int, const int32_t*, int, int, int, unsigned long long*, unsigned long long*);
+
+}
diff --git a/babble_amd/engine.py b/babble_amd/engine.py
--- a/babble_amd/engine.py
+++ b/babble_amd/engine.py
@@ -62,7 +62,7 @@
     "hge_fame", "hge_round_events", "hge_round_received", "hge_consensus_timestamp",
     "hge_consensus_timestamp_sources",
     "hge_ancestor", "hge_self_ancestor", "hge_see", "hge_strongly_see",
-    "hge_oldest_self_ancestor_to_see", "hge_coordinates", "hge_coordinate_sweeps", "hge_host_syncs", "hge_frontier_fallbacks",
+    "hge_oldest_self_ancestor_to_see", "hge_coordinates", "hge_coordinate_sweeps", "hge_walk_select_paths", "hge_host_syncs", "hge_frontier_fallbacks",
     "hge_stage_times",
     "hge_set_profiling", "hge_reset_kernel_stats", "hge_kernel_stats",
     "hge_consensus_log", "hge_event_rounds", "hge_event_received", "hge_set_cache_size",
@@ -147,6 +147,8 @@
     L.hge_stage_times.argtypes = [vp, P(ctypes.c_float), ctypes.c_int]
     L.hge_coordinate_sweeps.restype = ctypes.c_int32
     L.hge_coordinate_sweeps.argtypes = [vp]
+    if hasattr(L, "hge_walk_select_paths"):
+        L.hge_walk_select_paths.argtypes = [vp, P(i64), P(i64)]
     if hasattr(L, "hge_gob_encode_wire_events"):
         L.hge_gob_encode_wire_events.argtypes = [vp, i64, P(ctypes.c_uint8), P(i64), i32, P(ctypes.c_uint8), i64,
                                                  P(i64)]
@@ -607,6 +609,11 @@
     def coordinate_sweeps(self):
         return self.L.hge_coordinate_sweeps(self.h)
 
+    def walk_select_paths(self):
+        nar, ex = ctypes.c_int64(), ctypes.c_int64()
+        self._check(self.L.hge_walk_select_paths(self.h, ctypes.byref(nar), ctypes.byref(ex)))
+        return nar.value, ex.value
+
     def host_syncs(self):
         return int(self.L.hge_host_syncs(self.h))
 
diff --git a/include/hge.h b/include/hge.h
--- a/include/hge.h
+++ b/include/hge.h
@@ -208,6 +208,7 @@
 
 int hge_stage_times(hge_engine* h, float* ms_out, int cap);
 int32_t hge_coordinate_sweeps(hge_engine* h);
+int hge_walk_select_paths(hge_engine* h, int64_t* narrow, int64_t* exact);
 int64_t hge_host_syncs(hge_engine* h);
 int64_t hge_frontier_fallbacks(hge_engine* h);
 int hge_set_profiling(hge_engine* h, int on);
```
